# flupkede/codesearch

Measured on AMD Instinct MI355X. Metric: chunks embedded+searched/sec over 10M×384 corpus; recall@10 vs CPU ref, higher is better.
Workload: dtype f32

## Files before the change

codesearch_amd/_lib.py:

```python
from __future__ import annotations

import ctypes as C
import os

PKG_DIR = os.path.dirname(os.path.abspath(__file__))
LIB_PATH = os.environ.get("CS_LIBCSGPU") or os.path.join(PKG_DIR, "libcsgpu.so")
DIAG_LIB_PATH = os.environ.get("CS_LIBCSGPU_DIAG") or os.path.join(PKG_DIR, "libcsgpu_diag.so")

CS_OK, CS_ERR_BAD_ARG, CS_ERR_DIM_MISMATCH, CS_ERR_NOT_BUILT = 0, 1, 2, 3
CS_ERR_CANCELLED, CS_ERR_OOM, CS_ERR_HIP, CS_ERR_UNSUPPORTED = 4, 5, 6, 7
CS_GEMM_F32, CS_GEMM_SPLIT_F16, CS_GEMM_Q8_DYNAMIC = 0, 1, 2
CS_MAX_K = 1024
CS_MAX_QUERIES = 4096
CS_SIMILAR_EXCLUDE_NONE, CS_SIMILAR_EXCLUDE_SELF, CS_SIMILAR_EXCLUDE_GROUP = 0, 1, 2
CS_SIMILAR_ROUTE_AUTO, CS_SIMILAR_ROUTE_SCAN, CS_SIMILAR_ROUTE_FILTER = 0, 1, 2
CS_MAX_PAIRS = 1 << 22
CS_PAIRS_ALL, CS_PAIRS_OTHER_GROUP = 0, 1
CS_NO_ID = 0xFFFFFFFF
CS_NO_CLASS = 0xFFFF
CS_MAX_CLASSES = 4096

f32p = C.POINTER(C.c_float)
u32p = C.POINTER(C.c_uint32)
u16p = C.POINTER(C.c_uint16)
# ... 87 lines not shown
    "cs_index_search_similar": (C.c_int32, [vp, u32p, C.c_uint32, C.c_uint32, C.c_int32, C.c_float, f32p, u32p, u32p]),
    "cs_index_set_similar_route": (C.c_int32, [vp, C.c_int32]),
    "cs_index_similar_route_info": (C.c_int32, [vp, u64p, u64p, u64p]),
    "cs_index_search_similar_scoped": (C.c_int32, [vp, vp, u32p, C.c_uint32, C.c_uint32, C.c_int32, C.c_float, f32p, u32p,
                                                   u32p]),
    "cs_index_similar_pairs": (C.c_int32, [vp, C.c_float, C.c_int32, C.c_uint32, u32p, u32p, f32p, u64p]),
    "cs_index_similar_pairs_info": (C.c_int32, [u64p, u32p, f64p, f64p, f64p]),
    "cs_index_similar_clusters": (C.c_int32, [vp, C.c_float, C.c_int32, u32p, C.c_uint64, u64p, u64p]),
    "cs_index_similar_clusters_info": (C.c_int32, [u64p, u64p, u64p, u32p, f64p, f64p]),
    "cs_index_similar_clusters_scoped": (C.c_int32, [vp, vp, vp, C.c_float, C.c_int32, u32p, u32p, C.c_uint64, u64p, u64p, u64p]),
    "cs_index_similar_clusters_scoped_info": (C.c_int32, [f64p, u64p, u64p, u64p]),
    "cs_index_similar_pairs_scoped": (C.c_int32, [vp, vp, vp, C.c_float, C.c_int32, C.c_uint32, u32p, u32p, f32p, u64p]),
    "cs_index_similar_pairs_scoped_info": (C.c_int32, [f64p, u64p, u64p, u64p]),
    "cs_index_search_scoped": (C.c_int32, [vp, vp, f32p, C.c_uint32, C.c_uint32, C.c_uint32, f32p, u32p, u32p]),
    "cs_index_search_variants_scoped": (C.c_int32, [vp, vp, f32p, C.c_uint32, C.c_uint32, C.c_uint32, f32p, u32p, u32p,
                                                    i32p]),
    "cs_index_search_scoped_device": (C.c_int32, [vp, vp, vp, C.c_uint32, C.c_uint32, C.c_uint32, vp, vp, vp, vp, vp]),
    "cs_merge_variants_device": (C.c_int32, [C.c_int32, vp, C.c_uint32, C.c_uint32, C.c_uint32, vp, vp, vp, vp, vp, vp]),
    "cs_index_search_status": (C.c_int32, [vp, vp, u32p]),
    "cs_index_release_stream": (C.c_int32, [vp, vp]),
    "cs_merge_topk_device": (C.c_int32, [C.c_int32, vp, C.c_uint32, C.c_uint32, C.c_uint32, vp, vp, vp, vp, vp]),
    "cs_shards_create": (C.c_int32, [C.c_uint32, C.c_uint32, i32p, C.c_uint64, C.c_uint64, C.POINTER(vp)]),
    "cs_shards_destroy": (None, [vp]),
    "cs_shards_add": (C.c_int32, [vp, f32p, C.c_uint64, C.c_uint32, u32p]),
    "cs_shards_add_device": (C.c_int32, [vp, vp, C.c_int32, C.c_uint64, C.c_uint32, u32p, vp]),
    "cs_shards_add_synthetic": (C.c_int32, [vp, C.c_uint64, C.c_uint64, C.c_uint64, u32p]),
    "cs_shards_remove": (C.c_int32, [vp, u32p, C.c_uint64, u64p]),
    "cs_shards_build": (C.c_int32, [vp]),
    "cs_shards_clear": (C.c_int32, [vp]),
    "cs_shards_is_built": (C.c_int32, [vp]),
    "cs_shards_len": (C.c_uint64, [vp]),
    "cs_shards_stored_rows": (C.c_uint64, [vp]),
    "cs_shards_next_id": (C.c_uint32, [vp]),
    "cs_shards_dim": (C.c_uint32, [vp]),
    "cs_shards_count": (C.c_uint32, [vp]),
    "cs_shards_shard_len": (C.c_uint64, [vp, C.c_uint32]),
    "cs_shards_direct_gather": (C.c_int32, [vp]),
    "cs_shards_search": (C.c_int32, [vp, f32p, C.c_uint32, C.c_uint32, C.c_uint32, f32p, u32p, u32p]),
    "cs_shards_search_device": (C.c_int32, [vp, vp, C.c_uint32, C.c_uint32, C.c_uint32, vp, vp, vp, vp, vp]),
    "cs_shards_search_status": (C.c_int32, [vp, vp, u32p]),
    "cs_shards_root_device": (C.c_int32, [vp]),
    "cs_shards_shard_device": (C.c_int32, [vp, C.c_uint32]),
    "cs_shards_shard_index": (vp, [vp, C.c_uint32]),
    "cs_shards_search_variants": (C.c_int32, [vp, f32p, C.c_uint32, C.c_uint32, C.c_uint32, f32p, u32p, u32p, i32p]),
    "cs_shards_search_masked": (C.c_int32, [vp, f32p, C.c_uint32, C.c_uint32, C.c_uint32, u32p, C.c_uint64, f32p, u32p,
                                            u32p]),
    "cs_shards_search_variants_masked": (C.c_int32, [vp, f32p, C.c_uint32, C.c_uint32, C.c_uint32, u32p, C.c_uint64, f32p,
                                                     u32p, u32p, i32p]),
    "cs_shards_scope_create": (C.c_int32, [vp, u32p, C.c_uint64, C.POINTER(vp)]),
    "cs_shards_search_scoped": (C.c_int32, [vp, vp, f32p, C.c_uint32, C.c_uint32, C.c_uint32, f32p, u32p, u32p]),
    "cs_shards_search_variants_scoped": (C.c_int32, [vp, vp, f32p, C.c_uint32, C.c_uint32, C.c_uint32, f32p, u32p, u32p,
                                                     i32p]),
    "cs_shards_read_rows": (C.c_int32, [vp, C.c_uint64, C.c_uint64, f32p]),
    "cs_index_read_rows": (C.c_int32, [vp, C.c_uint64, C.c_uint64, f32p]),
    "cs_index_debug_counters": (C.c_int32, [vp, u64p, u64p]),
    "cs_index_filter_state": (C.c_int32, [vp, C.POINTER(C.c_int32), C.POINTER(C.c_float), u64p]),
    "cs_index_filter_copies": (C.c_int32, [vp, C.POINTER(C.c_int32), C.POINTER(C.c_int32), u64p]),
    "cs_index_set_filter_min_queries": (C.c_int32, [vp, C.c_uint32]),
    "cs_index_set_single_query_route": (C.c_int32, [vp, C.c_int32]),
    "cs_index_profile": (C.c_int32, [vp, C.c_int32]),
    "cs_index_profile_read": (C.c_int32, [vp, f64p, u64p, f64p, C.c_int32]),
    "cs_bert_config_bge_small": (None, [C.POINTER(BertConfig)]),
    "cs_bert_param_count": (C.c_uint64, [C.POINTER(BertConfig)]),
    "cs_embedder_create": (C.c_int32, [C.POINTER(BertConfig), f32p, C.c_uint64, C.c_int32, C.POINTER(vp)]),
    "cs_embedder_create_quantized": (C.c_int32, [C.POINTER(BertConfig), f32p, f32p, C.c_uint64, C.c_int32, C.POINTER(vp)]),
    "cs_bert_quant_columns": (C.c_uint64, [C.POINTER(BertConfig)]),
    "cs_bert_params_from_onnx_q": (C.c_int32, [C.c_char_p, C.POINTER(BertConfig), f32p, C.c_uint64, f32p, C.c_uint64,
                                               C.POINTER(C.c_int32)]),
    "cs_bert_config_from_dir": (C.c_int32, [C.c_char_p, C.c_int32, C.POINTER(BertConfig)]),
    "cs_bert_params_from_safetensors": (C.c_int32, [C.c_char_p, C.POINTER(BertConfig), f32p, C.c_uint64]),
    "cs_bert_params_from_onnx": (C.c_int32, [C.c_char_p, C.POINTER(BertConfig), f32p, C.c_uint64]),
    "cs_embedder_create_from_dir": (C.c_int32, [C.c_char_p, C.c_int32, C.c_int32, C.POINTER(vp)]),
    "cs_embedder_destroy": (None, [vp]),
    "cs_embedder_dim": (C.c_uint32, [vp]),
    "cs_embedder_embed_ids": (C.c_int32, [vp, i32p, i32p, C.c_uint64, C.c_uint32, C.c_uint32, f32p, i32p]),
    "cs_embedder_embed_ids_device": (C.c_int32, [vp, i32p, i32p, C.c_uint64, C.c_uint32, C.c_uint32, vp, i32p]),
    "cs_embedder_last_hidden": (C.c_int32, [vp, f32p, C.c_uint64]),
    "cs_embedder_profile_read": (C.c_int32, [vp, f64p, u64p, C.c_int32]),
    "cs_embedder_profile_stages": (C.c_int32, [vp, C.c_int32]),
    "cs_embedder_profile_stages_read": (C.c_int32, [vp, f64p, u64p, C.c_int32]),
    "cs_embedder_set_gemm_mode": (C.c_int32, [vp, C.c_int32]),
    "cs_embedder_gemm_mode": (C.c_int32, [vp]),
    "cs_embedder_debug_counters": (C.c_int32, [vp, u64p, u64p, u64p]),
    "cs_tokenizer_create": (C.c_int32, [C.c_char_p, C.c_uint64, C.c_int32, C.c_uint32, C.POINTER(vp)]),
    "cs_tokenizer_create_from_file": (C.c_int32, [C.c_char_p, C.c_int32, C.c_uint32, C.POINTER(vp)]),
    "cs_tokenizer_create_from_json": (C.c_int32, [C.c_char_p, C.c_uint32, C.POINTER(vp)]),
    "cs_tokenizer_create_from_dir": (C.c_int32, [C.c_char_p, C.c_uint32, C.POINTER(vp)]),
    "cs_tokenizer_destroy": (None, [vp]),
    "cs_tokenizer_vocab_size": (C.c_uint32, [vp]),
    "cs_tokenizer_max_length": (C.c_uint32, [vp]),
    "cs_tokenizer_pad_id": (C.c_int32, [vp]),
    "cs_tokenizer_token_to_id": (C.c_int32, [vp, C.c_char_p]),
    "cs_tokenizer_encode_batch": (C.c_int32, [vp, C.c_char_p, u64p, C.c_uint32, C.c_uint32, i32p, i32p,
                                              C.c_uint32, u32p]),
    "cs_tokenizer_encode_pairs": (C.c_int32, [vp, C.c_char_p, u64p, C.c_uint32, C.c_char_p, u64p, C.c_uint32, C.c_uint32, i32p, i32p,
                                              i32p, C.c_uint32, u32p]),
    "cs_embedder_embed_texts": (C.c_int32, [vp, vp, C.c_char_p, u64p, C.c_uint64, C.c_uint32, f32p, i32p]),
    "cs_embedder_embed_texts_device": (C.c_int32, [vp, vp, C.c_char_p, u64p, C.c_uint64, C.c_uint32, vp, i32p]),
    "cs_embedder_submit_texts": (C.c_int32, [vp, vp, C.c_char_p, u64p, C.c_uint64, u64p]),
    "cs_embedder_submit_ids": (C.c_int32, [vp, i32p, i32p, C.c_uint64, C.c_uint32, u64p]),
    "cs_embedder_wait": (C.c_int32, [vp, C.c_uint64, f32p, i32p]),
    "cs_embedder_wait_device": (C.c_int32, [vp, C.c_uint64, vp, i32p]),
    "cs_embedder_discard": (C.c_int32, [vp, C.c_uint64]),
    "cs_embedder_queued_rows": (C.c_uint64, [vp]),
    "cs_shards_plan_append": (C.c_int32, [vp, C.c_uint64, C.c_uint32, u32p, u64p, u64p, u32p]),
    "cs_shards_add_device_parts": (C.c_int32, [vp, C.c_uint32, C.POINTER(vp), i32p, u64p, C.c_uint32, u32p]),
    "cs_embedders_create": (C.c_int32, [C.POINTER(BertConfig), f32p, C.c_uint64, i32p, C.c_uint32, C.POINTER(vp)]),
    "cs_embedders_create_from_dir": (C.c_int32, [C.c_char_p, C.c_int32, i32p, C.c_uint32, C.POINTER(vp)]),
    "cs_embedders_destroy": (None, [vp]),
    "cs_embedders_count": (C.c_uint32, [vp]),
    "cs_embedders_dim": (C.c_uint32, [vp]),
    "cs_embedders_replica": (vp, [vp, C.c_uint32]),
    "cs_embedders_device": (C.c_int32, [vp, C.c_uint32]),
    "cs_embedders_embed_texts": (C.c_int32, [vp, vp, C.c_char_p, u64p, C.c_uint64, C.c_uint32, f32p, i32p]),
    "cs_embedders_embed_ids": (C.c_int32, [vp, i32p, i32p, C.c_uint64, C.c_uint32, C.c_uint32, f32p, i32p]),
    "cs_embedders_index_texts": (C.c_int32, [vp, vp, vp, C.c_char_p, u64p, C.c_uint64, C.c_uint32, u32p, i32p]),
    "cs_embedders_index_ids": (C.c_int32, [vp, vp, i32p, i32p, C.c_uint64, C.c_uint32, C.c_uint32, u32p, i32p]),
    "cs_rerank_head_count": (C.c_uint64, [C.POINTER(BertConfig)]),
    "cs_reranker_create": (C.c_int32, [C.POINTER(BertConfig), f32p, f32p, C.c_uint64, C.c_int32, C.POINTER(vp)]),
    "cs_rerank_head_from_safetensors": (C.c_int32, [C.c_char_p, C.POINTER(BertConfig), f32p, C.c_uint64]),
    "cs_reranker_create_from_dir": (C.c_int32, [C.c_char_p, C.c_int32, C.POINTER(vp)]),
    "cs_reranker_destroy": (None, [vp]),
    "cs_reranker_embedder": (vp, [vp]),
    "cs_reranker_score_ids": (C.c_int32, [vp, i32p, i32p, i32p, C.c_uint64, C.c_uint32, C.c_uint32, f32p, i32p]),
    "cs_reranker_rerank_texts": (C.c_int32, [vp, vp, C.c_char_p, C.c_char_p, u64p, C.c_uint64, C.c_uint32, f32p, u32p, f32p]),
    "cs_rerank_order": (C.c_int32, [f32p, C.c_uint64, u32p, f32p]),
    "cs_rerank_blend": (C.c_int32, [f32p, f32p, C.c_uint64, u32p, f32p]),
}

DIAG_SIGNATURES = {
    "cs_debug_small_forward_counters": (C.c_int32, [vp, u64p, u64p]),
    "cs_debug_gemm_time": (C.c_int32, [C.c_int32, C.c_int32, C.c_int32, C.c_uint32, C.c_uint32, C.c_uint32, C.c_uint32,
                                       C.c_int32, f64p]),
    "cs_debug_gemm_q8": (C.c_int32, [C.c_int32, C.c_int32, C.c_int32, f32p, f32p, f32p, f32p, f32p, f32p, C.c_uint32,
                                     C.c_uint32, C.c_uint32, C.POINTER(C.c_uint8), f32p, i32p]),
    "cs_debug_gemm_q8_units": (C.c_int32, [C.c_int32, C.c_int32, f32p, f32p, f32p, f32p, f32p, f32p, C.c_uint32, C.c_uint32,
                                           C.c_uint32, u32p, C.c_uint32, f32p, i32p]),
    "cs_debug_gemm": (C.c_int32, [C.c_int32, C.c_int32, C.c_int32, f32p, f32p, f32p, f32p, f32p,
                                  C.c_uint32, C.c_uint32, C.c_uint32, u32p]),
    "cs_debug_rows": (C.c_int32, [C.c_int32, C.c_int32, C.c_uint32, C.c_uint32, C.c_uint32, C.c_uint32, C.c_float, C.c_int32,
                                  i32p, f32p, f32p, f32p, i32p, C.c_uint32, C.c_uint32, f32p, i32p, f32p, C.c_uint32, f32p, f32p, f32p,
                                  C.c_int32, f32p, f32p, f32p, f32p, u32p]),
    "cs_debug_elementwise": (C.c_int32, [C.c_int32, C.c_int32, C.c_int32, C.c_uint32, C.c_uint32, C.c_uint32, C.c_uint32, C.c_uint32,
                                         C.c_int32, C.c_float, f32p, f32p, f32p, f32p, u32p]),
    "cs_debug_attention_cls": (C.c_int32, [C.c_int32, f32p, i32p, C.c_uint32, C.c_uint32, C.c_uint32, C.c_uint32, f32p, u32p, f32p,
                                           f32p, C.POINTER(C.c_uint16)]),
    "cs_debug_attention_f32": (C.c_int32, [C.c_int32, f32p, i32p, C.c_uint32, C.c_uint32, C.c_uint32, C.c_uint32, f32p, C.c_uint32,
                                           f32p]),
    "cs_debug_small_path": (C.c_int32, [C.c_int32, C.c_int32, C.c_int32, C.c_int32, C.c_uint32, C.c_uint32, C.c_uint32, C.c_uint32,
                                        C.c_float, f32p, f32p, f32p, f32p, f32p, f32p, i32p, f32p, f32p, f32p, i32p, C.c_uint32,
                                        C.c_uint32, f32p, f32p, f32p, f32p, f32p, f32p, u32p, u32p]),
    "cs_debug_attention": (C.c_int32, [C.c_int32, f32p, i32p, C.c_uint32, C.c_uint32, C.c_uint32, C.c_uint32, f32p, C.c_uint32,
                                       u32p, u32p, C.c_uint32, f32p, f32p, f32p, f32p, f32p, C.c_uint32, u32p, u32p]),
}

_LIB = None
_DIAG = None


def load() -> C.CDLL:
    global _LIB
    if _LIB is not None:
        return _LIB
    if not os.path.exists(LIB_PATH):
        raise FileNotFoundError(
            f"{LIB_PATH} is missing: build it with `python -c 'import __graft_entry__ as g; g.build()'` "
            "(make -C codesearch_amd/csrc). There is no CPU fallback."
        )
    try:
        import torch
    except Exception:
        pass
    lib = C.CDLL(LIB_PATH, mode=C.RTLD_GLOBAL)
    for name, (res, args) in SIGNATURES.items():
        fn = getattr(lib, name)
        fn.restype = res
        fn.argtypes = args
    _LIB = lib
    return lib


def load_diag() -> C.CDLL:
    global _DIAG
    if _DIAG is not None:
        return _DIAG
    if not os.path.exists(DIAG_LIB_PATH):
        raise FileNotFoundError(f"{DIAG_LIB_PATH} is missing: build it with `make -C codesearch_amd/csrc`")
    load()
    lib = C.CDLL(DIAG_LIB_PATH, mode=C.RTLD_LOCAL)
    for name, (res, args) in {**SIGNATURES, **DIAG_SIGNATURES}.items():
        fn = getattr(lib, name)
        fn.restype = res
        fn.argtypes = args
    _DIAG = lib
    return lib


def check_diag(status: int) -> None:
    if status != CS_OK:
        raise CsError(status, load_diag().cs_last_error().decode("utf-8", "replace"))


def last_error() -> str:
    return load().cs_last_error().decode("utf-8", "replace")


def check(status: int) -> None:
    if status != CS_OK:
        raise CsError(status, last_error())
```

codesearch_amd/csrc/attention_shx_body.hpp:

```cpp
#pragma once

#include "encoder.hpp"
#include "split_f16.hpp"

#ifndef AT_STAMP
#define AT_STAMP(i)
#endif
#ifndef CS_ATTN_ARITH
#define CS_ATTN_ARITH 2
#endif
#ifndef CS_ATTN_LAZY_RESCALE
#define CS_ATTN_LAZY_RESCALE 4.0f
#endif
#ifndef CS_ATTN_PIPE_FENCE
#define CS_ATTN_PIPE_FENCE __builtin_amdgcn_sched_barrier(0)
#endif

namespace cs {

typedef __fp16 h16x2 __attribute__((ext_vector_type(2)));

constexpr float kLog2e = 1.4426950408889634f;
constexpr float kMaskedLog2 = -3.0e38f;

union Frag8 {
    f16x8 v;
    uint32_t u[4];
    uint2 d[2];
};

typedef short s16x4 __attribute__((ext_vector_type(4)));

union FragTr {
    f16x8 v;
    s16x4 q[2];
};

__device__ __forceinline__ void split_pair_rtz_ng(float a, float b, uint32_t& hi, uint32_t& lo) {
    const h16x2 h = __builtin_amdgcn_cvt_pkrtz(a, b);
    const h16x2 l = __builtin_amdgcn_cvt_pkrtz((a - (float)h[0]) * kShLoScale, (b - (float)h[1]) * kShLoScale);
    hi = __builtin_bit_cast(uint32_t, h);
    lo = __builtin_bit_cast(uint32_t, l);
}

__device__ __forceinline__ float mix_residual_lo(float e, uint32_t hpair) {
    float r;
    asm("v_fma_mix_f32 %0, %1, -1.0, %2 op_sel_hi:[1,0,0]" : "=v"(r) : "v"(hpair), "v"(e));
    return r;
}
__device__ __forceinline__ float mix_residual_hi(float e, uint32_t hpair) {
    float r;
    asm("v_fma_mix_f32 %0, %1, -1.0, %2 op_sel:[1,0,0] op_sel_hi:[1,0,0]" : "=v"(r) : "v"(hpair), "v"(e));
    return r;
}

__device__ __forceinline__ float xhalf_max_swap(float t) {
    const uint32_t u = __builtin_bit_cast(uint32_t, t);
    const auto r = __builtin_amdgcn_permlane32_swap(u, u, false, false);
    const uint32_t a = r[0], b = r[1];
    return fmaxf(__builtin_bit_cast(float, a), __builtin_bit_cast(float, b));
}

struct AttnMemPlain {
    __device__ __forceinline__ f16x8 ld16(const _Float16* p) const { return *reinterpret_cast<const f16x8*>(p); }
    __device__ __forceinline__ f16x8 stage_load(const _Float16* src, char* lds_piece) const { sh_glds16(src, lds_piece); return f16x8{}; }
    __device__ __forceinline__ void stage_store(char*, int, f16x8) const {}
    __device__ __forceinline__ void st8(_Float16* p, f16x4 v) const { *reinterpret_cast<f16x4*>(p) = v; }
};

template <int NC, class MQ, class MO, int POS = 0, int PIPE = 0>
__device__ __forceinline__ void
attention_shx_body(char* smem, const MQ& mq, const MO& mo, const _Float16* qkvs, const int32_t* __restrict__ mask,
                   _Float16* ctxs, uint32_t* __restrict__ flag, uint32_t L, uint32_t H,
                   float scale_log2e, uint32_t HB, float* __restrict__ range_out,
                   const uint32_t* __restrict__ seq_unit, const uint32_t* __restrict__ unit_len,
                   uint32_t bx, uint32_t by, uint32_t bz, uint32_t gx, uint32_t gz, const float* __restrict__ alibi_log2 = nullptr,
                   uint32_t window = 0) {
    constexpr bool ALIBI = POS == 1, WINDOW = POS == 2;
    constexpr bool IMM = PIPE >= 2;
    constexpr bool EARLY = PIPE == 3;
    const float wlimit = (float)window;
    constexpr int KT = 128;
    const uint32_t Lp = (L + 31) & ~31u;
    char* Kt = smem;
    char* Vt = Kt + (size_t)NC * KT * 128;
    float* madd = reinterpret_cast<float*>(Vt + (size_t)NC * KT * 128);
    int* last_valid_p = reinterpret_cast<int*>(madd + Lp);
    const int tid = threadIdx.x, lane = tid & 63;
    const int wave = __builtin_amdgcn_readfirstlane(tid >> 6);
    const int l31 = lane & 31, h = lane >> 5;
    const uint32_t wq = 4 / HB, hsub = (uint32_t)wave / wq, qt = (uint32_t)wave % wq;
    const uint32_t head = bx * HB + hsub, b = by, qb = bz;
    Kt += (size_t)hsub * (KT / HB) * 128;
    Vt += (size_t)hsub * (KT / HB) * 128;
    const uint32_t nh = H / (32 * NC), nch = 3 * nh * NC;
    const _Float16* base = qkvs + (size_t)b * L * nch * 64;
    bool ovf = false;

    AT_STAMP(0);
    if (tid == 0) *last_valid_p = 0;

    const int kswz = (l31 >> 1) & 7;
    int k_hi[2], k_lo[2];
#pragma unroll
    for (int s = 0; s < 2; ++s) {
        k_hi[s] = ((2 * s + h) ^ kswz) * 16;
        k_lo[s] = ((4 + 2 * s + h) ^ kswz) * 16;
    }
    const int vq = (lane & 15) >> 2, vp = lane & 3, vg = (lane >> 4) & 1;
    const int vfv = 4 * ((vq >> 1) & 1);
    const int v_hi = (4 * h + vq) * 128 + (((2 * vg + (vp >> 1)) ^ vfv) * 16) + 8 * (vp & 1);
    const int v_lo = v_hi ^ 64;

    const bool wave_live = qb * 128 + qt * 32 < L;
    const uint32_t query = qb * 128 + qt * 32 + l31;
    const uint32_t qsrc = query < L ? query : L - 1;
    float neg_slope = 0.0f;
    const float qpos = (float)query - (float)(4 * h);
    if constexpr (ALIBI) neg_slope = -alibi_log2[head];
    f16x8 qh[NC][2], ql[NC][2];
#pragma unroll
    for (int c = 0; c < NC; ++c) {
        const _Float16* qp = base + ((size_t)qsrc * nch + head * NC + c) * 64 + 8 * h;
#pragma unroll
        for (int s = 0; s < 2; ++s) {
            qh[c][s] = mq.ld16(qp + 16 * s);
            ql[c][s] = mq.ld16(qp + 32 + 16 * s);
        }
    }
#if CS_ATTN_ARITH == 2 && !defined(CS_ATTN_SCALAR_SOFTMAX)
    f16x8 qhs[NC][2];
#pragma unroll
    for (int c = 0; c < NC; ++c)
#pragma unroll
        for (int s = 0; s < 2; ++s) {
            qhs[c][s] = qh[c][s] * (_Float16)kShLoInv;
            ql[c][s] = ql[c][s] * (_Float16)kShLoInv;
        }
#endif
    sh_f32x16 ohh[NC], oxx[NC];
#pragma unroll
    for (int c = 0; c < NC; ++c)
#pragma unroll
        for (int r = 0; r < 16; ++r) { ohh[c][r] = 0.0f; oxx[c][r] = 0.0f; }
    float m = -__builtin_huge_valf(), lsum = 0.0f;

    auto stage = [&](uint32_t st) {
        const uint32_t live = Lp - st * KT < (uint32_t)KT ? Lp - st * KT : (uint32_t)KT;
        for (uint32_t i0 = qt; i0 < live / 8; i0 += 4 * wq) {
            f16x8 rk[4][NC], rv[4][NC];
#pragma unroll
            for (int u = 0; u < 4; ++u) {
                const uint32_t ii = i0 + u * wq;
                if (ii < live / 8) {
                    const uint32_t row = ii * 8 + (lane >> 3);
                    const uint32_t gk = st * KT + row;
                    const uint32_t key = gk < L ? gk : L - 1;
                    const uint32_t ck = (lane & 7) ^ ((row >> 1) & 7);
                    const uint32_t cv = (lane & 7) ^ (4 * ((row >> 1) & 1));
#pragma unroll
                    for (int c = 0; c < NC; ++c) {
                        rk[u][c] = mq.stage_load(base + ((size_t)key * nch + (nh + head) * NC + c) * 64 + ck * 8, Kt + (size_t)c * KT * 128 + ii * 1024);
                        rv[u][c] = mq.stage_load(base + ((size_t)key * nch + (2 * nh + head) * NC + c) * 64 + cv * 8, Vt + (size_t)c * KT * 128 + ii * 1024);
                    }
                }
            }
#pragma unroll
            for (int u = 0; u < 4; ++u) {
                const uint32_t ii = i0 + u * wq;
                if (ii < live / 8) {
#pragma unroll
                    for (int c = 0; c < NC; ++c) {
                        mq.stage_store(Kt + (size_t)c * KT * 128 + ii * 1024, lane, rk[u][c]);
                        mq.stage_store(Vt + (size_t)c * KT * 128 + ii * 1024, lane, rv[u][c]);
                    }
                }
            }
        }
    };
    stage(0);
    __syncthreads();
    for (uint32_t key = tid; key < Lp; key += 256) {
        const bool ok = key < L && mask[(size_t)b * L + key] != 0;
        madd[key] = ok ? 0.0f : kMaskedLog2;
        if (ok) atomicMax(last_valid_p, (int)key);
    }
    asm volatile("s_waitcnt vmcnt(0)" ::: "memory");
    __syncthreads();
    const uint32_t ntiles = (uint32_t)(*last_valid_p) / 32 + 1;

    typedef __attribute__((address_space(3))) char* lds_char_p;
    typedef __attribute__((address_space(3))) const f16x8* lds_f16x8_cp;
    typedef __attribute__((address_space(3))) const sh_f32x4* lds_f32x4_cp;
    uint32_t ka[4] = {0, 0, 0, 0}, va[2] = {0, 0}, ma0 = 0;
    if constexpr (IMM) {
        const uint32_t k0 = (uint32_t)(uintptr_t)(lds_char_p)Kt + (uint32_t)l31 * 128u, v0 = (uint32_t)(uintptr_t)(lds_char_p)Vt;
#pragma unroll
        for (int s = 0; s < 2; ++s) { ka[s] = k0 + (uint32_t)k_hi[s]; ka[2 + s] = k0 + (uint32_t)k_lo[s]; }
        va[0] = v0 + (uint32_t)v_hi;
        va[1] = v0 + (uint32_t)v_lo;
        ma0 = (uint32_t)(uintptr_t)(lds_char_p)reinterpret_cast<char*>(madd) + 16u * (uint32_t)h;
#pragma unroll
        for (int i = 0; i < 4; ++i) asm volatile("" : "+v"(ka[i]));
        asm volatile("" : "+v"(va[0]), "+v"(va[1]), "+v"(ma0));
    }

    for (uint32_t st = 0; st * 4 < ntiles; ++st) {
        if constexpr (WINDOW) {
            if (st * KT > qb * 128 + 127 + window || st * KT + (KT - 1) + window < qb * 128) continue;
        }
        if (st > 0) {
            __syncthreads();
            stage(st);
            asm volatile("s_waitcnt vmcnt(0)" ::: "memory");
            __syncthreads();
        }
        if (!wave_live) continue;
        const uint32_t kt_end = ntiles - st * 4 < 4 ? ntiles - st * 4 : 4;
        const uint32_t ma_st = ma0 + st * 512u;
        uint32_t kl_lo = 0, kl_hi = kt_end;
        if constexpr (WINDOW) {
            const int q0 = (int)(qb * 128 + qt * 32), w = (int)window, t0 = (int)(st * 4);
            const int first = q0 - 31 - w > 0 ? (q0 - 31 - w + 31) / 32 : 0, past = (q0 + 31 + w) / 32 + 1;
            kl_lo = (uint32_t)(first > t0 ? first - t0 : 0);
            kl_hi = past - t0 < (int)kt_end ? (uint32_t)(past - t0 > 0 ? past - t0 : 0) : kt_end;
        }
        auto compute_s = [&](uint32_t kl, sh_f32x16& hh, sh_f32x16& xx) __attribute__((always_inline)) {
#pragma unroll
            for (int r = 0; r < 16; ++r) { hh[r] = 0.0f; xx[r] = 0.0f; }
            if constexpr (EARLY) {
                f16x8 kf[NC][4];
#pragma unroll
                for (int c = 0; c < NC; ++c)
#pragma unroll
                    for (int i = 0; i < 4; ++i) kf[c][i] = *(lds_f16x8_cp)(uintptr_t)(ka[i] + (uint32_t)(c * KT * 128) + kl * 4096u);
                __builtin_amdgcn_sched_barrier(0);
#pragma unroll
                for (int c = 0; c < NC; ++c)
#pragma unroll
                    for (int s = 0; s < 2; ++s) {
                        hh = __builtin_amdgcn_mfma_f32_32x32x16_f16(kf[c][s], qh[c][s], hh, 0, 0, 0);
#if CS_ATTN_ARITH == 2 && !defined(CS_ATTN_SCALAR_SOFTMAX)
                        hh = __builtin_amdgcn_mfma_f32_32x32x16_f16(kf[c][s], ql[c][s], hh, 0, 0, 0);
                        hh = __builtin_amdgcn_mfma_f32_32x32x16_f16(kf[c][2 + s], qhs[c][s], hh, 0, 0, 0);
#else
                        xx = __builtin_amdgcn_mfma_f32_32x32x16_f16(kf[c][s], ql[c][s], xx, 0, 0, 0);
                        xx = __builtin_amdgcn_mfma_f32_32x32x16_f16(kf[c][2 + s], qh[c][s], xx, 0, 0, 0);
#endif
                    }
                return;
            }
#pragma unroll
            for (int c = 0; c < NC; ++c) {
                const char* kr = Kt + (size_t)c * KT * 128 + (size_t)(kl * 32 + l31) * 128;
#pragma unroll
                for (int s = 0; s < 2; ++s) {
                    f16x8 kh, kl8;
                    if constexpr (IMM) {
                        kh = *(lds_f16x8_cp)(uintptr_t)(ka[s] + (uint32_t)(c * KT * 128) + kl * 4096u);
                        kl8 = *(lds_f16x8_cp)(uintptr_t)(ka[2 + s] + (uint32_t)(c * KT * 128) + kl * 4096u);
                    } else {
                        kh = *reinterpret_cast<const f16x8*>(kr + k_hi[s]);
                        kl8 = *reinterpret_cast<const f16x8*>(kr + k_lo[s]);
                    }
                    hh = __builtin_amdgcn_mfma_f32_32x32x16_f16(kh, qh[c][s], hh, 0, 0, 0);
#if CS_ATTN_ARITH == 2 && !defined(CS_ATTN_SCALAR_SOFTMAX)
                    hh = __builtin_amdgcn_mfma_f32_32x32x16_f16(kh, ql[c][s], hh, 0, 0, 0);
                    hh = __builtin_amdgcn_mfma_f32_32x32x16_f16(kl8, qhs[c][s], hh, 0, 0, 0);
#else
                    xx = __builtin_amdgcn_mfma_f32_32x32x16_f16(kh, ql[c][s], xx, 0, 0, 0);
                    xx = __builtin_amdgcn_mfma_f32_32x32x16_f16(kl8, qh[c][s], xx, 0, 0, 0);
#endif
                }
            }
        };
        auto finish_tile = [&](uint32_t kl, sh_f32x16& hh, sh_f32x16& xx) __attribute__((always_inline)) {
            const uint32_t kt = st * 4 + kl;
#ifndef CS_ATTN_SCALAR_SOFTMAX
            sh_f32x2 p2[8];
            float tmax = -__builtin_huge_valf();
            const sh_f32x2 lo_inv2 = {kShLoInv, kShLoInv}, scale2 = {scale_log2e, scale_log2e};
#pragma unroll
            for (int g = 0; g < 4; ++g) {
                sh_f32x4 ma;
                if constexpr (IMM) ma = *(lds_f32x4_cp)(uintptr_t)(ma_st + (kl * 32u + 8u * g) * 4u);
                else ma = *reinterpret_cast<const sh_f32x4*>(madd + kt * 32 + 8 * g + 4 * h);
#pragma unroll
                for (int e2 = 0; e2 < 2; ++e2) {
                    const int r = 4 * g + 2 * e2;
                    const sh_f32x2 x2 = {xx[r], xx[r + 1]}, h2 = {hh[r], hh[r + 1]};
                    sh_f32x2 m2 = {ma[2 * e2], ma[2 * e2 + 1]};
                    if constexpr (ALIBI) {
                        const float d0 = qpos - (float)(kt * 32 + 8 * g + 2 * e2);
                        m2[0] = fmaf(neg_slope, fabsf(d0), m2[0]);
                        m2[1] = fmaf(neg_slope, fabsf(d0 - 1.0f), m2[1]);
                    }
                    if constexpr (WINDOW) {
                        const float d0 = qpos - (float)(kt * 32 + 8 * g + 2 * e2);
                        m2[0] = fabsf(d0) > wlimit ? kMaskedLog2 : m2[0];
                        m2[1] = fabsf(d0 - 1.0f) > wlimit ? kMaskedLog2 : m2[1];
                    }
#if CS_ATTN_ARITH == 2
                    (void)x2; (void)lo_inv2;
                    const sh_f32x2 s2 = __builtin_elementwise_fma(h2, scale2, m2);
#else
                    const sh_f32x2 s2 = __builtin_elementwise_fma(__builtin_elementwise_fma(x2, lo_inv2, h2), scale2, m2);
#endif
                    p2[r / 2] = s2;
                    tmax = fmaxf(tmax, fmaxf(s2[0], s2[1]));
                }
            }
            if constexpr (IMM) tmax = xhalf_max_swap(tmax);
            else tmax = fmaxf(tmax, __shfl_xor(tmax, 32, 64));
#if CS_ATTN_ARITH == 2
            if (__any(tmax > m + CS_ATTN_LAZY_RESCALE)) {
#else
            if (__any(tmax > m)) {
#endif
                const float mnew = fmaxf(m, tmax);
                const float alpha = __builtin_amdgcn_exp2f(m - mnew);
                lsum *= alpha;
#pragma unroll
                for (int c = 0; c < NC; ++c)
#pragma unroll
                    for (int r = 0; r < 16; ++r) { ohh[c][r] *= alpha; oxx[c][r] *= alpha; }
                m = mnew;
            }
            typedef __attribute__((address_space(3))) s16x4* lds_s16x4_p;
            FragTr vhe[NC][2], vle[NC][2];
            if constexpr (EARLY) {
#pragma unroll
                for (int c = 0; c < NC; ++c)
#pragma unroll
                    for (int s = 0; s < 2; ++s) {
                        const uint32_t off = (uint32_t)(c * KT * 128) + kl * 4096u + (uint32_t)(s * 16 * 128);
                        vhe[c][s].q[0] = __builtin_amdgcn_ds_read_tr16_b64_v4i16((lds_s16x4_p)(uintptr_t)(va[0] + off));
                        vhe[c][s].q[1] = __builtin_amdgcn_ds_read_tr16_b64_v4i16((lds_s16x4_p)(uintptr_t)(va[0] + off + 1024u));
                        vle[c][s].q[0] = __builtin_amdgcn_ds_read_tr16_b64_v4i16((lds_s16x4_p)(uintptr_t)(va[1] + off));
                        vle[c][s].q[1] = __builtin_amdgcn_ds_read_tr16_b64_v4i16((lds_s16x4_p)(uintptr_t)(va[1] + off + 1024u));
                    }
                __builtin_amdgcn_sched_barrier(0);
            }
#if CS_ATTN_ARITH == 2
            const sh_f32x2 m2v = {m - 11.0f, m - 11.0f};
#else
            const sh_f32x2 m2v = {m, m};
#endif
            sh_f32x2 ps2 = {0.0f, 0.0f};
            Frag8 ph[2], pl[2];
            const sh_f32x2 lo_scale2 = {kShLoScale, kShLoScale};
#pragma unroll
            for (int i = 0; i < 8; ++i) {
                const sh_f32x2 d2 = p2[i] - m2v;
                const sh_f32x2 e2 = {__builtin_amdgcn_exp2f(d2[0]), __builtin_amdgcn_exp2f(d2[1])};
                ps2 += e2;
                const h16x2 hi = __builtin_amdgcn_cvt_pkrtz(e2[0], e2[1]);
#if CS_ATTN_ARITH == 2
                (void)lo_scale2;
                const uint32_t hib = __builtin_bit_cast(uint32_t, hi);
                const h16x2 lo = __builtin_amdgcn_cvt_pkrtz(mix_residual_lo(e2[0], hib), mix_residual_hi(e2[1], hib));
#else
                const sh_f32x2 back = {(float)hi[0], (float)hi[1]};
                const sh_f32x2 r2 = (e2 - back) * lo_scale2;
                const h16x2 lo = __builtin_amdgcn_cvt_pkrtz(r2[0], r2[1]);
#endif
                ph[i >> 2].u[i & 3] = __builtin_bit_cast(uint32_t, hi);
                pl[i >> 2].u[i & 3] = __builtin_bit_cast(uint32_t, lo);
            }
            lsum += ps2[0] + ps2[1];
#else
            float tmax = -__builtin_huge_valf();
#pragma unroll
            for (int g = 0; g < 4; ++g) {
                const sh_f32x4 ma = *reinterpret_cast<const sh_f32x4*>(madd + kt * 32 + 8 * g + 4 * h);
#pragma unroll
                for (int e = 0; e < 4; ++e) {
                    const int r = 4 * g + e;
                    float me = ma[e];
                    if constexpr (ALIBI) me = fmaf(neg_slope, fabsf(qpos - (float)(kt * 32 + 8 * g + e)), me);
                    if constexpr (WINDOW) me = fabsf(qpos - (float)(kt * 32 + 8 * g + e)) > wlimit ? kMaskedLog2 : me;
                    hh[r] = fmaf(fmaf(xx[r], kShLoInv, hh[r]), scale_log2e, me);
                    tmax = fmaxf(tmax, hh[r]);
                }
            }
            tmax = fmaxf(tmax, __shfl_xor(tmax, 32, 64));
            if (__any(tmax > m)) {
                const float mnew = fmaxf(m, tmax);
                const float alpha = __builtin_amdgcn_exp2f(m - mnew);
                lsum *= alpha;
#pragma unroll
                for (int c = 0; c < NC; ++c)
#pragma unroll
                    for (int r = 0; r < 16; ++r) { ohh[c][r] *= alpha; oxx[c][r] *= alpha; }
                m = mnew;
            }
            float psum = 0.0f;
#pragma unroll
            for (int r = 0; r < 16; ++r) {
                hh[r] = __builtin_amdgcn_exp2f(hh[r] - m);
                psum += hh[r];
            }
            lsum += psum;
            Frag8 ph[2], pl[2];
#pragma unroll
            for (int s = 0; s < 2; ++s)
#pragma unroll
                for (int w2 = 0; w2 < 4; ++w2) {
#ifdef CS_ATTN_P_HI_ONLY
                    const f16x2 pr = __builtin_convertvector(sh_f32x2{hh[8 * s + 2 * w2], hh[8 * s + 2 * w2 + 1]}, f16x2);
                    ph[s].u[w2] = __builtin_bit_cast(uint32_t, pr);
                    pl[s].u[w2] = 0u;
#else
                    split_pair_rtz_ng(hh[8 * s + 2 * w2], hh[8 * s + 2 * w2 + 1], ph[s].u[w2], pl[s].u[w2]);
#endif
                }
#endif
#ifdef CS_ATTN_SCALAR_SOFTMAX
            typedef __attribute__((address_space(3))) s16x4* lds_s16x4_p;
            FragTr vhe[NC][2], vle[NC][2];
#endif
#pragma unroll
            for (int c = 0; c < NC; ++c) {
                const char* vr = Vt + (size_t)c * KT * 128 + (size_t)kl * 32 * 128;
#pragma unroll
                for (int s = 0; s < 2; ++s) {
                    FragTr vh, vl;
                    if constexpr (EARLY) {
                        vh = vhe[c][s];
                        vl = vle[c][s];
                    } else if constexpr (IMM) {
                        const uint32_t off = (uint32_t)(c * KT * 128) + kl * 4096u + (uint32_t)(s * 16 * 128);
                        vh.q[0] = __builtin_amdgcn_ds_read_tr16_b64_v4i16((lds_s16x4_p)(uintptr_t)(va[0] + off));
                        vh.q[1] = __builtin_amdgcn_ds_read_tr16_b64_v4i16((lds_s16x4_p)(uintptr_t)(va[0] + off + 1024u));
                        vl.q[0] = __builtin_amdgcn_ds_read_tr16_b64_v4i16((lds_s16x4_p)(uintptr_t)(va[1] + off));
                        vl.q[1] = __builtin_amdgcn_ds_read_tr16_b64_v4i16((lds_s16x4_p)(uintptr_t)(va[1] + off + 1024u));
                    } else {
                    vh.q[0] = __builtin_amdgcn_ds_read_tr16_b64_v4i16((lds_s16x4_p)(vr + s * 16 * 128 + v_hi));
                    vh.q[1] = __builtin_amdgcn_ds_read_tr16_b64_v4i16((lds_s16x4_p)(vr + s * 16 * 128 + 8 * 128 + v_hi));
                    vl.q[0] = __builtin_amdgcn_ds_read_tr16_b64_v4i16((lds_s16x4_p)(vr + s * 16 * 128 + v_lo));
                    vl.q[1] = __builtin_amdgcn_ds_read_tr16_b64_v4i16((lds_s16x4_p)(vr + s * 16 * 128 + 8 * 128 + v_lo));
                    }
                    ohh[c] = __builtin_amdgcn_mfma_f32_32x32x16_f16(vh.v, ph[s].v, ohh[c], 0, 0, 0);
#if CS_ATTN_ARITH == 2 && !defined(CS_ATTN_SCALAR_SOFTMAX)
                    ohh[c] = __builtin_amdgcn_mfma_f32_32x32x16_f16(vh.v, pl[s].v, ohh[c], 0, 0, 0);
#elif !defined(CS_ATTN_P_HI_ONLY)
                    oxx[c] = __builtin_amdgcn_mfma_f32_32x32x16_f16(vh.v, pl[s].v, oxx[c], 0, 0, 0);
#endif
                    oxx[c] = __builtin_amdgcn_mfma_f32_32x32x16_f16(vl.v, ph[s].v, oxx[c], 0, 0, 0);
                }
            }
        };
        if constexpr (PIPE == 0) {
            for (uint32_t kl = kl_lo; kl < kl_hi; ++kl) {
                sh_f32x16 hh, xx;
                compute_s(kl, hh, xx);
                finish_tile(kl, hh, xx);
            }
        } else if constexpr (IMM) {
#pragma unroll
            for (uint32_t kl = 0; kl < 4; ++kl) {
                if (kl >= kl_lo && kl < kl_hi) {
                    sh_f32x16 hh, xx;
                    compute_s(kl, hh, xx);
                    finish_tile(kl, hh, xx);
                }
            }
        } else {
            sh_f32x16 hhA, xxA, hhB, xxB;
            if (kl_lo < kl_hi) compute_s(kl_lo, hhA, xxA);
            for (uint32_t kl = kl_lo; kl < kl_hi; kl += 2) {
                if (kl + 1 < kl_hi) compute_s(kl + 1, hhB, xxB);
                CS_ATTN_PIPE_FENCE;
                finish_tile(kl, hhA, xxA);
                if (kl + 1 < kl_hi) {
                    if (kl + 2 < kl_hi) compute_s(kl + 2, hhA, xxA);
                    CS_ATTN_PIPE_FENCE;
                    finish_tile(kl + 1, hhB, xxB);
                }
            }
        }
    }
    lsum += __shfl_xor(lsum, 32, 64);
    const float inv = lsum > 0.0f ? 1.0f / lsum : 0.0f;
    float rlo = 0.0f, rhi = 0.0f;
    if (wave_live && query < L) {
#pragma unroll
        for (int c = 0; c < NC; ++c) {
            _Float16* op = ctxs + (((size_t)b * L + query) * nh + head) * NC * 64 + c * 64 + 4 * h;
#pragma unroll
            for (int g = 0; g < 4; ++g) {
                f16x4 hi, lo;
#pragma unroll
                for (int e = 0; e < 4; ++e) {
                    _Float16 a, bb;
                    const float o = fmaf(oxx[c][4 * g + e], kShLoInv, ohh[c][4 * g + e]) * inv;
                    ovf |= sh_split(o, a, bb);
                    hi[e] = a; lo[e] = bb;
                    rlo = fminf(rlo, o);
                    rhi = fmaxf(rhi, o);
                }
                mo.st8(op + 8 * g, hi);
                mo.st8(op + 32 + 8 * g, lo);
            }
        }
    }
    AT_STAMP(2);
    if (ovf && flag) atomicOr(flag, 1u);
    if (range_out) {
        if (unit_len && query >= unit_len[seq_unit[b]]) rlo = rhi = 0.0f;
#pragma unroll
        for (int o = 32; o > 0; o >>= 1) {
            rlo = fminf(rlo, __shfl_xor(rlo, o, 64));
            rhi = fmaxf(rhi, __shfl_xor(rhi, o, 64));
        }
        if (lane == 0) {
            const size_t blk = ((size_t)by * gz + bz) * gx + bx;
            _Float16 a, bb;
            (void)sh_split(rlo, a, bb);
            range_out[(blk * 4 + wave) * 2] = fmaf((float)bb, kShLoInv, (float)a);
            (void)sh_split(rhi, a, bb);
            range_out[(blk * 4 + wave) * 2 + 1] = fmaf((float)bb, kShLoInv, (float)a);
        }
    }
}

}
```

codesearch_amd/csrc/attention_split.hip:

```cpp
#include <cstdlib>
#include "encoder.hpp"
#include "split_f16.hpp"
#include "attention_shx_body.hpp"

#ifndef AT_STAMP
#define AT_STAMP(i)
#endif

namespace cs {

#ifndef CS_ATTN_PIPE_WAVES
#define CS_ATTN_PIPE_WAVES 3
#endif

constexpr int kAttnPipeDefault32 = 2, kAttnPipeDefault64 = 3;

#ifdef CS_DIAGNOSTICS
__global__ void __launch_bounds__(256, 2)
attention_sh2_kernel(const _Float16* __restrict__ qkvs, const int32_t* __restrict__ mask,
                     _Float16* __restrict__ ctxs, uint32_t* __restrict__ flag, uint32_t L, uint32_t H,
                     float scale_log2e) {
    extern __shared__ __attribute__((aligned(16))) char smem[];
    const uint32_t Lp = (L + 31) & ~31u;
    char* Kt = smem;
    char* Vt = Kt + (size_t)Lp * 128;
    float* madd = reinterpret_cast<float*>(Vt + (size_t)Lp * 128);
    int* last_valid_p = reinterpret_cast<int*>(madd + Lp);
    const int tid = threadIdx.x, lane = tid & 63;
    const int wave = __builtin_amdgcn_readfirstlane(tid >> 6);
    const int l31 = lane & 31, h = lane >> 5;
    const uint32_t head = blockIdx.x, b = blockIdx.y;
    const uint32_t nh = H / 32, nch = 3 * nh;
    const _Float16* base = qkvs + (size_t)b * L * nch * 64;
    bool ovf = false;

    AT_STAMP(0);
    if (tid == 0) *last_valid_p = 0;
    for (uint32_t ii = wave; ii < Lp / 8; ii += 4) {
        const uint32_t row = ii * 8 + (lane >> 3);
        const uint32_t key = row < L ? row : L - 1;
        const uint32_t ck = (lane & 7) ^ ((row >> 1) & 7);
        const uint32_t cv = (lane & 7) ^ (4 * ((row >> 1) & 1));
        sh_glds16(base + ((size_t)key * nch + nh + head) * 64 + ck * 8, Kt + ii * 1024);
        sh_glds16(base + ((size_t)key * nch + 2 * nh + head) * 64 + cv * 8, Vt + ii * 1024);
    }
    __syncthreads();
    for (uint32_t key = tid; key < Lp; key += 256) {
        const bool ok = key < L && mask[(size_t)b * L + key] != 0;
        madd[key] = ok ? 0.0f : kMaskedLog2;
        if (ok) atomicMax(last_valid_p, (int)key);
    }
    asm volatile("s_waitcnt vmcnt(0)" ::: "memory");
    __syncthreads();
    const uint32_t ntiles = (uint32_t)(*last_valid_p) / 32 + 1;
    AT_STAMP(1);

    const int kswz = (l31 >> 1) & 7;
    const char* k_lane = Kt + l31 * 128;
    int k_hi[2], k_lo[2];
#pragma unroll
    for (int s = 0; s < 2; ++s) {
        k_hi[s] = ((2 * s + h) ^ kswz) * 16;
        k_lo[s] = ((4 + 2 * s + h) ^ kswz) * 16;
    }
    const int vq = (lane & 15) >> 2, vp = lane & 3, vg = (lane >> 4) & 1;
    const int vfv = 4 * ((vq >> 1) & 1);
    const int v_hi = (4 * h + vq) * 128 + (((2 * vg + (vp >> 1)) ^ vfv) * 16) + 8 * (vp & 1);
    const int v_lo = v_hi ^ 64;

    for (uint32_t qb = 0; qb * 128 < L; ++qb) {
        if (qb * 128 + wave * 32 >= L) break;
        const uint32_t query = qb * 128 + wave * 32 + l31;
        const uint32_t qsrc = query < L ? query : L - 1;
        const _Float16* qp = base + ((size_t)qsrc * nch + head) * 64 + 8 * h;
        f16x8 qh[2], ql[2];
#pragma unroll
        for (int s = 0; s < 2; ++s) {
            qh[s] = *reinterpret_cast<const f16x8*>(qp + 16 * s);
            ql[s] = *reinterpret_cast<const f16x8*>(qp + 32 + 16 * s);
        }
        sh_f32x16 ohh, oxx;
#pragma unroll
        for (int r = 0; r < 16; ++r) { ohh[r] = 0.0f; oxx[r] = 0.0f; }
        float m = -__builtin_huge_valf(), lsum = 0.0f;

        for (uint32_t kt = 0; kt < ntiles; ++kt) {
            sh_f32x16 hh, xx;
#pragma unroll
            for (int r = 0; r < 16; ++r) { hh[r] = 0.0f; xx[r] = 0.0f; }
            const char* kr = k_lane + (size_t)kt * 32 * 128;
#pragma unroll
            for (int s = 0; s < 2; ++s) {
                const f16x8 kh = *reinterpret_cast<const f16x8*>(kr + k_hi[s]);
                const f16x8 kl = *reinterpret_cast<const f16x8*>(kr + k_lo[s]);
                hh = __builtin_amdgcn_mfma_f32_32x32x16_f16(kh, qh[s], hh, 0, 0, 0);
                xx = __builtin_amdgcn_mfma_f32_32x32x16_f16(kh, ql[s], xx, 0, 0, 0);
                xx = __builtin_amdgcn_mfma_f32_32x32x16_f16(kl, qh[s], xx, 0, 0, 0);
            }
            float tmax = -__builtin_huge_valf();
#pragma unroll
            for (int g = 0; g < 4; ++g) {
                const sh_f32x4 ma = *reinterpret_cast<const sh_f32x4*>(madd + kt * 32 + 8 * g + 4 * h);
#pragma unroll
                for (int e = 0; e < 4; ++e) {
                    const int r = 4 * g + e;
                    hh[r] = fmaf(fmaf(xx[r], kShLoInv, hh[r]), scale_log2e, ma[e]);
                    tmax = fmaxf(tmax, hh[r]);
                }
            }
            tmax = fmaxf(tmax, __shfl_xor(tmax, 32, 64));
            if (__any(tmax > m)) {
                const float mnew = fmaxf(m, tmax);
                const float alpha = __builtin_amdgcn_exp2f(m - mnew);
                lsum *= alpha;
#pragma unroll
                for (int r = 0; r < 16; ++r) { ohh[r] *= alpha; oxx[r] *= alpha; }
                m = mnew;
            }
            float psum = 0.0f;
#pragma unroll
            for (int r = 0; r < 16; ++r) {
                hh[r] = __builtin_amdgcn_exp2f(hh[r] - m);
                psum += hh[r];
            }
            lsum += psum;
            Frag8 ph[2], pl[2];
#pragma unroll
            for (int s = 0; s < 2; ++s)
#pragma unroll
                for (int w2 = 0; w2 < 4; ++w2)
                    split_pair_rtz_ng(hh[8 * s + 2 * w2], hh[8 * s + 2 * w2 + 1], ph[s].u[w2], pl[s].u[w2]);
            typedef __attribute__((address_space(3))) s16x4* lds_s16x4_p;
            const char* vr = Vt + (size_t)kt * 32 * 128;
#pragma unroll
            for (int s = 0; s < 2; ++s) {
                FragTr vh, vl;
                vh.q[0] = __builtin_amdgcn_ds_read_tr16_b64_v4i16((lds_s16x4_p)(vr + s * 16 * 128 + v_hi));
                vh.q[1] = __builtin_amdgcn_ds_read_tr16_b64_v4i16((lds_s16x4_p)(vr + s * 16 * 128 + 8 * 128 + v_hi));
                vl.q[0] = __builtin_amdgcn_ds_read_tr16_b64_v4i16((lds_s16x4_p)(vr + s * 16 * 128 + v_lo));
                vl.q[1] = __builtin_amdgcn_ds_read_tr16_b64_v4i16((lds_s16x4_p)(vr + s * 16 * 128 + 8 * 128 + v_lo));
                ohh = __builtin_amdgcn_mfma_f32_32x32x16_f16(vh.v, ph[s].v, ohh, 0, 0, 0);
                oxx = __builtin_amdgcn_mfma_f32_32x32x16_f16(vh.v, pl[s].v, oxx, 0, 0, 0);
                oxx = __builtin_amdgcn_mfma_f32_32x32x16_f16(vl.v, ph[s].v, oxx, 0, 0, 0);
            }
        }
        lsum += __shfl_xor(lsum, 32, 64);
        const float inv = 1.0f / lsum;
        if (query < L) {
            _Float16* op = ctxs + (((size_t)b * L + query) * nh + head) * 64 + 4 * h;
#pragma unroll
            for (int g = 0; g < 4; ++g) {
                f16x4 hi, lo;
#pragma unroll
                for (int e = 0; e < 4; ++e) {
                    _Float16 a, bb;
                    ovf |= sh_split(fmaf(oxx[4 * g + e], kShLoInv, ohh[4 * g + e]) * inv, a, bb);
                    hi[e] = a; lo[e] = bb;
                }
                *reinterpret_cast<f16x4*>(op + 8 * g) = hi;
                *reinterpret_cast<f16x4*>(op + 32 + 8 * g) = lo;
            }
        }
    }
    AT_STAMP(2);
    if (ovf && flag) atomicOr(flag, 1u);
}
#endif

template <int NC, int POS = 0, int PIPE = 0>
__global__ void __launch_bounds__(256, NC == 1 ? (PIPE == 1 ? CS_ATTN_PIPE_WAVES : (PIPE >= 2 ? 4 : 2)) : 2)
attention_shx_kernel(const _Float16* __restrict__ qkvs, const int32_t* __restrict__ mask,
                     _Float16* __restrict__ ctxs, uint32_t* __restrict__ flag, uint32_t L, uint32_t H,
                     float scale_log2e, uint32_t HB, float* __restrict__ range_out,
                     const uint32_t* __restrict__ seq_unit, const uint32_t* __restrict__ unit_len,
                     const float* __restrict__ alibi_log2, uint32_t window) {
    extern __shared__ __attribute__((aligned(16))) char smem[];
    const AttnMemPlain mem;
    attention_shx_body<NC, AttnMemPlain, AttnMemPlain, POS, PIPE>(smem, mem, mem, qkvs, mask, ctxs, flag, L, H, scale_log2e, HB, range_out,
                                                            seq_unit, unit_len, blockIdx.x, blockIdx.y, blockIdx.z, gridDim.x,
                                                            gridDim.z, alibi_log2, window);
}

namespace {

struct ShxArgs {
    const _Float16* qkv; const int32_t* mask; _Float16* ctx; uint32_t* flag; uint32_t L, H; float scale_log2e; uint32_t hb;
    float* range_out; const uint32_t* seq_unit; const uint32_t* unit_len; const float* alibi_log2; uint32_t window;
};

template <int NC, int POS, int PIPE>
int32_t launch_shx_one(dim3 grid, size_t lds, hipStream_t s, const ShxArgs& a) {
    if (lds > 64 * 1024 - 256) {
        static PerDeviceOnce attr;
        CS_TRY(attr.run([&]() -> int32_t {
            CS_HIP(hipFuncSetAttribute(reinterpret_cast<const void*>(attention_shx_kernel<NC, POS, PIPE>),
                                       hipFuncAttributeMaxDynamicSharedMemorySize, 160 * 1024 - 64));
            return CS_OK;
        }));
    }
    hipLaunchKernelGGL((attention_shx_kernel<NC, POS, PIPE>), grid, dim3(256), lds, s, a.qkv, a.mask, a.ctx, a.flag, a.L, a.H,
                       a.scale_log2e, a.hb, a.range_out, a.seq_unit, a.unit_len, a.alibi_log2, a.window);
    CS_HIP(hipGetLastError());
    return CS_OK;
}

template <int NC>
int32_t launch_shx(int pos, int pipe, dim3 grid, size_t lds, hipStream_t s, const ShxArgs& a) {
#ifndef CS_DIAGNOSTICS
    constexpr int P = NC == 1 ? kAttnPipeDefault32 : kAttnPipeDefault64;
    (void)pipe;
    if (pos == 1) return launch_shx_one<NC, 1, P>(grid, lds, s, a);
    if (pos == 2) return launch_shx_one<NC, 2, P>(grid, lds, s, a);
    return launch_shx_one<NC, 0, P>(grid, lds, s, a);
#else
    if (pipe == 3) {
        if (pos == 1) return launch_shx_one<NC, 1, 3>(grid, lds, s, a);
        if (pos == 2) return launch_shx_one<NC, 2, 3>(grid, lds, s, a);
        return launch_shx_one<NC, 0, 3>(grid, lds, s, a);
    }
    if (pipe == 2) {
        if (pos == 1) return launch_shx_one<NC, 1, 2>(grid, lds, s, a);
        if (pos == 2) return launch_shx_one<NC, 2, 2>(grid, lds, s, a);
        return launch_shx_one<NC, 0, 2>(grid, lds, s, a);
    }
    if (pipe == 1) {
        if (pos == 1) return launch_shx_one<NC, 1, 1>(grid, lds, s, a);
        if (pos == 2) return launch_shx_one<NC, 2, 1>(grid, lds, s, a);
        return launch_shx_one<NC, 0, 1>(grid, lds, s, a);
    }
    if (pos == 1) return launch_shx_one<NC, 1, 0>(grid, lds, s, a);
    if (pos == 2) return launch_shx_one<NC, 2, 0>(grid, lds, s, a);
    return launch_shx_one<NC, 0, 0>(grid, lds, s, a);
#endif
}

}

int32_t launch_attention_sh2(const _Float16* qkv_split, const int32_t* mask, void* ctx_split, uint32_t* flag,
                             uint32_t B, uint32_t L, uint32_t H, uint32_t heads, hipStream_t s, float* range_out,
                             uint32_t* range_pairs, const uint32_t* seq_unit, const uint32_t* unit_len, const float* alibi,
                             uint32_t window) {
    if (alibi && window) return fail(CS_ERR_BAD_ARG, "attention: ALiBi and a local window together are not built");
    const float* alibi_log2 = alibi ? alibi + heads : nullptr;
    const int pos = alibi_log2 ? 1 : (window ? 2 : 0);
    if (range_pairs) *range_pairs = 0;
    const uint32_t dh = heads ? H / heads : 0;
    if ((dh != 32 && dh != 64) || H % heads)
        return fail(CS_ERR_UNSUPPORTED, "head_dim %u not supported (32 or 64)", dh);
    const size_t Lp = (L + 31) & ~31u;
    static const int pipe_env = [] { const char* e = cs_lab_env("CS_ATTN_PIPE"); return e && e[0] >= '0' && e[0] <= '3' ? e[0] - '0' : -1; }();
    ShxArgs a{qkv_split, mask, static_cast<_Float16*>(ctx_split), flag, L, H, 0.0f, 1u, range_out, seq_unit, unit_len, alibi_log2, window};
    if (dh == 64) {
        const size_t lds = 2 * 2 * 128 * 128 + Lp * sizeof(float) + 16;
        a.scale_log2e = (1.0f / sqrtf(64.0f)) * kLog2e;
        const int pipe = pipe_env < 0 ? kAttnPipeDefault64 : pipe_env;
        CS_TRY(launch_shx<2>(pos, pipe, dim3(heads, B, (L + 127) / 128), lds, s, a));
        if (range_pairs) *range_pairs = heads * B * ((L + 127) / 128) * 4;
        return CS_OK;
    }
    static const bool shx1 = [] { const char* e = cs_lab_env("CS_ATTN_SHX1"); return !(e && e[0] == '0'); }();
    if (shx1 || pos) {
        static const size_t lds_pad = [] { const char* e = cs_lab_env("CS_ATTN_LDS_PAD"); return e ? (size_t)std::atol(e) : (size_t)0; }();
        const size_t lds1 = 2 * 1 * 128 * 128 + Lp * sizeof(float) + 16 + lds_pad;
        static const bool pack_heads = [] { const char* e = cs_lab_env("CS_ATTN_PACK_HEADS"); return !(e && e[0] == '0'); }();
        uint32_t hb = !pack_heads ? 1u : (Lp <= 32 ? 4u : (Lp <= 64 ? 2u : 1u));
        while (heads % hb) hb >>= 1;
        a.scale_log2e = (1.0f / sqrtf(32.0f)) * kLog2e;
        a.hb = hb;
        const int pipe = pipe_env < 0 ? kAttnPipeDefault32 : pipe_env;
        CS_TRY(launch_shx<1>(pos, pipe, dim3(heads / hb, B, (L + 127) / 128), lds1, s, a));
        if (range_pairs) *range_pairs = (heads / hb) * B * ((L + 127) / 128) * 4;
        return CS_OK;
    }
#ifndef CS_DIAGNOSTICS
    return fail(CS_ERR_UNSUPPORTED, "attention: no kernel for head_dim %u", dh);
#else
    const size_t lds = 2 * Lp * 128 + Lp * sizeof(float) + 16;
    if (lds > 160 * 1024 - 64) return fail(CS_ERR_UNSUPPORTED, "sequence length %u exceeds the LDS-resident K/V limit", L);
    static PerDeviceOnce attr_set;
    CS_TRY(attr_set.run([&]() -> int32_t {
        CS_HIP(hipFuncSetAttribute(reinterpret_cast<const void*>(attention_sh2_kernel),
                                   hipFuncAttributeMaxDynamicSharedMemorySize, 160 * 1024 - 64));
        return CS_OK;
    }));
    hipLaunchKernelGGL(attention_sh2_kernel, dim3(heads, B), dim3(256), lds, s, qkv_split, mask,
                       static_cast<_Float16*>(ctx_split), flag, L, H, (1.0f / sqrtf(32.0f)) * kLog2e);
    CS_HIP(hipGetLastError());
    return CS_OK;
#endif
}

}
```

codesearch_amd/csrc/diagnostics.hip:

```cpp
#include "embedder_state.hpp"
#include "scan.hpp"
#include "../../include/codesearch_gpu_diag.h"

using namespace cs;
using namespace cs::emb;

extern "C" {

int32_t cs_debug_gemm(int32_t device, int32_t mode, int32_t epilogue, const float* A, const float* W,
                      const float* bias, const float* resid, float* C, uint32_t M, uint32_t N, uint32_t K,
                      uint32_t* range_flag) {
    if (!A || !W || !bias || !C || ((epilogue == 2 || epilogue == 3) && !resid)) return fail(CS_ERR_BAD_ARG, "null buffer");
    const bool wide = mode == 2;
    if (wide) mode = CS_GEMM_SPLIT_F16;
    if (epilogue == 3 && !(wide && N == 384)) return fail(CS_ERR_UNSUPPORTED, "epilogue 3 needs mode 2 and N = 384");
    if (epilogue < 0 || epilogue > 4 || (mode != CS_GEMM_F32 && mode != CS_GEMM_SPLIT_F16))
        return fail(CS_ERR_BAD_ARG, "unknown epilogue/mode");
    if (wide && !gemm_wide_supported(N, K)) return fail(CS_ERR_UNSUPPORTED, "wide kernel needs N %% 384 == 0");
    if (M == 0 || N % 128 || K % 32 || K == 0) return fail(CS_ERR_UNSUPPORTED, "cs_debug_gemm needs M > 0, N %% 128 == 0, K %% 32 == 0");
    int ndev = 0;
    CS_HIP(hipGetDeviceCount(&ndev));
    if (device < 0 || device >= ndev) return fail(CS_ERR_HIP, "HIP device %d not available (%d visible)", device, ndev);
    DeviceGuard g(device);
    const size_t a_n = (size_t)M * K, w_n = (size_t)N * K, c_n = (size_t)M * N;
// ... 163 lines not shown
                Q8RowMeta rm0;
                CS_HIP(hipMemcpy(hq.data(), dXq, a_n, hipMemcpyDeviceToHost));
                CS_HIP(hipMemcpy(&rm0, dRm, sizeof(rm0), hipMemcpyDeviceToHost));
                if (xq_out) for (size_t i = 0; i < a_n; ++i) xq_out[i] = (uint8_t)((int)hq[i] + 128);
                if (xparams) { xparams[0] = rm0.xs; xparams[1] = (float)(rm0.za + 128); }
            }
            return CS_OK;
        }
        const int epi = epilogue == 0 ? SH_OUT_F32 : epilogue == 1 ? SH_OUT_SPLIT_GELU : epilogue == 2 ? SH_OUT_F32_RESID : SH_OUT_SPLIT;
        if (epi == SH_OUT_SPLIT_GELU || epi == SH_OUT_SPLIT) CS_HIP(hipMalloc(&sC, c_n * 4));
        if (a_split & 4) {
            if (dAcc) CS_HIP(hipMemset(dAcc, 0, c_n * 4));
            CS_TRY(launch_gemm_q8_skinny(epi, (a_split & 1) ? Q8_SRC_SPLIT : Q8_SRC_F32, (a_split & 1) ? (const void*)sA : (const void*)dA,
                                         reinterpret_cast<const float*>(dRange), 1, dWq, dCm, dR, dC, sC, M, N, K, dF, nullptr, nullptr, nullptr));
        } else if (a_split & 16) {
            if (dAcc) CS_HIP(hipMemset(dAcc, 0, c_n * 4));
            CS_TRY(launch_gemm_q8_slab_split(dA, dRange, dWq, dCmT, sC, M, N, K, dF, nullptr));
        } else if (a_split & 8) {
            if (dAcc) CS_HIP(hipMemset(dAcc, 0, c_n * 4));
            CS_TRY(launch_gemm_q8_from_source(epi, (a_split & 1) ? Q8_SRC_SPLIT : Q8_SRC_F32, (a_split & 1) ? (const void*)sA : (const void*)dA, dRange,
                                              dWq, dCm, dB, dR, dC, sC, M, N, K, dF, nullptr));
        } else
        CS_TRY(launch_gemm_q8(epi, dXq, dRm, dWq, dCm, dB, dR, dC, sC, M, N, K, dF, nullptr, dAcc));
        CS_HIP(hipDeviceSynchronize());
        uint32_t flags[2] = {0, 0};
        CS_HIP(hipMemcpy(flags, dF, 8, hipMemcpyDeviceToHost));
        if (flags[1]) return fail(CS_ERR_BAD_ARG, "cs_debug_gemm_q8: W is not a quantised matrix for these column scales (flag %u)", flags[1]);
        if (sC) {
            std::vector<_Float16> hs(c_n * 2);
            CS_HIP(hipMemcpy(hs.data(), sC, c_n * 4, hipMemcpyDeviceToHost));
            const size_t nch = N / 32;
            for (size_t m = 0; m < M; ++m)
                for (size_t n = 0; n < N; ++n) {
                    const _Float16* line = hs.data() + (m * nch + n / 32) * 64;
                    C[m * N + n] = (float)line[n % 32] + (float)line[32 + n % 32] * (1.0f / 2048.0f);
                }
        } else {
            CS_HIP(hipMemcpy(C, dC, c_n * 4, hipMemcpyDeviceToHost));
        }
        if (acc_out) CS_HIP(hipMemcpy(acc_out, dAcc, c_n * 4, hipMemcpyDeviceToHost));
        if (xq_out || xparams) {
            std::vector<int8_t> hq(a_n);
            Q8RowMeta rm0;
            CS_HIP(hipMemcpy(hq.data(), dXq, a_n, hipMemcpyDeviceToHost));
            CS_HIP(hipMemcpy(&rm0, dRm, sizeof(rm0), hipMemcpyDeviceToHost));
            if (xq_out) for (size_t i = 0; i < a_n; ++i) xq_out[i] = (uint8_t)((int)hq[i] + 128);
            if (xparams) { xparams[0] = rm0.xs; xparams[1] = (float)(rm0.za + 128); }
        }
        return CS_OK;
    };
    const int32_t st = run();
    for (void* p : {(void*)dA, (void*)dW, (void*)dS, (void*)dB, (void*)dR, (void*)dC, (void*)sA, (void*)sC, (void*)dXq, (void*)dWq,
                    (void*)dRm, (void*)dCm, (void*)dF, (void*)dRange, (void*)dAcc, (void*)dCmT})
        if (p) (void)hipFree(p);
    return st;
}

int32_t cs_debug_gemm_q8_units(int32_t device, int32_t epilogue, const float* A, const float* W, const float* wscale,
                               const float* bias, const float* resid, float* C, uint32_t M, uint32_t N, uint32_t K,
                               const uint32_t* row_slot, uint32_t units, float* row_params, int32_t* rowsums) {
    if (!A || !W || !wscale || !bias || !C || !row_slot || (epilogue == 2 && !resid)) return fail(CS_ERR_BAD_ARG, "null buffer");
    if (epilogue != 2 && epilogue != 4 && epilogue != 5) return fail(CS_ERR_BAD_ARG, "unknown epilogue %d", epilogue);
    if (M == 0 || units == 0 || N % 128 || !q8_rows_from_source(forward_knobs(), M, K))
        return fail(CS_ERR_UNSUPPORTED, "cs_debug_gemm_q8_units: M=%u N=%u K=%u is not a row-block product", M, N, K);
    for (uint32_t m = 0; m < M; ++m)
        if ((row_slot[m] & 0x7fffffffu) >= units || (m && (row_slot[m] & 0x7fffffffu) < (row_slot[m - 1] & 0x7fffffffu)))
            return fail(CS_ERR_BAD_ARG, "row_slot[%u]: units must be consecutive runs of rows, in order", m);
    int ndev = 0;
    CS_HIP(hipGetDeviceCount(&ndev));
    if (device < 0 || device >= ndev) return fail(CS_ERR_HIP, "HIP device %d not available (%d visible)", device, ndev);
    DeviceGuard g(device);
    const size_t a_n = (size_t)M * K, w_n = (size_t)N * K, c_n = (size_t)M * N;
    float *dA = nullptr, *dW = nullptr, *dS = nullptr, *dB = nullptr, *dR = nullptr, *dC = nullptr;
    _Float16 *sA = nullptr, *sC = nullptr;
    int8_t *dXq = nullptr, *dWq = nullptr, *dOut = nullptr;
    Q8RowMeta *dRm = nullptr, *dRm2 = nullptr;
    Q8ColMeta* dCm = nullptr;
    uint32_t *dF = nullptr, *dRange = nullptr, *dRange2 = nullptr, *dSlot = nullptr;
    auto run = [&]() -> int32_t {
        const size_t rbytes = (size_t)units * Q8_RANGE_WORDS * 4;
        CS_HIP(hipMalloc(&dA, a_n * 4)); CS_HIP(hipMalloc(&dW, w_n * 4)); CS_HIP(hipMalloc(&dS, (size_t)N * 4));
        CS_HIP(hipMalloc(&dB, (size_t)N * 4)); CS_HIP(hipMalloc(&dC, c_n * 4)); CS_HIP(hipMalloc(&dF, 16));
        CS_HIP(hipMalloc(&dXq, a_n)); CS_HIP(hipMalloc(&dWq, w_n)); CS_HIP(hipMalloc(&dRm, (size_t)M * sizeof(Q8RowMeta)));
        CS_HIP(hipMalloc(&dCm, (size_t)N * sizeof(Q8ColMeta))); CS_HIP(hipMalloc(&dRange, rbytes)); CS_HIP(hipMalloc(&dRange2, rbytes));
        CS_HIP(hipMalloc(&dSlot, (size_t)M * 4));
        CS_HIP(hipMemcpy(dA, A, a_n * 4, hipMemcpyHostToDevice));
        CS_HIP(hipMemcpy(dW, W, w_n * 4, hipMemcpyHostToDevice));
        CS_HIP(hipMemcpy(dS, wscale, (size_t)N * 4, hipMemcpyHostToDevice));
        CS_HIP(hipMemcpy(dB, bias, (size_t)N * 4, hipMemcpyHostToDevice));
        CS_HIP(hipMemcpy(dSlot, row_slot, (size_t)M * 4, hipMemcpyHostToDevice));
        CS_HIP(hipMemset(dF, 0, 16));
        CS_HIP(hipMemset(dRange, 0, rbytes));
        CS_HIP(hipMemset(dRange2, 0, rbytes));
        CS_TRY(launch_q8_pack_weight(dW, dS, dB, N, K, dWq, dCm, dF + 1, nullptr));
        if (epilogue == 2) {
            CS_HIP(hipMalloc(&sA, a_n * 4));
            CS_HIP(hipMalloc(&dR, c_n * 4));
            CS_HIP(hipMemcpy(dR, resid, c_n * 4, hipMemcpyHostToDevice));
            CS_TRY(launch_split_rows(dA, sA, M, K, dF, nullptr));
            CS_TRY(launch_q8_quantize(Q8_SRC_SPLIT, sA, M, K, dRange, dSlot, dXq, dRm, nullptr));
            CS_TRY(launch_gemm_q8_from_source(SH_OUT_F32_RESID, Q8_SRC_SPLIT, sA, dRange, dWq, dCm, dB, dR, dC, nullptr, M, N, K, dF, nullptr, dSlot));
        } else {
            CS_TRY(launch_q8_quantize(Q8_SRC_F32, dA, M, K, dRange, dSlot, dXq, dRm, nullptr));
            if (epilogue == 4) {
                CS_HIP(hipMalloc(&sC, c_n * 4));
                CS_TRY(launch_gemm_q8_from_source(SH_OUT_SPLIT, Q8_SRC_F32, dA, dRange, dWq, dCm, dB, nullptr, nullptr, sC, M, N, K, dF, nullptr, dSlot));
            } else {
                CS_HIP(hipMalloc(&dOut, c_n));
                CS_HIP(hipMalloc(&dRm2, (size_t)M * sizeof(Q8RowMeta)));
                CS_TRY(launch_gemm_q8_gelu_requant_from_source(dA, dRange, dWq, dCm, dB, M, N, K, dRange2, dOut, dRm2, nullptr, dSlot));
            }
        }
        CS_HIP(hipDeviceSynchronize());
        uint32_t flags[2] = {0, 0};
        CS_HIP(hipMemcpy(flags, dF, 8, hipMemcpyDeviceToHost));
        if (flags[1]) return fail(CS_ERR_BAD_ARG, "cs_debug_gemm_q8_units: W is not a quantised matrix for these column scales (flag %u)", flags[1]);
        std::vector<Q8RowMeta> hr(M), hr2;
        CS_HIP(hipMemcpy(hr.data(), dRm, (size_t)M * sizeof(Q8RowMeta), hipMemcpyDeviceToHost));
        if (epilogue == 5) {
            std::vector<int8_t> ho(c_n);
            hr2.resize(M);
            CS_HIP(hipMemcpy(ho.data(), dOut, c_n, hipMemcpyDeviceToHost));
            CS_HIP(hipMemcpy(hr2.data(), dRm2, (size_t)M * sizeof(Q8RowMeta), hipMemcpyDeviceToHost));
            for (size_t i = 0; i < c_n; ++i) C[i] = (float)((int)ho[i] + 128);
            if (rowsums) for (size_t m = 0; m < M; ++m) rowsums[m] = hr2[m].rowsum + 128 * (int32_t)N;
        } else if (sC) {
            std::vector<_Float16> hs(c_n * 2);
            CS_HIP(hipMemcpy(hs.data(), sC, c_n * 4, hipMemcpyDeviceToHost));
            const size_t nch = N / 32;
            for (size_t m = 0; m < M; ++m)
                for (size_t n = 0; n < N; ++n) {
                    const _Float16* line = hs.data() + (m * nch + n / 32) * 64;
                    C[m * N + n] = (float)line[n % 32] + (float)line[32 + n % 32] * (1.0f / 2048.0f);
                }
        } else {
            CS_HIP(hipMemcpy(C, dC, c_n * 4, hipMemcpyDeviceToHost));
        }
        if (row_params)
            for (size_t m = 0; m < M; ++m) {
                row_params[4 * m] = hr[m].xs;
                row_params[4 * m + 1] = (float)(hr[m].za + 128);
                row_params[4 * m + 2] = epilogue == 5 ? hr2[m].xs : 0.0f;
                row_params[4 * m + 3] = epilogue == 5 ? (float)(hr2[m].za + 128) : 0.0f;
            }
        return CS_OK;
    };
    const int32_t st = run();
    for (void* p : {(void*)dA, (void*)dW, (void*)dS, (void*)dB, (void*)dR, (void*)dC, (void*)sA, (void*)sC, (void*)dXq, (void*)dWq,
                    (void*)dOut, (void*)dRm, (void*)dRm2, (void*)dCm, (void*)dF, (void*)dRange, (void*)dRange2, (void*)dSlot})
        if (p) (void)hipFree(p);
    return st;
}

int32_t cs_debug_attention(int32_t device, const float* qkv, const int32_t* mask, uint32_t B, uint32_t L, uint32_t H,
                           uint32_t heads, const float* alibi_slopes, uint32_t window, const uint32_t* seq_unit,
                           const uint32_t* unit_len, uint32_t units, const float* proj_w, const float* proj_bias,
                           const float* proj_resid, float* out, float* range_pairs_out, uint32_t range_pairs_cap,
                           uint32_t* range_pairs, uint32_t* range_flag) {
    if (!qkv || !mask || !out) return fail(CS_ERR_BAD_ARG, "null buffer");
    if (B == 0 || L == 0 || H == 0 || heads == 0) return fail(CS_ERR_BAD_ARG, "cs_debug_attention needs B, L, H, heads > 0");
    if (H % heads || (H / heads != 32 && H / heads != 64))
        return fail(CS_ERR_UNSUPPORTED, "head_dim %u not supported (32 or 64)", H / heads);
    if (L > 8192 || (uint64_t)B * L > (1u << 20)) return fail(CS_ERR_UNSUPPORTED, "cs_debug_attention: L <= 8192, B * L <= 2^20");
    if ((units != 0) != (seq_unit != nullptr) || (units != 0) != (unit_len != nullptr))
        return fail(CS_ERR_BAD_ARG, "seq_unit, unit_len and units go together");
    for (uint32_t b = 0; b < B && units; ++b)
        if (seq_unit[b] >= units) return fail(CS_ERR_BAD_ARG, "seq_unit[%u] = %u: only %u units", b, seq_unit[b], units);
    if ((range_pairs_out != nullptr) != (range_pairs != nullptr) || (range_pairs_out && range_pairs_cap == 0))
        return fail(CS_ERR_BAD_ARG, "range_pairs_out, its capacity and range_pairs go together");
    const uint32_t T = B * L;
    if (!proj_w != !proj_bias || !proj_w != !proj_resid) return fail(CS_ERR_BAD_ARG, "proj_w, proj_bias and proj_resid go together");
    if (proj_w) {
        if (alibi_slopes || window || units || range_pairs_out)
            return fail(CS_ERR_BAD_ARG, "attention inside the out-projection takes no ALiBi, window, units or range pairs");
        if (!sp_attn_proj_supported(H, heads, T, L))
            return fail(CS_ERR_UNSUPPORTED, "attention + out-projection in one launch: %u rows of %u tokens, hidden %u, %u heads not built", T, L, H, heads);
    }
    int ndev = 0;
    CS_HIP(hipGetDeviceCount(&ndev));
    if (device < 0 || device >= ndev) return fail(CS_ERR_HIP, "HIP device %d not available (%d visible)", device, ndev);
    DeviceGuard g(device);
    const size_t q_n = (size_t)T * 3 * H, c_n = (size_t)T * H;
    const size_t pair_cap = (size_t)heads * B * ((L + 127) / 128) * 4;
    float *dQ = nullptr, *dW = nullptr, *dB = nullptr, *dR = nullptr, *dC = nullptr, *dAl = nullptr, *dRp = nullptr;
    _Float16 *sQ = nullptr, *sW = nullptr, *sC = nullptr;
    int32_t* dM = nullptr;
    uint32_t *dF = nullptr, *dSu = nullptr, *dUl = nullptr;
    auto run = [&]() -> int32_t {
        CS_HIP(hipMalloc(&dQ, q_n * 4)); CS_HIP(hipMalloc(&sQ, q_n * 4)); CS_HIP(hipMalloc(&dM, (size_t)T * 4)); CS_HIP(hipMalloc(&dF, 4));
        CS_HIP(hipMemcpy(dQ, qkv, q_n * 4, hipMemcpyHostToDevice));
        CS_HIP(hipMemcpy(dM, mask, (size_t)T * 4, hipMemcpyHostToDevice));
        CS_HIP(hipMemset(dF, 0, 4));
        CS_TRY(launch_split_rows(dQ, sQ, T, 3 * H, dF, nullptr));
        if (proj_w) {
            CS_HIP(hipMalloc(&dW, (size_t)H * H * 4)); CS_HIP(hipMalloc(&sW, (size_t)H * H * 4)); CS_HIP(hipMalloc(&dB, (size_t)H * 4));
            CS_HIP(hipMalloc(&dR, c_n * 4)); CS_HIP(hipMalloc(&dC, c_n * 4));
            CS_HIP(hipMemcpy(dW, proj_w, (size_t)H * H * 4, hipMemcpyHostToDevice));
            CS_HIP(hipMemcpy(dB, proj_bias, (size_t)H * 4, hipMemcpyHostToDevice));
            CS_HIP(hipMemcpy(dR, proj_resid, c_n * 4, hipMemcpyHostToDevice));
            CS_TRY(launch_split_rows(dW, sW, H, H, dF, nullptr));
            CS_TRY(launch_sp_attn_proj(sQ, dM, sW, dB, dR, dC, T, L, H, heads, dF, nullptr));
            CS_HIP(hipDeviceSynchronize());
            CS_HIP(hipMemcpy(out, dC, c_n * 4, hipMemcpyDeviceToHost));
            if (range_flag) CS_HIP(hipMemcpy(range_flag, dF, 4, hipMemcpyDeviceToHost));
            return CS_OK;
        }
        CS_HIP(hipMalloc(&sC, c_n * 4));
        CS_HIP(hipMemset(sC, 0, c_n * 4));
        if (alibi_slopes) {
            std::vector<float> sl(2 * (size_t)heads);
            for (uint32_t i = 0; i < heads; ++i) { sl[i] = alibi_slopes[i]; sl[heads + i] = sl[i] * 1.4426950408889634f; }
            CS_HIP(hipMalloc(&dAl, sl.size() * 4));
            CS_HIP(hipMemcpy(dAl, sl.data(), sl.size() * 4, hipMemcpyHostToDevice));
        }
        if (units) {
            CS_HIP(hipMalloc(&dSu, (size_t)B * 4)); CS_HIP(hipMalloc(&dUl, (size_t)units * 4));
            CS_HIP(hipMemcpy(dSu, seq_unit, (size_t)B * 4, hipMemcpyHostToDevice));
            CS_HIP(hipMemcpy(dUl, unit_len, (size_t)units * 4, hipMemcpyHostToDevice));
        }
        if (range_pairs_out) {
            CS_HIP(hipMalloc(&dRp, pair_cap * 8));
            CS_HIP(hipMemset(dRp, 0, pair_cap * 8));
        }
        uint32_t pairs = 0;
        CS_TRY(launch_attention_sh2(sQ, dM, sC, dF, B, L, H, heads, nullptr, dRp, range_pairs_out ? &pairs : nullptr, dSu, dUl, dAl, window));
        CS_HIP(hipDeviceSynchronize());
        if (range_pairs_out) {
            *range_pairs = pairs;
            if (pairs > pair_cap) return fail(CS_ERR_HIP, "attention reported %u range pairs, more than one per wave (%zu)", pairs, pair_cap);
            if (pairs > range_pairs_cap) return fail(CS_ERR_BAD_ARG, "range_pairs_out holds %u pairs, the launch wrote %u", range_pairs_cap, pairs);
            CS_HIP(hipMemcpy(range_pairs_out, dRp, (size_t)pairs * 8, hipMemcpyDeviceToHost));
        }
        std::vector<_Float16> hs(c_n * 2);
        CS_HIP(hipMemcpy(hs.data(), sC, c_n * 4, hipMemcpyDeviceToHost));
        const size_t nch = H / 32;
        for (size_t m = 0; m < T; ++m)
            for (size_t n = 0; n < H; ++n) {
                const _Float16* line = hs.data() + (m * nch + n / 32) * 64;
                out[m * H + n] = (float)line[n % 32] + (float)line[32 + n % 32] * (1.0f / 2048.0f);
            }
        if (range_flag) CS_HIP(hipMemcpy(range_flag, dF, 4, hipMemcpyDeviceToHost));
        return CS_OK;
    };
    const int32_t st = run();
    if (st != CS_OK) (void)hipDeviceSynchronize();
    for (void* p : {(void*)dQ, (void*)dW, (void*)dB, (void*)dR, (void*)dC, (void*)dAl, (void*)dRp, (void*)sQ, (void*)sW, (void*)sC,
                    (void*)dM, (void*)dF, (void*)dSu, (void*)dUl})
        if (p) (void)hipFree(p);
    return st;
}

}

namespace {

struct DiagBufs {
    std::vector<void*> owned;
    ~DiagBufs() {
        (void)hipDeviceSynchronize();
        for (void* q : owned) (void)hipFree(q);
    }
    template <class T>
    int32_t get(T** out, size_t bytes, const void* host = nullptr) {
        void* q = nullptr;
        CS_HIP(hipMalloc(&q, bytes ? bytes : 4));
        owned.push_back(q);
        if (host && bytes) CS_HIP(hipMemcpy(q, host, bytes, hipMemcpyHostToDevice));
        *out = static_cast<T*>(q);
        return CS_OK;
    }
};

int32_t diag_device(int32_t device) {
    int ndev = 0;
    CS_HIP(hipGetDeviceCount(&ndev));
    if (device < 0 || device >= ndev) return fail(CS_ERR_HIP, "HIP device %d not available (%d visible)", device, ndev);
    return CS_OK;
}

int32_t diag_read_split(const _Float16* d_split, size_t rows, size_t N, float* out) {
    std::vector<_Float16> hs(rows * N * 2);
    CS_HIP(hipMemcpy(hs.data(), d_split, rows * N * 4, hipMemcpyDeviceToHost));
    const size_t nch = N / 32;
    for (size_t m = 0; m < rows; ++m)
        for (size_t n = 0; n < N; ++n) {
            const _Float16* line = hs.data() + (m * nch + n / 32) * 64;
            out[m * N + n] = (float)line[n % 32] + (float)line[32 + n % 32] * (1.0f / 2048.0f);
        }
    return CS_OK;
}

}

extern "C" {

int32_t cs_debug_rows(int32_t device, int32_t which, uint32_t H, uint32_t T, uint32_t L, uint32_t B, float eps, int32_t pooling,
                      const int32_t* ids, const float* word, const float* pos, const float* type_table, const int32_t* types,
                      uint32_t ntypes, uint32_t vocab, const float* x, const int32_t* mask, const float* parts, uint32_t nparts,
                      const float* bias, const float* gamma, const float* beta, int32_t range_mode, float* out, float* out_split,
                      float* src_after, float* range_out, uint32_t* range_flag) {
    if (which < 0 || which > 4) return fail(CS_ERR_BAD_ARG, "cs_debug_rows: which = %d (0 embeddings, 1 LayerNorm, 2 pooling, 3 slab sum, 4 LayerNorm of a source)", which);
    if (!out || H == 0) return fail(CS_ERR_BAD_ARG, "cs_debug_rows: null output or H = 0");
    if (which == 2) {
        if (!x || !mask || B == 0 || L == 0) return fail(CS_ERR_BAD_ARG, "cs_debug_rows: pooling needs x, mask, B > 0 and L > 0");
        if (pooling != CS_POOL_CLS && pooling != CS_POOL_MEAN) return fail(CS_ERR_BAD_ARG, "cs_debug_rows: unknown pooling %d", pooling);
        if (out_split || src_after || range_mode) return fail(CS_ERR_BAD_ARG, "cs_debug_rows: pooling writes f32 rows only");
        T = B * L;
    } else {
        if (T == 0 || !gamma || !beta) return fail(CS_ERR_BAD_ARG, "cs_debug_rows: needs T > 0, gamma and beta");
        if (which == 0 && (!ids || !word || !type_table || vocab == 0 || ntypes == 0 || L == 0))
            return fail(CS_ERR_BAD_ARG, "cs_debug_rows: the embedding kernel needs ids, the word and type tables, vocab, ntypes and L > 0");
        if (which != 0 && !x) return fail(CS_ERR_BAD_ARG, "cs_debug_rows: null input rows");
        if (which == 3 && (!parts || !bias || nparts == 0)) return fail(CS_ERR_BAD_ARG, "cs_debug_rows: the slab sum needs parts, bias and nparts > 0");
        if (range_mode < 0 || range_mode > 2 || (range_mode != 0) != (range_out != nullptr))
            return fail(CS_ERR_BAD_ARG, "cs_debug_rows: range_mode (1 per block, 2 per row) and range_out go together");
        if (range_mode && which != 0 && which != 1) return fail(CS_ERR_BAD_ARG, "cs_debug_rows: only kernels 0 and 1 report ranges");
        if (src_after && which != 4) return fail(CS_ERR_BAD_ARG, "cs_debug_rows: src_after belongs to kernel 4");
    }
    if ((uint64_t)T * H > (1ull << 28)) return fail(CS_ERR_UNSUPPORTED, "cs_debug_rows: T * H <= 2^28");
    CS_TRY(diag_device(device));
    DeviceGuard g(device);
    DiagBufs bufs;
    const size_t row_n = (size_t)T * H;
    EncoderLaunch a;
    float *dX = nullptr, *dSrc = nullptr, *dOut = nullptr, *dRange = nullptr;
    _Float16* dXs = nullptr;
    uint32_t* dF = nullptr;
    CS_TRY(bufs.get(&dF, 4));
    CS_HIP(hipMemset(dF, 0, 4));
    a.flag = dF;
    a.eps = eps;
    a.T = T; a.L = L; a.B = B;
    if (which == 2) {
        int32_t* dM = nullptr;
        CS_TRY(bufs.get(&dX, row_n * 4, x));
        CS_TRY(bufs.get(&dM, (size_t)T * 4, mask));
        CS_TRY(bufs.get(&dOut, (size_t)B * H * 4));
        CS_HIP(hipMemset(dOut, 0xff, (size_t)B * H * 4));
        a.x = dX; a.mask = dM; a.out = dOut; a.pooling = pooling;
        CS_TRY(launch_row_kernel(2, a, H, nullptr));
        CS_HIP(hipDeviceSynchronize());
        CS_HIP(hipMemcpy(out, dOut, (size_t)B * H * 4, hipMemcpyDeviceToHost));
        if (range_flag) CS_HIP(hipMemcpy(range_flag, dF, 4, hipMemcpyDeviceToHost));
        return CS_OK;
    }
    float *dG = nullptr, *dB = nullptr;
    CS_TRY(bufs.get(&dG, (size_t)H * 4, gamma));
    CS_TRY(bufs.get(&dB, (size_t)H * 4, beta));
    a.g = dG; a.b = dB;
    if (which == 0) {
        int32_t *dIds = nullptr, *dTypes = nullptr;
        float *dWord = nullptr, *dPos = nullptr, *dType = nullptr;
        CS_TRY(bufs.get(&dIds, (size_t)T * 4, ids));
        CS_TRY(bufs.get(&dWord, (size_t)vocab * H * 4, word));
        CS_TRY(bufs.get(&dType, (size_t)ntypes * H * 4, type_table));
        if (pos) CS_TRY(bufs.get(&dPos, (size_t)L * H * 4, pos));
        if (types) CS_TRY(bufs.get(&dTypes, (size_t)T * 4, types));
        CS_TRY(bufs.get(&dX, row_n * 4));
        CS_HIP(hipMemset(dX, 0xff, row_n * 4));
        a.ids = dIds; a.word = dWord; a.pos = dPos; a.type0 = dType; a.types = dTypes; a.ntypes = ntypes; a.vocab = vocab;
    } else if (which == 4) {
        CS_TRY(bufs.get(&dSrc, row_n * 4, x));
        CS_TRY(bufs.get(&dX, row_n * 4));
        CS_HIP(hipMemset(dX, 0xff, row_n * 4));
        a.src = dSrc;
    } else {
        CS_TRY(bufs.get(&dX, row_n * 4, x));
        if (which == 3) {
            float *dParts = nullptr, *dBias = nullptr;
            CS_TRY(bufs.get(&dParts, (size_t)nparts * row_n * 4, parts));
            CS_TRY(bufs.get(&dBias, (size_t)H * 4, bias));
            a.parts = dParts; a.nparts = nparts; a.bias = dBias;
        }
    }
    a.x = dX;
    if (out_split) {
        if (H % 32) return fail(CS_ERR_UNSUPPORTED, "cs_debug_rows: the split form needs H %% 32 == 0");
        CS_TRY(bufs.get(&dXs, row_n * 4));
        CS_HIP(hipMemset(dXs, 0xff, row_n * 4));
        a.xs = dXs;
    }
    const size_t range_pairs = range_mode == 2 ? T : (T + 3) / 4;
    if (range_mode) {
        CS_TRY(bufs.get(&dRange, range_pairs * 8));
        CS_HIP(hipMemset(dRange, 0xff, range_pairs * 8));
        a.range_out = dRange;
        a.range_rows = range_mode == 2;
    }
    CS_TRY(launch_row_kernel(which, a, H, nullptr));
    CS_HIP(hipDeviceSynchronize());
    CS_HIP(hipMemcpy(out, dX, row_n * 4, hipMemcpyDeviceToHost));
    if (out_split) CS_TRY(diag_read_split(dXs, T, H, out_split));
    if (src_after) CS_HIP(hipMemcpy(src_after, dSrc, row_n * 4, hipMemcpyDeviceToHost));
    if (range_mode) CS_HIP(hipMemcpy(range_out, dRange, range_pairs * 8, hipMemcpyDeviceToHost));
    if (range_flag) CS_HIP(hipMemcpy(range_flag, dF, 4, hipMemcpyDeviceToHost));
    return CS_OK;
}

int32_t cs_debug_elementwise(int32_t device, int32_t op, int32_t split, uint32_t T, uint32_t L, uint32_t H, uint32_t heads,
                             uint32_t I, int32_t gelu_gate, float eps, const float* a, const float* b, const float* table,
                             float* out, uint32_t* flags) {
    if (op < 0 || op > 2) return fail(CS_ERR_BAD_ARG, "cs_debug_elementwise: op = %d (0 rotary map, 1 gate, 2 query / key LayerNorm)", op);
// ... 303 lines not shown
```

codesearch_amd/csrc/embedder_forward.hip:

```cpp
#include "embedder_state.hpp"

using namespace cs;

namespace cs {
namespace emb {

size_t mid_width(const cs_bert_config& c) { return (size_t)c.intermediate * (cs_arch_gated(c.arch) ? 3 : 1); }

void free_workspace(cs_embedder* h) {
    if (h->d_ids) (void)hipFree(h->d_ids);
    if (h->d_mask) (void)hipFree(h->d_mask);
    if (h->d_types) (void)hipFree(h->d_types);
    if (h->d_x) (void)hipFree(h->d_x);
    if (h->d_xs) (void)hipFree(h->d_xs);
    if (h->d_qkv) (void)hipFree(h->d_qkv);
    if (h->d_ctx) (void)hipFree(h->d_ctx);
    if (h->d_mid) (void)hipFree(h->d_mid);
    if (h->d_pooled) (void)hipFree(h->d_pooled);
    if (h->d_perm) (void)hipFree(h->d_perm);
    if (h->d_rmeta) (void)hipFree(h->d_rmeta);
    if (h->d_rmeta2) (void)hipFree(h->d_rmeta2);
    if (h->d_range_pairs) (void)hipFree(h->d_range_pairs);
    if (h->d_seq_unit) (void)hipFree(h->d_seq_unit);
    if (h->d_unit_len) (void)hipFree(h->d_unit_len);
    if (h->d_row_slot) (void)hipFree(h->d_row_slot);
    if (h->d_range) (void)hipFree(h->d_range);
    h->d_rmeta = h->d_rmeta2 = nullptr;
    h->d_range_pairs = nullptr;
    h->d_seq_unit = h->d_unit_len = h->d_row_slot = h->d_range = nullptr;
    h->d_perm = nullptr;
    h->d_ids = h->d_mask = h->d_types = nullptr;
    h->cap_types = 0;
    h->d_x = h->d_xs = h->d_qkv = h->d_ctx = h->d_mid = h->d_pooled = nullptr;
    h->cap_tokens = h->cap_seqs = 0;
}

int32_t reserve(cs_embedder* h, size_t seqs, size_t tokens) {
    if (tokens <= h->cap_tokens && seqs <= h->cap_seqs) return CS_OK;
    free_workspace(h);
    const size_t H = h->cfg.hidden, I = h->cfg.intermediate;
    CS_HIP(hipMalloc(&h->d_ids, tokens * sizeof(int32_t)));
    CS_HIP(hipMalloc(&h->d_mask, tokens * sizeof(int32_t)));
    CS_HIP(hipMalloc(&h->d_x, tokens * H * sizeof(float)));
    CS_HIP(hipMalloc(&h->d_xs, tokens * H * sizeof(float)));
    CS_HIP(hipMalloc(&h->d_qkv, tokens * 3 * H * sizeof(float)));
    CS_HIP(hipMalloc(&h->d_ctx, tokens * H * sizeof(float)));
    CS_HIP(hipMalloc(&h->d_mid, tokens * mid_width(h->cfg) * sizeof(float)));
    CS_HIP(hipMalloc(&h->d_pooled, seqs * H * sizeof(float)));
    CS_HIP(hipMalloc(&h->d_perm, seqs * sizeof(uint32_t)));
    if (h->quantized) {
        CS_HIP(hipMalloc(&h->d_rmeta, tokens * sizeof(Q8RowMeta)));
        CS_HIP(hipMalloc(&h->d_rmeta2, tokens * sizeof(Q8RowMeta)));
        h->cap_range_pairs = std::max<size_t>(tokens + 1, (size_t)h->cfg.heads * 4 * (tokens / 128 + seqs));
        h->cap_range_pairs2 = (size_t)(I / 16) * (tokens / 16 + 1);
        CS_HIP(hipMalloc(&h->d_range_pairs, (h->cap_range_pairs + h->cap_range_pairs2) * 2 * sizeof(float)));
        CS_HIP(hipMalloc(&h->d_seq_unit, seqs * sizeof(uint32_t)));
        CS_HIP(hipMalloc(&h->d_unit_len, seqs * sizeof(uint32_t)));
        CS_HIP(hipMalloc(&h->d_row_slot, tokens * sizeof(uint32_t)));
        h->q8_units = (uint32_t)seqs;
        CS_HIP(hipMalloc(&h->d_range, (size_t)h->cfg.layers * 4 * Q8_RANGE_WORDS * h->q8_units * sizeof(uint32_t)));
    }
    h->cap_tokens = tokens;
    h->cap_seqs = seqs;
    return CS_OK;
}

SplitLayer split_layer(const cs_bert_config& c) {
    const size_t H = c.hidden, I = c.intermediate;
    SplitLayer o;
    o.qkv = 0;
    o.ao = o.qkv + 3 * H * H * 2;
    o.up = o.ao + H * H * 2;
    o.down = o.up + (cs_arch_gated(c.arch) ? 2 : 1) * I * H * 2;
    o.total = o.down + H * I * 2;
    return o;
}

}

static ForwardKnobs forward_knobs_from_env() {
    ForwardKnobs kn;
    auto on = [](const char* e) { return !(e && e[0] == '0'); };
    if (const char* e = cs_lab_env("CS_GEMM_SPLITK_MIN_M")) kn.split_k_min = (uint32_t)std::atoi(e);
    if (const char* e = cs_lab_env("CS_GEMM_SPLITK_MAX_M")) kn.split_k_max = (uint32_t)std::atoi(e);
    if (const char* e = cs_lab_env("CS_GEMM_SPLITK_MAX2_M")) kn.split_k_max2 = (uint32_t)std::atoi(e);
    if (const char* e = cs_lab_env("CS_GEMM_SPLITK_AO_MAX_M")) kn.split_k_ao_max = (uint32_t)std::atoi(e);
    if (const char* e = cs_lab_env("CS_GEMM_WIDE_MIN_M")) kn.wide_min_m = (uint32_t)std::atoll(e);
    kn.mid192 = on(cs_lab_env("CS_GEMM_WIDE_MID"));
    kn.ln_fuse = on(cs_lab_env("CS_GEMM_WIDE_LN"));
    kn.split_resid = on(cs_lab_env("CS_GEMM_WIDE_LN_SPLIT_RESID"));
    kn.gate_fused = on(cs_lab_env("CS_NOMIC_GATE_FUSED"));
    kn.q8_rows_units = on(cs_lab_env("CS_Q8_ROWS_UNITS"));
    if (const char* e = cs_lab_env("CS_Q8_LN_SLOT")) kn.q8_ln_slot = e[0] == '1';
    if (const char* e = cs_lab_env("CS_Q8_ROWS")) kn.q8_rows_min_m = std::atoi(e);
    kn.q8_rows_src = on(cs_lab_env("CS_Q8_ROWS_SRC"));
    if (const char* e = cs_lab_env("CS_Q8_SKINNY_MAX_M")) kn.q8_skinny_max_m = (uint32_t)std::atoll(e);
    kn.cls_tail = on(std::getenv("CS_ENCODER_CLS_TAIL"));
    if (const char* e = std::getenv("CS_ENCODER_CLS_TAIL_MIN_TOKENS")) kn.cls_tail_min_tokens = (uint32_t)std::atoll(e);
    if (const char* e = cs_lab_env("CS_ENCODER_STREAM_MIN_TOKENS")) kn.stream_min_tokens = (uint64_t)std::atoll(e);
    return kn;
}
const ForwardKnobs& forward_knobs() {
    static const ForwardKnobs kn = forward_knobs_from_env();
    return kn;
}

namespace emb {
namespace {

ForwardToggles forward_toggles_from_env() {
    ForwardToggles tg;
    auto on = [](const char* e) { return !(e && e[0] == '0'); };
    tg.small_path = on(std::getenv("CS_SMALL_PATH"));
    tg.small_fuse = on(std::getenv("CS_SMALL_FUSE"));
    tg.q8_skinny_ln = on(std::getenv("CS_Q8_SKINNY_LN"));
    tg.q8_ln_fused = on(cs_lab_env("CS_Q8_LN_FUSED"));
    if (const char* e = cs_lab_env("CS_SMALL_FORWARD")) tg.small_forward = e[0] == '1';
    return tg;
}

ForwardShape shape_of(const cs_embedder* h, uint32_t b0, uint32_t nb, uint32_t L, int mode) {
    const cs_bert_config& c = h->cfg;
    ForwardShape s;
    s.arch = c.arch; s.hidden = c.hidden; s.intermediate = c.intermediate; s.heads = c.heads; s.layers = c.layers;
    s.pooling = c.pooling; s.mode = mode;
    s.nb = nb; s.L = L; s.b0 = b0; s.units = h->cur_units;
    s.streams_in_flight = h->streams_in_flight; s.n_streams = h->n_streams; s.streams_forced = h->streams_forced;
    s.wide_ok = h->wide_ok;
    s.cap_range_pairs = h->cap_range_pairs; s.cap_range_pairs2 = h->cap_range_pairs2;
    s.stage_profile = h->stage_profile;
    s.cus = h->cus;
    return s;
}

struct Q8LayerArgs {
    Q8Layer ql;
    const int8_t *wq, *wst;
    const Q8ColMeta* cm;
    const uint32_t* cmt;
    uint32_t U, ln_pairs;
    uint32_t* rg;
    size_t rstep;
    const uint32_t* rs;
    int8_t* xq;
    Q8RowMeta* rm;
    float* rp;
};

struct Slice {
    cs_embedder* h;
    const cs_bert_config& cfg;
    hipStream_t s;
    uint32_t b0, nb, L, T, H, I;
    int mode;
    size_t t0;
    const float* P;
    float *x, *qkv, *ctx, *mid;
    const int32_t* mask;
    _Float16 *xs, *qkvs, *ctxs, *mids;
    SplitLayer sl;
    EncoderLaunch a;
    cs_bert_layer_offsets lo;
    const float* bqkv;

    Slice(cs_embedder* h_, hipStream_t s_, uint32_t b0_, uint32_t nb_, uint32_t L_, int mode_, const ForwardPlan& p)
        : h(h_), cfg(h_->cfg), s(s_), b0(b0_), nb(nb_), L(L_), T(nb_ * L_), H(cfg.hidden), I(cfg.intermediate), mode(mode_),
          t0((size_t)b0_ * L_), P(h_->d_params), sl(split_layer(cfg)) {
        x = h->d_x + t0 * H;
        qkv = h->d_qkv + t0 * 3 * H;
        ctx = h->d_ctx + t0 * H;
        mid = h->d_mid + t0 * mid_width(cfg);
        mask = h->d_mask + t0;
        xs = reinterpret_cast<_Float16*>(h->d_xs + t0 * H);
        qkvs = reinterpret_cast<_Float16*>(qkv);
        ctxs = reinterpret_cast<_Float16*>(ctx);
        mids = reinterpret_cast<_Float16*>(mid);
        a.ids = h->d_ids + t0; a.mask = mask;
        a.word = P + h->off.word; a.pos = cs_arch_gated(cfg.arch) ? nullptr : P + h->off.pos; a.type0 = P + h->off.type;
        a.types = h->types_on ? h->d_types + t0 : nullptr; a.ntypes = cfg.type_vocab_size;
        a.g = P + h->off.emb_ln_g; a.b = P + h->off.emb_ln_b;
        a.eps = cfg.layer_norm_eps; a.T = T; a.L = L; a.B = nb; a.vocab = cfg.vocab_size;
        a.pooling = cfg.pooling; a.x = x; a.out = (h->pooled_dst ? h->pooled_dst : h->d_pooled) + (size_t)b0 * out_width(h);
        a.xs = mode == CS_GEMM_SPLIT_F16 ? (void*)(h->d_xs + t0 * H) : nullptr;
        a.flag = h->d_flag;
        if (mode == CS_GEMM_Q8_DYNAMIC) a.range_out = h->d_range_pairs;
        a.range_rows = p.multi_unit;
    }

    int32_t mark(int tag) const {
        if (!h->stage_profile) return CS_OK;
        const size_t i = h->stage_tag.size() + 1;
        while (h->stage_ev.size() <= i) {
            hipEvent_t e;
            CS_HIP(hipEventCreate(&e));
            h->stage_ev.push_back(e);
        }
        if (tag < 0) { CS_HIP(hipEventRecord(h->stage_ev[0], s)); return CS_OK; }
        CS_HIP(hipEventRecord(h->stage_ev[i], s));
        h->stage_tag.push_back(tag);
        return CS_OK;
    }
    int32_t dense(DenseKernel k, int epi, const _Float16* Ain, const _Float16* Wt, const float* bias, const float* resid, float* Cf,
                  _Float16* Csp, uint32_t Mr, uint32_t Nn, uint32_t Kk) const {
        if (k == DenseKernel::Wide384) return launch_gemm_wide(epi, Ain, Wt, bias, resid, Cf, Csp, Mr, Nn, Kk, h->d_flag, s);
        if (k == DenseKernel::Wide192) return launch_gemm_wide(epi, Ain, Wt, bias, resid, Cf, Csp, Mr, Nn, Kk, h->d_flag, s, 192);
        return launch_gemm_split(epi, Ain, Wt, bias, resid, Cf, Csp, Mr, Nn, Kk, h->d_flag, s);
    }
    int32_t embed() const {
        CS_TRY(mark(-1));
        CS_TRY(launch_row_kernel(0, a, H, s));
        return mark(CS_STAGE_EMBED_LN);
    }
    int32_t layer_norm(uint64_t g, uint64_t b) {
        a.g = P + g; a.b = P + b;
        return launch_row_kernel(1, a, H, s);
    }
    int32_t out_stage(const EncoderLaunch& e) const {
        if (h->head_on) return launch_rerank_head(e.x, (size_t)e.L * H, h->d_head, e.B, H, e.out, s);
        return launch_row_kernel(2, e, H, s);
    }
    int32_t pool() const {
        CS_TRY(out_stage(a));
        return mark(CS_STAGE_POOL);
    }
    void layer_begin(uint32_t l) {
        cs_bert_layer_layout(&cfg, &h->off, l, &lo);
        bqkv = h->d_bqkv + (size_t)l * 3 * H;
    }
    Q8LayerArgs q8_layer_begin(uint32_t l);
    int32_t run_modern(const ForwardPlan& p);
    int32_t run_small(const ForwardPlan& p);
    int32_t run_q8_few_rows(const ForwardPlan& p);
    int32_t run_q8_rows_source(const ForwardPlan& p);
    int32_t run_q8_multi_unit();
    int32_t run_q8_quantise();
    int32_t run_cls_tail(const ForwardPlan& p, const _Float16* ws);
    int32_t run_split(const ForwardPlan& p);
    int32_t run_f32();
};

int32_t Slice::run_modern(const ForwardPlan& p) {
    const bool split = mode == CS_GEMM_SPLIT_F16;
    if (a.types) return fail(CS_ERR_UNSUPPORTED, "the ModernBERT encoder has no token-type table: token-type ids cannot be given");
    a.pos = nullptr; a.type0 = h->d_zero_row;
    CS_TRY(embed());
    EncoderLaunch n = a;
    n.src = x; n.x = ctx;
    for (uint32_t l = 0; l < cfg.layers; ++l) {
        layer_begin(l);
        const bool global = cfg.global_every == 0 || l % cfg.global_every == 0;
        const float2* rope = global ? h->d_rope : h->d_rope_local;
        const uint32_t window = global ? 0u : cfg.local_window;
        if (l) {
            n.g = P + lo.ao_ln_g; n.b = P + lo.ao_ln_b;
            CS_TRY(launch_row_kernel(4, n, H, s));
        }
        if (split) {
            const _Float16* ws = h->d_wsplit + (size_t)l * sl.total;
            CS_TRY(dense(p.qkv, SH_OUT_SPLIT, xs, ws + sl.qkv, bqkv, nullptr, nullptr, qkvs, T, 3 * H, H));
            CS_TRY(launch_rope_split(qkvs, rope, T, L, H, cfg.heads, h->d_flag, s));
            CS_TRY(mark(CS_STAGE_QKV));
            CS_TRY(launch_attention_sh2(qkvs, mask, ctxs, h->d_flag, nb, L, H, cfg.heads, s, nullptr, nullptr, nullptr, nullptr, nullptr, window));
            CS_TRY(mark(CS_STAGE_ATTENTION));
            CS_TRY(dense(p.ao, SH_OUT_F32_RESID, ctxs, ws + sl.ao, P + lo.ao_b, x, x, nullptr, T, H, H));
            CS_TRY(mark(CS_STAGE_OUT_PROJ));
            n.g = P + lo.out_ln_g; n.b = P + lo.out_ln_b;
            CS_TRY(launch_row_kernel(4, n, H, s));
            CS_TRY(mark(CS_STAGE_LN_ATTN));
            _Float16* gated = reinterpret_cast<_Float16*>(mid + (size_t)T * 2 * I);
            const float* bup = h->d_bup + (size_t)l * 2 * I;
            if (p.gate_epilogue) {
                CS_TRY(launch_gemm_wide(GW_OUT_GEGLU, xs, ws + sl.up, bup, nullptr, nullptr, gated, T, 2 * I, H, h->d_flag, s, p.up == DenseKernel::Wide192 ? 192 : 0));
            } else {
                CS_TRY(dense(p.up, SH_OUT_SPLIT, xs, ws + sl.up, bup, nullptr, nullptr, mids, T, 2 * I, H));
                CS_TRY(launch_swiglu_split(mids, gated, T, I, h->d_flag, s, true));
            }
            CS_TRY(mark(CS_STAGE_FFN_UP));
            CS_TRY(dense(p.down, SH_OUT_F32_RESID, gated, ws + sl.down, P + lo.down_b, x, x, nullptr, T, H, I));
            CS_TRY(mark(CS_STAGE_FFN_DOWN));
        } else {
            const float* nin = l ? ctx : x;
            const float* wqkv = h->d_wqkv + (size_t)l * 3 * H * H;
            CS_TRY(launch_gemm(GEMM_BIAS, nin, wqkv, bqkv, nullptr, qkv, T, 3 * H, H, s));
            CS_TRY(launch_rope_f32(qkv, rope, T, L, H, cfg.heads, s));
            CS_TRY(mark(CS_STAGE_QKV));
            CS_TRY(launch_attention(qkv, mask, ctx, nb, L, H, cfg.heads, s, nullptr, window));
            CS_TRY(mark(CS_STAGE_ATTENTION));
            CS_TRY(launch_gemm(GEMM_RESID, ctx, P + lo.ao_w, P + lo.ao_b, x, x, T, H, H, s));
            CS_TRY(mark(CS_STAGE_OUT_PROJ));
            n.g = P + lo.out_ln_g; n.b = P + lo.out_ln_b;
            CS_TRY(launch_row_kernel(4, n, H, s));
            CS_TRY(mark(CS_STAGE_LN_ATTN));
            float* gate = mid + (size_t)T * I;
            CS_TRY(launch_gemm(GEMM_BIAS, ctx, P + lo.up_w, P + lo.up_b, nullptr, mid, T, I, H, s));
            CS_TRY(launch_gemm(GEMM_BIAS, ctx, P + lo.gate_w, P + lo.gate_b, nullptr, gate, T, I, H, s));
            CS_TRY(launch_swiglu_f32(mid, gate, T, I, s, true));
            CS_TRY(mark(CS_STAGE_FFN_UP));
            CS_TRY(launch_gemm(GEMM_RESID, mid, P + lo.down_w, P + lo.down_b, x, x, T, H, I, s));
            CS_TRY(mark(CS_STAGE_FFN_DOWN));
        }
    }
    a.g = P + h->off.final_ln_g; a.b = P + h->off.final_ln_b; a.xs = nullptr;
    CS_TRY(launch_row_kernel(1, a, H, s));
    CS_TRY(mark(CS_STAGE_LN_FFN));
    h->last_hidden_partial = false;
    return pool();
}

int32_t Slice::run_small(const ForwardPlan& p) {
    if (!h->d_sp_ws) CS_HIP(hipMalloc(&h->d_sp_ws, (size_t)5 * SP_MAX_ROWS * H * sizeof(float)));
    float* parts = h->d_sp_ws;
    float* xa = h->d_sp_ws + (size_t)4 * SP_MAX_ROWS * H;
    float* y = h->d_xs + t0 * H;
#ifdef CS_DIAGNOSTICS
    if (p.path == ForwardPath::SmallOneLaunch) {
        uint32_t hb = L <= 32 ? 4u : (L <= 64 ? 2u : 1u);
        if (const char* ph = cs_lab_env("CS_ATTN_PACK_HEADS")) if (ph[0] == '0') hb = 1;
        while (cfg.heads % hb) hb >>= 1;
        SfArgs sa{};
        sa.ids = a.ids; sa.mask = mask; sa.word = a.word; sa.pos = a.pos; sa.type0 = a.type0; sa.types = a.types; sa.ntypes = a.ntypes; sa.emb_g = a.g; sa.emb_b = a.b;
        sa.layers = h->d_sf_layers; sa.n_layers = cfg.layers; sa.eps = cfg.layer_norm_eps;
        sa.T = T; sa.L = L; sa.B = nb; sa.vocab = cfg.vocab_size; sa.heads = cfg.heads; sa.hb = hb;
        sa.X = x; sa.XA = xa; sa.Y = y; sa.PARTS = parts; sa.QKVS = qkvs; sa.CTXS = ctxs;
        sa.MIDS = mids; sa.flag = h->d_flag; sa.sync = h->d_sf_sync;
        sa.dbg = h->d_sf_dbg;
        CS_HIP(hipMemsetAsync(h->d_sf_sync, 0, 16, s));
        CS_TRY(launch_small_forward(sa, s));
        h->sf_ran = true;
        h->last_hidden_partial = false;
        CS_TRY(out_stage(a));
        return CS_OK;
    }
#endif
    CS_TRY(mark(-1));
    for (uint32_t l = 0; l < cfg.layers; ++l) {
        cs_bert_layer_offsets lp;
        layer_begin(l);
        if (l) cs_bert_layer_layout(&cfg, &h->off, l - 1, &lp);
        const _Float16* ws = h->d_wsplit + (size_t)l * sl.total;
        SpLnGemmArgs g1{};
        g1.Y = y; g1.parts = parts; g1.parts_bias = l ? P + lp.down_b : nullptr; g1.X = x;
        g1.ids = a.ids; g1.word = a.word; g1.pos = a.pos; g1.type0 = a.type0; g1.types = a.types; g1.ntypes = a.ntypes; g1.L = L; g1.vocab = cfg.vocab_size;
        g1.ln_g = l ? P + lp.out_ln_g : a.g; g1.ln_b = l ? P + lp.out_ln_b : a.b; g1.eps = cfg.layer_norm_eps;
        g1.Xout = xa; g1.W = ws + sl.qkv; g1.bias = bqkv; g1.Cs = qkvs; g1.T = T; g1.N = 3 * H; g1.flag = h->d_flag;
        CS_TRY(launch_sp_ln_gemm(SH_OUT_SPLIT, l ? 1 : 2, g1, H, s));
        CS_TRY(mark(CS_STAGE_QKV));
        if (p.attn_proj_fused) {
            CS_TRY(mark(CS_STAGE_ATTENTION));
            CS_TRY(launch_sp_attn_proj(qkvs, mask, ws + sl.ao, P + lo.ao_b, xa, y, T, L, H, cfg.heads, h->d_flag, s));
        } else {
            CS_TRY(launch_attention_sh2(qkvs, mask, ctxs, h->d_flag, nb, L, H, cfg.heads, s));
            CS_TRY(mark(CS_STAGE_ATTENTION));
            CS_TRY(launch_gemm_split(SH_OUT_F32_RESID, ctxs, ws + sl.ao, P + lo.ao_b, xa, y, nullptr, T, H, H, h->d_flag, s));
        }
        CS_TRY(mark(CS_STAGE_OUT_PROJ));
        SpLnGemmArgs g4 = g1;
        g4.ln_g = P + lo.ao_ln_g; g4.ln_b = P + lo.ao_ln_b; g4.Xout = x; g4.W = ws + sl.up; g4.bias = P + lo.up_b; g4.Cs = mids; g4.N = I;
        CS_TRY(launch_sp_ln_gemm(SH_OUT_SPLIT_GELU, 0, g4, H, s));
        CS_TRY(mark(CS_STAGE_FFN_UP));
        CS_TRY(launch_sp_partial(mids, ws + sl.down, parts, T, H, H, s));
        CS_TRY(mark(CS_STAGE_FFN_DOWN));
    }
    cs_bert_layer_offsets ll;
    cs_bert_layer_layout(&cfg, &h->off, cfg.layers - 1, &ll);
    a.parts = parts; a.nparts = 4; a.bias = P + ll.down_b; a.g = P + ll.out_ln_g; a.b = P + ll.out_ln_b;
    a.xs = nullptr;
    CS_TRY(launch_row_kernel(3, a, H, s));
    CS_TRY(mark(CS_STAGE_LN_FFN));
    h->last_hidden_partial = false;
    return pool();
}

Q8LayerArgs Slice::q8_layer_begin(uint32_t l) {
    layer_begin(l);
    Q8LayerArgs q;
    q.ql = q8_layer(H, I);
    q.wq = h->d_wq8 + (size_t)l * q.ql.total;
    q.cm = h->d_cmeta + (size_t)l * (5 * (size_t)H + I);
    q.wst = h->d_wq8_stages ? h->d_wq8_stages + (size_t)l * ((size_t)H * H + (size_t)H * I) : nullptr;
    q.cmt = (H % 128 == 0 && I % 128 == 0) ? h->d_cmeta_tiles + (size_t)l * (5 * (size_t)H + I) * 4 : nullptr;
    q.U = h->cur_units;
    q.rg = h->d_range + (size_t)l * 4 * Q8_RANGE_WORDS * q.U;
    q.rstep = (size_t)Q8_RANGE_WORDS * q.U;
    q.rs = q.U > 1 ? h->d_row_slot : nullptr;
    q.xq = reinterpret_cast<int8_t*>(h->d_xs + t0 * H);
    q.rm = h->d_rmeta + t0;
    q.rp = h->d_range_pairs;
    q.ln_pairs = (T + 3) / 4;
    return q;
}

int32_t Slice::run_q8_few_rows(const ForwardPlan& p) {
    CS_TRY(embed());
    for (uint32_t l = 0; l < cfg.layers; ++l) {
        const Q8LayerArgs q = q8_layer_begin(l);
        float* rp2 = q.rp + 2 * h->cap_range_pairs;
        const bool fold = p.fold_ln;
        float* ybuf = h->d_xs + t0 * H;
        const bool last = l + 1 == cfg.layers;
        if (fold && l) {
            cs_bert_layer_offsets lp;
            cs_bert_layer_layout(&cfg, &h->off, l - 1, &lp);
            CS_TRY(launch_gemm_q8_skinny_ln(SH_OUT_SPLIT, ybuf, P + lp.out_ln_g, P + lp.out_ln_b, cfg.layer_norm_eps, x, q.wq + q.ql.qkv, q.cm, qkvs, T, 3 * H,
                                            h->d_flag, nullptr, nullptr, s));
        } else {
            CS_TRY(launch_gemm_q8_skinny(SH_OUT_SPLIT, Q8_SRC_F32, x, q.rp, q.ln_pairs, q.wq + q.ql.qkv, q.cm, nullptr, nullptr, qkvs, T, 3 * H, H, h->d_flag,
                                         nullptr, nullptr, s));
        }
        CS_TRY(mark(CS_STAGE_QKV));
        uint32_t att_pairs = 0, up_pairs = 0;
        CS_TRY(launch_attention_sh2(qkvs, mask, ctxs, h->d_flag, nb, L, H, cfg.heads, s, q.rp, &att_pairs));
        CS_TRY(mark(CS_STAGE_ATTENTION));
        if (!att_pairs) return fail(CS_ERR_UNSUPPORTED, "attention kernel without range pairs in the few-rows quantised path");
        CS_TRY(launch_gemm_q8_skinny(SH_OUT_F32_RESID, Q8_SRC_SPLIT, ctxs, q.rp, att_pairs, q.wq + q.ql.ao, q.cm + 3 * H, x, fold ? ybuf : x, nullptr, T, H, H,
                                     h->d_flag, nullptr, nullptr, s));
        CS_TRY(mark(CS_STAGE_OUT_PROJ));
        if (fold) {
            CS_TRY(mark(CS_STAGE_LN_ATTN));
            CS_TRY(launch_gemm_q8_skinny_ln(SH_OUT_SPLIT_GELU, ybuf, P + lo.ao_ln_g, P + lo.ao_ln_b, cfg.layer_norm_eps, x, q.wq + q.ql.up, q.cm + 4 * H, mids, T, I,
                                            h->d_flag, rp2, &up_pairs, s));
        } else {
            CS_TRY(layer_norm(lo.ao_ln_g, lo.ao_ln_b));
            CS_TRY(mark(CS_STAGE_LN_ATTN));
            CS_TRY(launch_gemm_q8_skinny(SH_OUT_SPLIT_GELU, Q8_SRC_F32, x, q.rp, q.ln_pairs, q.wq + q.ql.up, q.cm + 4 * H, nullptr, nullptr, mids, T, I, H,
                                         h->d_flag, rp2, &up_pairs, s));
        }
        CS_TRY(mark(CS_STAGE_FFN_UP));
        CS_TRY(launch_gemm_q8_skinny(SH_OUT_F32_RESID, Q8_SRC_SPLIT, mids, rp2, up_pairs, q.wq + q.ql.down, q.cm + 4 * H + I, x, fold && !last ? ybuf : x, nullptr,
                                     T, H, I, h->d_flag, nullptr, nullptr, s));
        CS_TRY(mark(CS_STAGE_FFN_DOWN));
        if (!fold || last) {
            CS_TRY(layer_norm(lo.out_ln_g, lo.out_ln_b));
        }
        CS_TRY(mark(CS_STAGE_LN_FFN));
        if (last) h->last_hidden_partial = false;
    }
    return pool();
}

int32_t Slice::run_q8_rows_source(const ForwardPlan& p) {
    CS_TRY(embed());
    for (uint32_t l = 0; l < cfg.layers; ++l) {
        const Q8LayerArgs q = q8_layer_begin(l);
        if (l == 0) h->q8_x_pairs = q.ln_pairs;
        if (h->q8_x_pairs) CS_TRY(launch_q8_range(Q8_SRC_F32, x, T, H, q.rg, s, q.rp, h->q8_x_pairs));
        CS_TRY(launch_gemm_q8_from_source(SH_OUT_SPLIT, Q8_SRC_F32, x, q.rg, q.wq + q.ql.qkv, q.cm, bqkv, nullptr, nullptr, qkvs, T, 3 * H, H, h->d_flag, s, nullptr, q.cmt,
                                          q.xq));
        CS_TRY(mark(CS_STAGE_QKV));
        uint32_t att_pairs = 0;
        CS_TRY(launch_attention_sh2(qkvs, mask, ctxs, h->d_flag, nb, L, H, cfg.heads, s, q.rp, &att_pairs));
        CS_TRY(mark(CS_STAGE_ATTENTION));
        CS_TRY(launch_q8_range(Q8_SRC_SPLIT, ctxs, T, H, q.rg + q.rstep, s, q.rp, att_pairs));
        if (p.ln_fused_ao) {
            CS_TRY(launch_gemm_q8_ln(Q8_SRC_SPLIT, ctxs, nullptr, q.rg + q.rstep, q.wst ? q.wst : q.wq + q.ql.ao, q.cm + 3 * H, x, P + lo.ao_ln_g, P + lo.ao_ln_b,
                                     cfg.layer_norm_eps, T, H, q.rp, &h->q8_x_pairs, s, p.ln_slot ? q.rg + 2 * q.rstep : nullptr, q.wst != nullptr));
            CS_TRY(mark(CS_STAGE_OUT_PROJ));
        } else {
            CS_TRY(launch_gemm_q8_from_source(SH_OUT_F32_RESID, Q8_SRC_SPLIT, ctxs, q.rg + q.rstep, q.wq + q.ql.ao, q.cm + 3 * H, P + lo.ao_b, x, x, nullptr, T, H, H,
                                              h->d_flag, s));
            CS_TRY(mark(CS_STAGE_OUT_PROJ));
            CS_TRY(layer_norm(lo.ao_ln_g, lo.ao_ln_b));
            h->q8_x_pairs = q.ln_pairs;
        }
        CS_TRY(mark(CS_STAGE_LN_ATTN));
        if (h->q8_x_pairs) CS_TRY(launch_q8_range(Q8_SRC_F32, x, T, H, q.rg + 2 * q.rstep, s, q.rp, h->q8_x_pairs));
        int8_t* midq = reinterpret_cast<int8_t*>(mid);
        Q8RowMeta* rm2 = h->d_rmeta2 + t0;
        CS_TRY(launch_gemm_q8_gelu_requant_from_source(x, q.rg + 2 * q.rstep, q.wq + q.ql.up, q.cm + 4 * H, P + lo.up_b, T, I, H, q.rg + 3 * q.rstep, midq, rm2, s, nullptr,
                                                       q.cmt ? q.cmt + 4 * 4 * H : nullptr, q.xq));
        CS_TRY(mark(CS_STAGE_FFN_UP));
        if (p.ln_fused_down) {
            CS_TRY(launch_gemm_q8_ln(Q8_SRC_PREQUANT, midq, rm2, nullptr, q.wst ? q.wst + (size_t)H * H : q.wq + q.ql.down, q.cm + 4 * H + I, x, P + lo.out_ln_g, P + lo.out_ln_b,
                                     cfg.layer_norm_eps, T, I, q.rp, &h->q8_x_pairs, s, p.ln_slot && l + 1 < cfg.layers ? q.rg + 4 * q.rstep : nullptr, q.wst != nullptr));
            CS_TRY(mark(CS_STAGE_FFN_DOWN));
        } else {
            CS_TRY(launch_gemm_q8(SH_OUT_F32_RESID, midq, rm2, q.wq + q.ql.down, q.cm + 4 * H + I, P + lo.down_b, x, x, nullptr, T, H, I, h->d_flag, s));
            CS_TRY(mark(CS_STAGE_FFN_DOWN));
            CS_TRY(layer_norm(lo.out_ln_g, lo.out_ln_b));
            h->q8_x_pairs = q.ln_pairs;
        }
        CS_TRY(mark(CS_STAGE_LN_FFN));
        if (l + 1 == cfg.layers) h->last_hidden_partial = false;
    }
    return pool();
}

int32_t Slice::run_q8_multi_unit() {
    CS_TRY(embed());
    for (uint32_t l = 0; l < cfg.layers; ++l) {
        const Q8LayerArgs q = q8_layer_begin(l);
        if (q.rs && l == 0) CS_TRY(launch_q8_row_slots(h->d_seq_unit, h->d_unit_len, T, L, h->d_row_slot, s));
        const uint32_t* su = h->d_seq_unit + b0;
        CS_TRY(launch_q8_range_units(q.rp, L, true, su, h->d_unit_len, nb, q.U, q.rg, s));
        CS_TRY(launch_gemm_q8_from_source(SH_OUT_SPLIT, Q8_SRC_F32, x, q.rg, q.wq + q.ql.qkv, q.cm, bqkv, nullptr, nullptr, qkvs, T, 3 * H, H, h->d_flag, s, q.rs));
        CS_TRY(mark(CS_STAGE_QKV));
        uint32_t att_pairs = 0;
        CS_TRY(launch_attention_sh2(qkvs, mask, ctxs, h->d_flag, nb, L, H, cfg.heads, s, q.rp, &att_pairs, su, h->d_unit_len));
        CS_TRY(mark(CS_STAGE_ATTENTION));
        if (!att_pairs || att_pairs > h->cap_range_pairs)
            return fail(CS_ERR_HIP, "attention range pairs (%u) do not fit the pair buffer (%zu)", att_pairs, h->cap_range_pairs);
        CS_TRY(launch_q8_range_units(q.rp, att_pairs / nb, false, su, h->d_unit_len, nb, q.U, q.rg + q.rstep, s));
        CS_TRY(launch_gemm_q8_from_source(SH_OUT_F32_RESID, Q8_SRC_SPLIT, ctxs, q.rg + q.rstep, q.wq + q.ql.ao, q.cm + 3 * H, P + lo.ao_b, x, x, nullptr, T, H, H,
                                          h->d_flag, s, q.rs));
        CS_TRY(mark(CS_STAGE_OUT_PROJ));
        CS_TRY(layer_norm(lo.ao_ln_g, lo.ao_ln_b));
        CS_TRY(mark(CS_STAGE_LN_ATTN));
        CS_TRY(launch_q8_range_units(q.rp, L, true, su, h->d_unit_len, nb, q.U, q.rg + 2 * q.rstep, s));
        int8_t* midq = reinterpret_cast<int8_t*>(mid);
        Q8RowMeta* rm2 = h->d_rmeta2 + t0;
        CS_TRY(launch_gemm_q8_gelu_requant_from_source(x, q.rg + 2 * q.rstep, q.wq + q.ql.up, q.cm + 4 * H, P + lo.up_b, T, I, H, q.rg + 3 * q.rstep, midq, rm2, s, q.rs));
        CS_TRY(mark(CS_STAGE_FFN_UP));
        CS_TRY(launch_gemm_q8(SH_OUT_F32_RESID, midq, rm2, q.wq + q.ql.down, q.cm + 4 * H + I, P + lo.down_b, x, x, nullptr, T, H, I, h->d_flag, s));
        CS_TRY(mark(CS_STAGE_FFN_DOWN));
        CS_TRY(layer_norm(lo.out_ln_g, lo.out_ln_b));
        CS_TRY(mark(CS_STAGE_LN_FFN));
        if (l + 1 == cfg.layers) h->last_hidden_partial = false;
    }
    return pool();
}

int32_t Slice::run_q8_quantise() {
    CS_TRY(embed());
    for (uint32_t l = 0; l < cfg.layers; ++l) {
        const Q8LayerArgs q = q8_layer_begin(l);
        if (q.rs && l == 0) CS_TRY(launch_q8_row_slots(h->d_seq_unit, h->d_unit_len, T, L, h->d_row_slot, s));
        CS_TRY(launch_q8_quantize(Q8_SRC_F32, x, T, H, q.rg, q.rs, q.xq, q.rm, s, q.rp, q.ln_pairs));
        CS_TRY(launch_gemm_q8(SH_OUT_SPLIT, q.xq, q.rm, q.wq + q.ql.qkv, q.cm, bqkv, nullptr, nullptr, qkvs, T, 3 * H, H, h->d_flag, s));
        CS_TRY(mark(CS_STAGE_QKV));
        uint32_t att_pairs = 0;
        CS_TRY(launch_attention_sh2(qkvs, mask, ctxs, h->d_flag, nb, L, H, cfg.heads, s, q.rp, &att_pairs));
        if (att_pairs > h->cap_range_pairs) return fail(CS_ERR_HIP, "range pair buffer too small (%u > %zu)", att_pairs, h->cap_range_pairs);
        CS_TRY(mark(CS_STAGE_ATTENTION));
        CS_TRY(launch_q8_quantize(Q8_SRC_SPLIT, ctxs, T, H, q.rg + q.rstep, q.rs, q.xq, q.rm, s, q.rp, att_pairs));
        CS_TRY(launch_gemm_q8(SH_OUT_F32_RESID, q.xq, q.rm, q.wq + q.ql.ao, q.cm + 3 * H, P + lo.ao_b, x, x, nullptr, T, H, H, h->d_flag, s));
        CS_TRY(mark(CS_STAGE_OUT_PROJ));
        CS_TRY(layer_norm(lo.ao_ln_g, lo.ao_ln_b));
        CS_TRY(mark(CS_STAGE_LN_ATTN));
        CS_TRY(launch_q8_quantize(Q8_SRC_F32, x, T, H, q.rg + 2 * q.rstep, q.rs, q.xq, q.rm, s, q.rp, q.ln_pairs));
        int8_t* midq = reinterpret_cast<int8_t*>(mid);
        Q8RowMeta* rm2 = h->d_rmeta2 + t0;
        if (q.rs) {
            CS_TRY(launch_gemm_q8(SH_OUT_SPLIT_GELU, q.xq, q.rm, q.wq + q.ql.up, q.cm + 4 * H, P + lo.up_b, nullptr, nullptr, mids, T, I, H, h->d_flag, s));
            CS_TRY(mark(CS_STAGE_FFN_UP));
            CS_TRY(launch_q8_quantize(Q8_SRC_SPLIT, mids, T, I, q.rg + 3 * q.rstep, q.rs, q.xq, q.rm, s));
            midq = q.xq;
            rm2 = q.rm;
        } else {
            CS_TRY(launch_gemm_q8_gelu_requant(q.xq, q.rm, q.wq + q.ql.up, q.cm + 4 * H, P + lo.up_b, T, I, H, q.rg + 3 * q.rstep, midq, rm2, s));
            CS_TRY(mark(CS_STAGE_FFN_UP));
        }
        CS_TRY(launch_gemm_q8(SH_OUT_F32_RESID, midq, rm2, q.wq + q.ql.down, q.cm + 4 * H + I, P + lo.down_b, x, x, nullptr, T, H, I, h->d_flag, s));
        CS_TRY(mark(CS_STAGE_FFN_DOWN));
        CS_TRY(layer_norm(lo.out_ln_g, lo.out_ln_b));
        CS_TRY(mark(CS_STAGE_LN_FFN));
        if (l + 1 == cfg.layers) h->last_hidden_partial = false;
    }
    return pool();
}

int32_t Slice::run_cls_tail(const ForwardPlan& p, const _Float16* ws) {
    h->last_hidden_partial = true;
    float* x_cls = mid;
    _Float16* xs_cls = reinterpret_cast<_Float16*>(mid + (size_t)nb * H);
    _Float16* ctxs_cls = reinterpret_cast<_Float16*>(mid + (size_t)2 * nb * H);
    _Float16* q_cls = reinterpret_cast<_Float16*>(mid + (size_t)3 * nb * H);
    _Float16* mids_cls = reinterpret_cast<_Float16*>(mid + (size_t)4 * nb * H);
    CS_TRY(dense(p.kv_tail, SH_OUT_SPLIT, xs, ws + sl.qkv + (size_t)H * H * 2, bqkv + H, nullptr, nullptr, qkvs, T, 2 * H, H));
    CS_TRY(launch_gather_cls(xs, x_cls, xs_cls, nb, L, H, s));
    CS_TRY(launch_gemm_split(SH_OUT_SPLIT, xs_cls, ws + sl.qkv, bqkv, nullptr, nullptr, q_cls, nb, H, H, h->d_flag, s));
    CS_TRY(mark(CS_STAGE_QKV));
    CS_TRY(launch_attention_cls(q_cls, qkvs, mask, ctxs_cls, h->d_flag, nb, L, H, cfg.heads, s));
    CS_TRY(mark(CS_STAGE_ATTENTION));
    EncoderLaunch t = a;
    t.x = x_cls; t.xs = xs_cls; t.T = nb; t.L = 1; t.B = nb;
    CS_TRY(launch_gemm_split(SH_OUT_F32_RESID, ctxs_cls, ws + sl.ao, P + lo.ao_b, x_cls, x_cls, nullptr, nb, H, H, h->d_flag, s));
    CS_TRY(mark(CS_STAGE_OUT_PROJ));
    t.g = P + lo.ao_ln_g; t.b = P + lo.ao_ln_b;
    CS_TRY(launch_row_kernel(1, t, H, s));
    CS_TRY(mark(CS_STAGE_LN_ATTN));
    CS_TRY(launch_gemm_split(SH_OUT_SPLIT_GELU, xs_cls, ws + sl.up, P + lo.up_b, nullptr, nullptr, mids_cls, nb, I, H, h->d_flag, s));
    CS_TRY(mark(CS_STAGE_FFN_UP));
    CS_TRY(launch_gemm_split(SH_OUT_F32_RESID, mids_cls, ws + sl.down, P + lo.down_b, x_cls, x_cls, nullptr, nb, H, I, h->d_flag, s));
    CS_TRY(mark(CS_STAGE_FFN_DOWN));
    t.g = P + lo.out_ln_g; t.b = P + lo.out_ln_b;
    CS_TRY(launch_row_kernel(1, t, H, s));
    CS_TRY(mark(CS_STAGE_LN_FFN));
    CS_TRY(out_stage(t));
    return mark(CS_STAGE_POOL);
}

int32_t Slice::run_split(const ForwardPlan& p) {
    const bool nomic = cs_arch_gated(cfg.arch), rotary = cfg.arch == CS_ARCH_NOMIC, jina = cs_arch_alibi(cfg.arch);
    const bool qknorm = cfg.arch == CS_ARCH_JINA_QKNORM;
    const float* alibi = jina ? h->d_alibi : nullptr;
    CS_TRY(embed());
    for (uint32_t l = 0; l < cfg.layers; ++l) {
        layer_begin(l);
        const _Float16* ws = h->d_wsplit + (size_t)l * sl.total;
        if (l + 1 == cfg.layers) h->last_hidden_partial = false;
        if (p.cls_tail && l + 1 == cfg.layers) return run_cls_tail(p, ws);
        CS_TRY(dense(p.qkv, SH_OUT_SPLIT, xs, ws + sl.qkv, bqkv, nullptr, nullptr, qkvs, T, 3 * H, H));
        if (rotary) CS_TRY(launch_rope_split(qkvs, h->d_rope, T, L, H, cfg.heads, h->d_flag, s));
        if (qknorm) CS_TRY(launch_qk_layernorm_split(qkvs, P + lo.qln_g, cfg.layer_norm_eps, T, H, h->d_flag, s));
        CS_TRY(mark(CS_STAGE_QKV));
        CS_TRY(launch_attention_sh2(qkvs, mask, ctxs, h->d_flag, nb, L, H, cfg.heads, s, nullptr, nullptr, nullptr, nullptr, alibi));
        CS_TRY(mark(CS_STAGE_ATTENTION));
        a.g = P + lo.ao_ln_g; a.b = P + lo.ao_ln_b;
        if (p.fuse_ln) {
            CS_TRY(launch_gemm_wide_ln(ctxs, ws + sl.ao, P + lo.ao_b, x, a.g, a.b, cfg.layer_norm_eps,
                                       p.split_resid ? nullptr : x, xs, T, H, h->d_flag, s, p.split_resid ? xs : nullptr));
            CS_TRY(mark(CS_STAGE_OUT_PROJ));
        } else if (p.ao_slices) {
            CS_TRY(launch_gemm_split_partial(ctxs, ws + sl.ao, qkv, T, H, H, p.ao_slices, s));
            CS_TRY(mark(CS_STAGE_OUT_PROJ));
            a.parts = qkv; a.nparts = p.ao_slices; a.bias = P + lo.ao_b;
            CS_TRY(launch_row_kernel(3, a, H, s));
        } else {
            CS_TRY(dense(p.ao, SH_OUT_F32_RESID, ctxs, ws + sl.ao, P + lo.ao_b, x, x, nullptr, T, H, H));
            CS_TRY(mark(CS_STAGE_OUT_PROJ));
            CS_TRY(launch_row_kernel(1, a, H, s));
        }
        CS_TRY(mark(CS_STAGE_LN_ATTN));
        a.g = P + lo.out_ln_g; a.b = P + lo.out_ln_b;
        const _Float16* ffn_in = mids;
        if (nomic) {
            _Float16* gated = reinterpret_cast<_Float16*>(mid + (size_t)T * 2 * I);
            const float* bup = h->d_bup + (size_t)l * 2 * I;
            if (p.gate_epilogue) {
                CS_TRY(launch_gemm_wide(jina ? GW_OUT_GEGLU : GW_OUT_SWIGLU, xs, ws + sl.up, bup, nullptr, nullptr, gated, T, 2 * I, H, h->d_flag, s, p.up == DenseKernel::Wide192 ? 192 : 0));
            } else {
                CS_TRY(dense(p.up, SH_OUT_SPLIT, xs, ws + sl.up, bup, nullptr, nullptr, mids, T, 2 * I, H));
                CS_TRY(launch_swiglu_split(mids, gated, T, I, h->d_flag, s, jina));
            }
            ffn_in = gated;
        } else {
            CS_TRY(dense(p.up, SH_OUT_SPLIT_GELU, xs, ws + sl.up, P + lo.up_b, nullptr, nullptr, mids, T, I, H));
        }
        CS_TRY(mark(CS_STAGE_FFN_UP));
        if (p.fuse_ln) {
            CS_TRY(launch_gemm_wide_ln(ffn_in, ws + sl.down, P + lo.down_b, x, a.g, a.b, cfg.layer_norm_eps,
                                       (p.split_resid && l + 1 < cfg.layers) ? nullptr : x, xs, T, I, h->d_flag, s,
                                       p.split_resid ? xs : nullptr));
            CS_TRY(mark(CS_STAGE_FFN_DOWN));
        } else if (p.down_slices) {
            CS_TRY(launch_gemm_split_partial(ffn_in, ws + sl.down, qkv, T, H, I, p.down_slices, s));
            CS_TRY(mark(CS_STAGE_FFN_DOWN));
            a.parts = qkv; a.nparts = p.down_slices; a.bias = P + lo.down_b;
            CS_TRY(launch_row_kernel(3, a, H, s));
        } else {
            CS_TRY(dense(p.down, SH_OUT_F32_RESID, ffn_in, ws + sl.down, P + lo.down_b, x, x, nullptr, T, H, I));
            CS_TRY(mark(CS_STAGE_FFN_DOWN));
            CS_TRY(launch_row_kernel(1, a, H, s));
        }
        CS_TRY(mark(CS_STAGE_LN_FFN));
    }
    return pool();
}

int32_t Slice::run_f32() {
    const bool nomic = cs_arch_gated(cfg.arch), rotary = cfg.arch == CS_ARCH_NOMIC, jina = cs_arch_alibi(cfg.arch);
    const bool qknorm = cfg.arch == CS_ARCH_JINA_QKNORM;
    const float* alibi = jina ? h->d_alibi : nullptr;
    CS_TRY(embed());
    for (uint32_t l = 0; l < cfg.layers; ++l) {
        layer_begin(l);
        const float* wqkv = h->d_wqkv + (size_t)l * 3 * H * H;
        CS_TRY(launch_gemm(GEMM_BIAS, x, wqkv, bqkv, nullptr, qkv, T, 3 * H, H, s));
        if (rotary) CS_TRY(launch_rope_f32(qkv, h->d_rope, T, L, H, cfg.heads, s));
        if (qknorm) CS_TRY(launch_qk_layernorm_f32(qkv, P + lo.qln_g, cfg.layer_norm_eps, T, H, s));
        CS_TRY(mark(CS_STAGE_QKV));
        CS_TRY(launch_attention(qkv, mask, ctx, nb, L, H, cfg.heads, s, alibi));
        CS_TRY(mark(CS_STAGE_ATTENTION));
        CS_TRY(launch_gemm(GEMM_RESID, ctx, P + lo.ao_w, P + lo.ao_b, x, x, T, H, H, s));
        CS_TRY(mark(CS_STAGE_OUT_PROJ));
        CS_TRY(layer_norm(lo.ao_ln_g, lo.ao_ln_b));
        CS_TRY(mark(CS_STAGE_LN_ATTN));
        if (nomic) {
            float* gate = mid + (size_t)T * I;
            CS_TRY(launch_gemm(GEMM_BIAS, x, P + lo.up_w, P + lo.up_b, nullptr, mid, T, I, H, s));
            CS_TRY(launch_gemm(GEMM_BIAS, x, P + lo.gate_w, P + lo.gate_b, nullptr, gate, T, I, H, s));
            CS_TRY(launch_swiglu_f32(mid, gate, T, I, s, jina));
        } else {
            CS_TRY(launch_gemm(GEMM_GELU, x, P + lo.up_w, P + lo.up_b, nullptr, mid, T, I, H, s));
        }
        CS_TRY(mark(CS_STAGE_FFN_UP));
        CS_TRY(launch_gemm(GEMM_RESID, mid, P + lo.down_w, P + lo.down_b, x, x, T, H, I, s));
        CS_TRY(mark(CS_STAGE_FFN_DOWN));
        CS_TRY(layer_norm(lo.out_ln_g, lo.out_ln_b));
        CS_TRY(mark(CS_STAGE_LN_FFN));
    }
    return pool();
}

int32_t forward_range(cs_embedder* h, hipStream_t s, const ForwardToggles& tg, uint32_t b0, uint32_t nb, uint32_t L, int mode) {
    ForwardShape shape = shape_of(h, b0, nb, L, mode);
#ifdef CS_DIAGNOSTICS
    if (tg.small_forward)
        shape.small_forward_ok = h->d_sf_layers && !h->sf_off && small_forward_supported(h->cfg.hidden, h->cfg.intermediate, h->cfg.heads, nb * L, L);
#endif
    const ForwardPlan p = plan_forward(forward_knobs(), tg, shape);
    if (p.path == ForwardPath::Refused) return fail(CS_ERR_UNSUPPORTED, "the dynamic-quantisation mode is not built for the ModernBERT encoder");
    Slice c(h, s, b0, nb, L, mode, p);
    if (p.path == ForwardPath::Modern) return c.run_modern(p);
    h->sf_ran = false;
    switch (p.path) {
        case ForwardPath::Small:
        case ForwardPath::SmallOneLaunch: return c.run_small(p);
        case ForwardPath::Q8FewRows: return c.run_q8_few_rows(p);
        case ForwardPath::Q8RowsSource: return c.run_q8_rows_source(p);
        case ForwardPath::Q8MultiUnit: return c.run_q8_multi_unit();
        case ForwardPath::Q8Quantise: return c.run_q8_quantise();
        case ForwardPath::Split: return c.run_split(p);
        default: return c.run_f32();
    }
}

}

int32_t forward(cs_embedder* h, uint32_t B, uint32_t L, int mode) {
    hipStream_t s = h->stream;
    CS_HIP(hipEventRecord(h->ev0, s));
    if (mode != CS_GEMM_F32) CS_HIP(hipMemsetAsync(h->d_flag, 0, sizeof(uint32_t), s));
    if (mode == CS_GEMM_Q8_DYNAMIC)
        CS_HIP(hipMemsetAsync(h->d_range, 0, (size_t)h->cfg.layers * 4 * Q8_RANGE_WORDS * h->cur_units * sizeof(uint32_t), s));
    h->stage_tag.clear();
    const ForwardToggles tg = forward_toggles_from_env();
    const uint32_t ns = plan_streams(forward_knobs(), shape_of(h, 0, B, L, mode));
    h->streams_in_flight = (int)ns;
    if (ns >= 2) {
        hipStream_t st[4] = {s, h->stream2, h->xstreams[0], h->xstreams[1]};
        hipEvent_t jn[4] = {nullptr, h->ev_join, h->xjoin[0], h->xjoin[1]};
        CS_HIP(hipEventRecord(h->ev_fork, s));
        for (uint32_t i = ns; i-- > 0;) {
            const uint32_t lo = (uint32_t)((uint64_t)B * i / ns), hi = (uint32_t)((uint64_t)B * (i + 1) / ns);
            if (i) CS_HIP(hipStreamWaitEvent(st[i], h->ev_fork, 0));
            CS_TRY(forward_range(h, st[i], tg, lo, hi - lo, L, mode));
            if (i) CS_HIP(hipEventRecord(jn[i], st[i]));
        }
        for (uint32_t i = 1; i < ns; ++i) CS_HIP(hipStreamWaitEvent(s, jn[i], 0));
    } else {
        CS_TRY(forward_range(h, s, tg, 0, B, L, mode));
    }
    CS_HIP(hipEventRecord(h->ev1, s));
    h->last_B = B;
    h->last_L = L;
    return CS_OK;
}
}
}
```

codesearch_amd/csrc/embedder_state.hpp:

```cpp
#pragma once

#include <algorithm>
#include <cstdlib>
#include <cstring>
#include <map>
#include <memory>
#include <mutex>
#include <thread>
#include <vector>

#include "encoder.hpp"
#include "small_forward.hpp"
#include "small_path.hpp"
#include "split_f16.hpp"
#include "gemm_q8.hpp"

using namespace cs;

struct QueuePool {
    std::mutex mu;
    std::vector<std::pair<float*, size_t>> free_bufs;
    std::vector<std::pair<float*, size_t>> free_host;
    int device = 0;
    ~QueuePool() {
        cs::DeviceGuard g(device);
        for (auto& b : free_bufs) (void)hipFree(b.first);
        for (auto& b : free_host) (void)hipHostFree(b.first);
    }
};
struct QueueFlush {
    std::shared_ptr<QueuePool> pool;
    float* d_rows = nullptr;
    size_t cap = 0;
    size_t used = 0;
    std::mutex hmu;
    float* h_rows = nullptr;
    size_t h_cap = 0;
    bool host_ready = false;
    ~QueueFlush() {
        std::lock_guard<std::mutex> lk(pool->mu);
        if (d_rows) pool->free_bufs.emplace_back(d_rows, cap);
        if (h_rows) pool->free_host.emplace_back(h_rows, h_cap);
    }
};
struct QueueEntry {
    uint64_t ticket = 0;
    std::vector<std::vector<int32_t>> ids;
    std::vector<std::vector<int32_t>> mask;
    enum { QUEUED, COMPUTING, DONE, FAILED } state = QUEUED;
    std::shared_ptr<QueueFlush> flush;
    uint64_t first_row = 0;
    int32_t error = 0;
    std::string error_text;
};

struct cs_embedder {
    std::mutex qmu;
    std::mutex cmu;
    std::map<uint64_t, std::shared_ptr<QueueEntry>> queue;
    std::shared_ptr<QueuePool> qpool;
    uint64_t next_ticket = 1;
    int device = 0;
    int cus = 0;
    cs_bert_config cfg{};
    cs_bert_offsets off{};
    float* d_params = nullptr;
    float* d_wqkv = nullptr;
    float* d_bqkv = nullptr;
    float* d_bup = nullptr;
    float2* d_rope = nullptr;
    float2* d_rope_local = nullptr;
    float* d_zero_row = nullptr;
    float* d_alibi = nullptr;
    _Float16* d_wsplit = nullptr;
    uint32_t* d_flag = nullptr;
    SfLayer* d_sf_layers = nullptr;
    uint32_t* d_sf_sync = nullptr;
    uint64_t* d_sf_dbg = nullptr;
    float* d_sp_ws = nullptr;
    bool sf_ran = false, sf_off = false;
    uint64_t sf_forwards = 0, sf_fallbacks = 0;
    bool quantized = false;
    int8_t* d_wq8 = nullptr;
    Q8ColMeta* d_cmeta = nullptr;
    int8_t* d_wq8_stages = nullptr;
    uint32_t* d_cmeta_tiles = nullptr;
    uint32_t* d_range = nullptr;
    uint32_t q8_units = 1;
    Q8RowMeta* d_rmeta = nullptr;
    Q8RowMeta* d_rmeta2 = nullptr;
    float* d_range_pairs = nullptr;
    size_t cap_range_pairs = 0, cap_range_pairs2 = 0;
    uint32_t* d_seq_unit = nullptr;
    uint32_t* d_unit_len = nullptr;
    uint32_t* d_row_slot = nullptr;
    uint32_t cur_units = 1;
    uint32_t q8_x_pairs = 0;
    int gemm_mode = CS_GEMM_SPLIT_F16;
    bool split_unavailable = false;
    bool wide_ok = false;
    int streams_in_flight = 1;
    uint64_t split_forwards = 0, f32_forwards = 0, range_fallbacks = 0, q8_forwards = 0;
    hipStream_t stream = nullptr;
    hipStream_t stream2 = nullptr;
    hipEvent_t ev_fork = nullptr, ev_join = nullptr;
    hipStream_t xstreams[2] = {nullptr, nullptr};
    hipEvent_t xjoin[2] = {nullptr, nullptr};
    int n_streams = 2;
    bool streams_forced = false;
    size_t cap_tokens = 0, cap_seqs = 0;
    int32_t* d_ids = nullptr;
    int32_t* d_mask = nullptr;
    int32_t* d_types = nullptr;
    size_t cap_types = 0;
    bool types_on = false;
    const float* d_head = nullptr;
    bool head_on = false;
    float* d_x = nullptr;
    float* d_xs = nullptr;
    float* d_qkv = nullptr;
    float* d_ctx = nullptr;
    float* d_mid = nullptr;
    float* d_pooled = nullptr;
    float* pooled_dst = nullptr;
    uint32_t* d_perm = nullptr;
    std::vector<float> h_pooled;
    char* h_pin = nullptr;
    uint32_t last_B = 0, last_L = 0;
    bool last_hidden_partial = false;
    hipEvent_t ev0 = nullptr, ev1 = nullptr;
    double forward_ms = 0.0;
    uint64_t forwards = 0;
    bool stage_profile = false;
    std::vector<hipEvent_t> stage_ev;
    std::vector<int> stage_tag;
    double stage_us[CS_ENCODER_STAGES] = {};
    uint64_t stage_forwards = 0;
};

namespace cs {
namespace emb {

size_t mid_width(const cs_bert_config& c);
void free_workspace(cs_embedder* h);
int32_t reserve(cs_embedder* h, size_t seqs, size_t tokens);
struct SplitLayer { size_t qkv, ao, up, down, total; };
SplitLayer split_layer(const cs_bert_config& c);
int32_t forward(cs_embedder* h, uint32_t B, uint32_t L, int mode);
uint32_t default_batch(const cs_embedder* h);
inline uint32_t out_width(const cs_embedder* h) { return h->head_on ? 1u : h->cfg.hidden; }

struct UnitSpec {
    const uint32_t* seq_unit = nullptr;
    const uint32_t* unit_len = nullptr;
    uint32_t units = 1;
};
int32_t embed_impl(cs_embedder* h, const int32_t* ids, const int32_t* mask, uint64_t n, uint32_t seq_len, uint32_t batch,
                   float* out, bool out_on_device, const volatile int32_t* cancel, const uint32_t* perm = nullptr,
                   const UnitSpec* units = nullptr, const int32_t* types = nullptr);
int32_t embed_texts_impl(cs_embedder* h, const cs_tokenizer* t, const char* utf8, const uint64_t* offsets,
                         uint64_t n, uint32_t batch, float* out, bool out_on_device, const volatile int32_t* cancel);
int32_t embed_ids_entry(cs_embedder* h, const int32_t* ids, const int32_t* mask, uint64_t n, uint32_t seq_len,
                        uint32_t batch, float* out, bool out_on_device, const volatile int32_t* cancel,
                        const int32_t* types = nullptr);
struct SeqView { const int32_t* ids; const int32_t* mask; uint32_t len; const int32_t* types = nullptr; };
int32_t run_window(cs_embedder* h, const std::vector<SeqView>& seqs, uint32_t batch, int32_t pad, float* out,
                   bool out_on_device, const volatile int32_t* cancel, std::vector<uint32_t>& order,
                   std::vector<int32_t>& ids, std::vector<int32_t>& mask);

}
}
```

codesearch_amd/csrc/encoder.hpp:

```cpp
#pragma once

#include "common.hpp"
#include "forward_plan.hpp"

#include "../../include/cs_bert_params.h"

namespace cs {

struct EncoderLaunch {
    const int32_t* ids = nullptr;
    const int32_t* mask = nullptr;
    const float* word = nullptr;
    const float* pos = nullptr;
    const float* type0 = nullptr;
    const int32_t* types = nullptr;
    uint32_t ntypes = 1;
    const float* g = nullptr;
    const float* b = nullptr;
    float eps = 1e-12f;
    uint32_t T = 0, L = 0, B = 0, vocab = 0;
    int pooling = CS_POOL_CLS;
    float* x = nullptr;
    float* out = nullptr;
    void* xs = nullptr;
    const float* parts = nullptr;
    const float* bias = nullptr;
    uint32_t nparts = 0;
    const float* src = nullptr;
    uint32_t* flag = nullptr;
    float* range_out = nullptr;
    bool range_rows = false;
};

enum { GEMM_BIAS = 0, GEMM_GELU = 1, GEMM_RESID = 2 };

int32_t launch_row_kernel(int which, const EncoderLaunch& a, uint32_t H, hipStream_t s);
int32_t launch_gemm(int epi, const float* A, const float* W, const float* bias, const float* resid,
                    float* C, uint32_t M, uint32_t N, uint32_t K, hipStream_t s);
int32_t launch_attention(const float* qkv, const int32_t* mask, float* ctx, uint32_t B, uint32_t L,
                         uint32_t H, uint32_t heads, hipStream_t s, const float* alibi = nullptr, uint32_t window = 0);
size_t attention_lds_bytes(uint32_t L);
int32_t launch_attention_sh2(const _Float16* qkv_split, const int32_t* mask, void* ctx_split, uint32_t* flag,
                             uint32_t B, uint32_t L, uint32_t H, uint32_t heads, hipStream_t s, float* range_out = nullptr,
                             uint32_t* range_pairs = nullptr, const uint32_t* seq_unit = nullptr,
                             const uint32_t* unit_len = nullptr, const float* alibi = nullptr, uint32_t window = 0);

enum { SH_OUT_F32 = 0, SH_OUT_F32_RESID = 1, SH_OUT_SPLIT_GELU = 2, SH_OUT_SPLIT = 3,
       SH_OUT_PARTIAL = 4  };
int32_t launch_gemm_split_partial(const _Float16* A, const _Float16* W, float* Cpart, uint32_t M, uint32_t N,
                                  uint32_t K, uint32_t ksplit, hipStream_t s);
int32_t launch_gemm_split(int epi, const _Float16* A, const _Float16* W, const float* bias, const float* resid,
                          float* C, _Float16* Cs, uint32_t M, uint32_t N, uint32_t K, uint32_t* d_flag,
                          hipStream_t s);
constexpr int GW_OUT_SWIGLU = 17;
constexpr int GW_OUT_GEGLU = 18;
int32_t launch_gemm_wide(int epi, const _Float16* A, const _Float16* W, const float* bias, const float* resid, float* C,
                         _Float16* Cs, uint32_t M, uint32_t N, uint32_t K, uint32_t* d_flag, hipStream_t s, int shape = 0);
int32_t launch_gemm_wide_ln(const _Float16* A, const _Float16* W, const float* bias, const float* resid, const float* gamma,
                            const float* beta, float eps, float* X, _Float16* Xs, uint32_t M, uint32_t K, uint32_t* d_flag,
                            hipStream_t s, const _Float16* resid_split = nullptr);
int32_t launch_attention_cls(const _Float16* q_cls, const _Float16* kv_split, const int32_t* mask, _Float16* ctxs_cls,
                             uint32_t* flag, uint32_t B, uint32_t L, uint32_t H, uint32_t heads, hipStream_t s);
int32_t launch_rerank_head(const float* x, size_t row_stride, const float* head, uint32_t B, uint32_t H, float* out, hipStream_t s);
int32_t launch_gather_cls(const _Float16* xs, float* x_cls, _Float16* xs_cls, uint32_t B, uint32_t L, uint32_t H, hipStream_t s);
int32_t launch_rope_split(_Float16* qkvs, const float2* rope, uint32_t T, uint32_t L, uint32_t H, uint32_t heads,
                          uint32_t* flag, hipStream_t s);
int32_t launch_rope_f32(float* qkv, const float2* rope, uint32_t T, uint32_t L, uint32_t H, uint32_t heads, hipStream_t s);
int32_t launch_swiglu_split(const _Float16* up2, _Float16* out, uint32_t T, uint32_t I, uint32_t* flag, hipStream_t s,
                            bool gelu_gate = false);
int32_t launch_swiglu_f32(float* value, const float* gate, uint32_t T, uint32_t I, hipStream_t s, bool gelu_gate = false);
int32_t launch_qk_layernorm_split(_Float16* qkvs, const float* ln, float eps, uint32_t T, uint32_t H, uint32_t* flag, hipStream_t s);
int32_t launch_qk_layernorm_f32(float* qkv, const float* ln, float eps, uint32_t T, uint32_t H, hipStream_t s);
#ifdef CS_DIAGNOSTICS
extern int g_gemm_wide_ablation;
extern int g_gemm_wide_shape;
extern int g_gemm_wide_mfma;
double gemm_wide_read_clock_ghz(double* main_cycles, double* epi_cycles);
#else
constexpr int g_gemm_wide_ablation = 0, g_gemm_wide_shape = 0, g_gemm_wide_mfma = 0;
#endif
const ForwardKnobs& forward_knobs();
int32_t sh_weights_fit_wide(const _Float16* d_wsplit, uint64_t n_f16, uint32_t* d_scratch_flag, bool* ok, hipStream_t s);
int32_t launch_synth_params(float* d_out, const cs_bert_config& cfg, uint64_t seed, hipStream_t s);

}
```

include/codesearch_gpu_diag.h:

```cpp
#ifndef CODESEARCH_GPU_DIAG_H
#define CODESEARCH_GPU_DIAG_H

#include "codesearch_gpu.h"

#ifdef __cplusplus
extern "C" {
#endif

CS_API int32_t cs_debug_gemm(int32_t device, int32_t mode, int32_t epilogue, const float* A,
                      const float* W, const float* bias, const float* resid, float* C,
                      uint32_t M, uint32_t N, uint32_t K, uint32_t* range_flag);

CS_API int32_t cs_debug_gemm_q8(int32_t device, int32_t epilogue, int32_t a_split, const float* A, const float* W,
                         const float* wscale, const float* bias, const float* resid, float* C, uint32_t M, uint32_t N,
                         uint32_t K, uint8_t* xq, float* xparams, int32_t* acc);

CS_API int32_t cs_debug_gemm_q8_units(int32_t device, int32_t epilogue, const float* A, const float* W, const float* wscale,
                               const float* bias, const float* resid, float* C, uint32_t M, uint32_t N, uint32_t K,
                               const uint32_t* row_slot, uint32_t units, float* row_params, int32_t* rowsums);

CS_API int32_t cs_debug_small_forward_counters(cs_embedder* h, uint64_t* forwards, uint64_t* fallbacks);

CS_API int32_t cs_debug_attention(int32_t device, const float* qkv, const int32_t* mask, uint32_t B, uint32_t L, uint32_t H,
                           uint32_t heads, const float* alibi_slopes, uint32_t window, const uint32_t* seq_unit,
                           const uint32_t* unit_len, uint32_t units, const float* proj_w, const float* proj_bias,
                           const float* proj_resid, float* out, float* range_pairs_out, uint32_t range_pairs_cap,
                           uint32_t* range_pairs, uint32_t* range_flag);

CS_API int32_t cs_debug_rows(int32_t device, int32_t which, uint32_t H, uint32_t T, uint32_t L, uint32_t B, float eps, int32_t pooling,
                      const int32_t* ids, const float* word, const float* pos, const float* type_table, const int32_t* types,
                      uint32_t ntypes, uint32_t vocab, const float* x, const int32_t* mask, const float* parts, uint32_t nparts,
                      const float* bias, const float* gamma, const float* beta, int32_t range_mode, float* out, float* out_split,
                      float* src_after, float* range_out, uint32_t* range_flag);

CS_API int32_t cs_debug_elementwise(int32_t device, int32_t op, int32_t split, uint32_t T, uint32_t L, uint32_t H, uint32_t heads,
                             uint32_t I, int32_t gelu_gate, float eps, const float* a, const float* b, const float* table,
                             float* out, uint32_t* flags);

CS_API int32_t cs_debug_attention_cls(int32_t device, const float* qkv, const int32_t* mask, uint32_t B, uint32_t L, uint32_t H,
                               uint32_t heads, float* out, uint32_t* flags, const float* gather_src, float* x_cls,
                               uint16_t* xs_cls);

CS_API int32_t cs_debug_attention_f32(int32_t device, const float* qkv, const int32_t* mask, uint32_t B, uint32_t L, uint32_t H,
                               uint32_t heads, const float* alibi_slopes, uint32_t window, float* out);

CS_API int32_t cs_debug_small_path(int32_t device, int32_t op, int32_t epi, int32_t pro, uint32_t H, uint32_t T, uint32_t N, uint32_t L,
                            float eps, const float* gamma, const float* beta, const float* rows, const float* parts,
                            const float* parts_bias, const float* x, const int32_t* ids, const float* word, const float* pos,
                            const float* type_table, const int32_t* types, uint32_t ntypes, uint32_t vocab, const float* W,
                            const float* bias, float* xout, float* cs_out, float* x_after, float* parts_out, uint32_t* flags,
                            uint32_t* guard_changed);

CS_API int32_t cs_debug_gemm_time(int32_t device, int32_t mode, int32_t epilogue, uint32_t M, uint32_t N, uint32_t K,
                           uint32_t iters, int32_t ablation, double* ms_per_launch);

#ifdef __cplusplus
}
#endif
#endif
```

Measured before the change: 4.638 billion.

## Precompute attention mask plan once per forward and ring-buffer key/value loads

Adds a per-batch mask-plan kernel, run once per forward, that writes the additive mask row and the live tile count. The attention kernel now copies these into LDS instead of rebuilding them with atomics in every block and layer. When planned and pipelined, a four-slot key/value ring issues buffer-to-LDS loads two tiles ahead, replacing the stage/sync/wait sequence per super-tile. Range min/max tracking is compiled out when no range output is needed. The ring adds barrier complexity and extra template instantiations, and the plan costs one extra kernel launch and buffer per forward.

Result: no change. 4.622 billion (-0.3%).

```diff
diff --git a/codesearch_amd/_lib.py b/codesearch_amd/_lib.py
--- a/codesearch_amd/_lib.py
+++ b/codesearch_amd/_lib.py
@@ -263,6 +263,8 @@
                                         C.c_uint32, f32p, f32p, f32p, f32p, f32p, f32p, u32p, u32p]),
     "cs_debug_attention": (C.c_int32, [C.c_int32, f32p, i32p, C.c_uint32, C.c_uint32, C.c_uint32, C.c_uint32, f32p, C.c_uint32,
                                        u32p, u32p, C.c_uint32, f32p, f32p, f32p, f32p, f32p, C.c_uint32, u32p, u32p]),
+    "cs_debug_attention_plan": (C.c_int32, [C.c_int32, f32p, i32p, C.c_uint32, C.c_uint32, C.c_uint32, C.c_uint32, f32p, C.c_uint32,
+                                            u32p, u32p, C.c_uint32, f32p, f32p, C.c_uint32, u32p, u32p]),
 }
 
 _LIB = None
diff --git a/codesearch_amd/csrc/attention_shx_body.hpp b/codesearch_amd/csrc/attention_shx_body.hpp
--- a/codesearch_amd/csrc/attention_shx_body.hpp
+++ b/codesearch_amd/csrc/attention_shx_body.hpp
@@ -68,17 +68,19 @@
     __device__ __forceinline__ void st8(_Float16* p, f16x4 v) const { *reinterpret_cast<f16x4*>(p) = v; }
 };
 
-template <int NC, class MQ, class MO, int POS = 0, int PIPE = 0>
+template <int NC, class MQ, class MO, int POS = 0, int PIPE = 0, bool PLAN = false, bool RANGE = true, bool RING = false>
 __device__ __forceinline__ void
 attention_shx_body(char* smem, const MQ& mq, const MO& mo, const _Float16* qkvs, const int32_t* __restrict__ mask,
                    _Float16* ctxs, uint32_t* __restrict__ flag, uint32_t L, uint32_t H,
                    float scale_log2e, uint32_t HB, float* __restrict__ range_out,
                    const uint32_t* __restrict__ seq_unit, const uint32_t* __restrict__ unit_len,
                    uint32_t bx, uint32_t by, uint32_t bz, uint32_t gx, uint32_t gz, const float* __restrict__ alibi_log2 = nullptr,
-                   uint32_t window = 0) {
+                   uint32_t window = 0, const float* __restrict__ madd_plan = nullptr,
+                   const uint32_t* __restrict__ ntiles_plan = nullptr) {
     constexpr bool ALIBI = POS == 1, WINDOW = POS == 2;
     constexpr bool IMM = PIPE >= 2;
     constexpr bool EARLY = PIPE == 3;
+    static_assert(!RING || (PIPE >= 2 && POS != 2), "the key ring is built for the written-out tile loop without a window");
     const float wlimit = (float)window;
     constexpr int KT = 128;
     const uint32_t Lp = (L + 31) & ~31u;
@@ -98,7 +100,7 @@
     bool ovf = false;
 
     AT_STAMP(0);
-    if (tid == 0) *last_valid_p = 0;
+    if constexpr (!PLAN) { if (tid == 0) *last_valid_p = 0; }
 
     const int kswz = (l31 >> 1) & 7;
     int k_hi[2], k_lo[2];
@@ -179,15 +181,29 @@
         }
     };
     stage(0);
-    __syncthreads();
-    for (uint32_t key = tid; key < Lp; key += 256) {
-        const bool ok = key < L && mask[(size_t)b * L + key] != 0;
-        madd[key] = ok ? 0.0f : kMaskedLog2;
-        if (ok) atomicMax(last_valid_p, (int)key);
-    }
-    asm volatile("s_waitcnt vmcnt(0)" ::: "memory");
-    __syncthreads();
-    const uint32_t ntiles = (uint32_t)(*last_valid_p) / 32 + 1;
+    uint32_t ntiles;
+    if constexpr (PLAN) {
+        const uint32_t stride = attn_plan_stride(L);
+        const _Float16* mrow = reinterpret_cast<const _Float16*>(madd_plan + (size_t)b * stride);
+        for (uint32_t pc = (uint32_t)wave; pc * 256 < stride; pc += 4) {
+            char* piece = reinterpret_cast<char*>(madd) + (size_t)pc * 1024;
+            const f16x8 r = mq.stage_load(mrow + (size_t)pc * 512 + lane * 8, piece);
+            mq.stage_store(piece, lane, r);
+        }
+        ntiles = ntiles_plan[b];
+        asm volatile("s_waitcnt vmcnt(0)" ::: "memory");
+        __syncthreads();
+    } else {
+        __syncthreads();
+        for (uint32_t key = tid; key < Lp; key += 256) {
+            const bool ok = key < L && mask[(size_t)b * L + key] != 0;
+            madd[key] = ok ? 0.0f : kMaskedLog2;
+            if (ok) atomicMax(last_valid_p, (int)key);
+        }
+        asm volatile("s_waitcnt vmcnt(0)" ::: "memory");
+        __syncthreads();
+        ntiles = (uint32_t)(*last_valid_p) / 32 + 1;
+    }
 
     typedef __attribute__((address_space(3))) char* lds_char_p;
     typedef __attribute__((address_space(3))) const f16x8* lds_f16x8_cp;
@@ -205,17 +221,44 @@
         asm volatile("" : "+v"(va[0]), "+v"(va[1]), "+v"(ma0));
     }
 
+    const sh_rsrc kv_rsrc = sh_make_rsrc(base, RING ? L * nch * 128u : 0u);
+    const uint32_t ring_row = qt * 8 + ((uint32_t)lane >> 3);
+    auto ring_request = [&](uint32_t r) __attribute__((always_inline)) {
+        const uint32_t gk = r * 32 + ring_row, key = gk < L ? gk : L - 1;
+        const uint32_t ck = (lane & 7) ^ ((ring_row >> 1) & 7), cv = (lane & 7) ^ (4 * ((ring_row >> 1) & 1));
+        const uint32_t piece = ((r & 3) * 4 + qt) * 1024;
+#pragma unroll
+        for (int c = 0; c < NC; ++c) {
+            sh_blds16(kv_rsrc, (key * nch + (nh + head) * NC + c) * 128 + ck * 16, 0, Kt + (size_t)c * KT * 128 + piece);
+            sh_blds16(kv_rsrc, (key * nch + (2 * nh + head) * NC + c) * 128 + cv * 16, 0, Vt + (size_t)c * KT * 128 + piece);
+        }
+    };
+    auto ring_top = [&](uint32_t t) __attribute__((always_inline)) {
+        const bool data = t >= 4, more = t + 2 < ntiles;
+        if (!data && !more) return;
+        __builtin_amdgcn_sched_barrier(0);
+        if (data) asm volatile("s_waitcnt vmcnt(0)" ::: "memory");
+        asm volatile("s_waitcnt lgkmcnt(0)\n\ts_barrier" ::: "memory");
+        if (more) {
+            ring_request(t + 2);
+            if (t + 3 < ntiles) ring_request(t + 3);
+        }
+        __builtin_amdgcn_sched_barrier(0);
+    };
+
     for (uint32_t st = 0; st * 4 < ntiles; ++st) {
         if constexpr (WINDOW) {
             if (st * KT > qb * 128 + 127 + window || st * KT + (KT - 1) + window < qb * 128) continue;
         }
-        if (st > 0) {
-            __syncthreads();
-            stage(st);
-            asm volatile("s_waitcnt vmcnt(0)" ::: "memory");
-            __syncthreads();
-        }
-        if (!wave_live) continue;
+        if constexpr (!RING) {
+            if (st > 0) {
+                __syncthreads();
+                stage(st);
+                asm volatile("s_waitcnt vmcnt(0)" ::: "memory");
+                __syncthreads();
+            }
+            if (!wave_live) continue;
+        }
         const uint32_t kt_end = ntiles - st * 4 < 4 ? ntiles - st * 4 : 4;
         const uint32_t ma_st = ma0 + st * 512u;
         uint32_t kl_lo = 0, kl_hi = kt_end;
@@ -450,7 +493,19 @@
                 }
             }
         };
-        if constexpr (PIPE == 0) {
+        if constexpr (RING) {
+#pragma unroll
+            for (uint32_t kl = 0; kl < 4; ++kl) {
+                if (kl < kt_end) {
+                    if (kl % 2 == 0 && (st > 0 || kl > 0)) ring_top(st * 4 + kl);
+                    if (wave_live) {
+                        sh_f32x16 hh, xx;
+                        compute_s(kl, hh, xx);
+                        finish_tile(kl, hh, xx);
+                    }
+                }
+            }
+        } else if constexpr (PIPE == 0) {
             for (uint32_t kl = kl_lo; kl < kl_hi; ++kl) {
                 sh_f32x16 hh, xx;
                 compute_s(kl, hh, xx);
@@ -496,8 +551,10 @@
                     const float o = fmaf(oxx[c][4 * g + e], kShLoInv, ohh[c][4 * g + e]) * inv;
                     ovf |= sh_split(o, a, bb);
                     hi[e] = a; lo[e] = bb;
-                    rlo = fminf(rlo, o);
-                    rhi = fmaxf(rhi, o);
+                    if constexpr (RANGE) {
+                        rlo = fminf(rlo, o);
+                        rhi = fmaxf(rhi, o);
+                    }
                 }
                 mo.st8(op + 8 * g, hi);
                 mo.st8(op + 32 + 8 * g, lo);
@@ -506,7 +563,7 @@
     }
     AT_STAMP(2);
     if (ovf && flag) atomicOr(flag, 1u);
-    if (range_out) {
+    if (RANGE && range_out) {
         if (unit_len && query >= unit_len[seq_unit[b]]) rlo = rhi = 0.0f;
 #pragma unroll
         for (int o = 32; o > 0; o >>= 1) {
diff --git a/codesearch_amd/csrc/attention_split.hip b/codesearch_amd/csrc/attention_split.hip
--- a/codesearch_amd/csrc/attention_split.hip
+++ b/codesearch_amd/csrc/attention_split.hip
@@ -167,18 +167,40 @@
 }
 #endif
 
-template <int NC, int POS = 0, int PIPE = 0>
+template <int NC, int POS = 0, int PIPE = 0, bool PLAN = false, bool RANGE = true>
 __global__ void __launch_bounds__(256, NC == 1 ? (PIPE == 1 ? CS_ATTN_PIPE_WAVES : (PIPE >= 2 ? 4 : 2)) : 2)
 attention_shx_kernel(const _Float16* __restrict__ qkvs, const int32_t* __restrict__ mask,
                      _Float16* __restrict__ ctxs, uint32_t* __restrict__ flag, uint32_t L, uint32_t H,
                      float scale_log2e, uint32_t HB, float* __restrict__ range_out,
                      const uint32_t* __restrict__ seq_unit, const uint32_t* __restrict__ unit_len,
-                     const float* __restrict__ alibi_log2, uint32_t window) {
+                     const float* __restrict__ alibi_log2, uint32_t window, const float* __restrict__ plan_madd,
+                     const uint32_t* __restrict__ plan_ntiles) {
     extern __shared__ __attribute__((aligned(16))) char smem[];
     const AttnMemPlain mem;
-    attention_shx_body<NC, AttnMemPlain, AttnMemPlain, POS, PIPE>(smem, mem, mem, qkvs, mask, ctxs, flag, L, H, scale_log2e, HB, range_out,
-                                                            seq_unit, unit_len, blockIdx.x, blockIdx.y, blockIdx.z, gridDim.x,
-                                                            gridDim.z, alibi_log2, window);
+    constexpr bool RING = PLAN && PIPE >= 2 && POS != 2;
+    attention_shx_body<NC, AttnMemPlain, AttnMemPlain, POS, PIPE, PLAN, RANGE, RING>(smem, mem, mem, qkvs, mask, ctxs, flag, L, H, scale_log2e, HB,
+                                                                           range_out, seq_unit, unit_len, blockIdx.x, blockIdx.y,
+                                                                           blockIdx.z, gridDim.x, gridDim.z, alibi_log2, window,
+                                                                           plan_madd, plan_ntiles);
+}
+
+__global__ void __launch_bounds__(256)
+attention_mask_plan_kernel(const int32_t* __restrict__ mask, float* __restrict__ plan_madd, uint32_t* __restrict__ plan_ntiles,
+                           uint32_t L) {
+    __shared__ int wave_last[4];
+    const uint32_t b = blockIdx.x, stride = attn_plan_stride(L);
+    int last = 0;
+    for (uint32_t key = threadIdx.x; key < stride; key += 256) {
+        const bool ok = key < L && mask[(size_t)b * L + key] != 0;
+        plan_madd[(size_t)b * stride + key] = ok ? 0.0f : kMaskedLog2;
+        if (ok) last = (int)key;
+    }
+#pragma unroll
+    for (int o = 32; o > 0; o >>= 1) last = max(last, __shfl_xor(last, o, 64));
+    if ((threadIdx.x & 63) == 0) wave_last[threadIdx.x >> 6] = last;
+    __syncthreads();
+    if (threadIdx.x == 0)
+        plan_ntiles[b] = (uint32_t)max(max(wave_last[0], wave_last[1]), max(wave_last[2], wave_last[3])) / 32 + 1;
 }
 
 namespace {
@@ -186,22 +208,36 @@
 struct ShxArgs {
     const _Float16* qkv; const int32_t* mask; _Float16* ctx; uint32_t* flag; uint32_t L, H; float scale_log2e; uint32_t hb;
     float* range_out; const uint32_t* seq_unit; const uint32_t* unit_len; const float* alibi_log2; uint32_t window;
+    const float* plan_madd; const uint32_t* plan_ntiles;
 };
 
-template <int NC, int POS, int PIPE>
+template <int NC, int POS, int PIPE, bool PLAN = false, bool RANGE = true>
 int32_t launch_shx_one(dim3 grid, size_t lds, hipStream_t s, const ShxArgs& a) {
     if (lds > 64 * 1024 - 256) {
         static PerDeviceOnce attr;
         CS_TRY(attr.run([&]() -> int32_t {
-            CS_HIP(hipFuncSetAttribute(reinterpret_cast<const void*>(attention_shx_kernel<NC, POS, PIPE>),
+            CS_HIP(hipFuncSetAttribute(reinterpret_cast<const void*>(attention_shx_kernel<NC, POS, PIPE, PLAN, RANGE>),
                                        hipFuncAttributeMaxDynamicSharedMemorySize, 160 * 1024 - 64));
             return CS_OK;
         }));
     }
-    hipLaunchKernelGGL((attention_shx_kernel<NC, POS, PIPE>), grid, dim3(256), lds, s, a.qkv, a.mask, a.ctx, a.flag, a.L, a.H,
-                       a.scale_log2e, a.hb, a.range_out, a.seq_unit, a.unit_len, a.alibi_log2, a.window);
+    hipLaunchKernelGGL((attention_shx_kernel<NC, POS, PIPE, PLAN, RANGE>), grid, dim3(256), lds, s, a.qkv, a.mask, a.ctx, a.flag, a.L, a.H,
+                       a.scale_log2e, a.hb, a.range_out, a.seq_unit, a.unit_len, a.alibi_log2, a.window, a.plan_madd, a.plan_ntiles);
     CS_HIP(hipGetLastError());
     return CS_OK;
+}
+
+template <int NC, int PIPE>
+int32_t launch_shx_form(int pos, dim3 grid, size_t lds, hipStream_t s, const ShxArgs& a) {
+    if (a.plan_madd) {
+        if (a.range_out) return launch_shx_one<NC, 0, PIPE, true, true>(grid, lds, s, a);
+        if (pos == 1) return launch_shx_one<NC, 1, PIPE, true, false>(grid, lds, s, a);
+        if (pos == 2) return launch_shx_one<NC, 2, PIPE, true, false>(grid, lds, s, a);
+        return launch_shx_one<NC, 0, PIPE, true, false>(grid, lds, s, a);
+    }
+    if (pos == 1) return launch_shx_one<NC, 1, PIPE>(grid, lds, s, a);
+    if (pos == 2) return launch_shx_one<NC, 2, PIPE>(grid, lds, s, a);
+    return launch_shx_one<NC, 0, PIPE>(grid, lds, s, a);
 }
 
 template <int NC>
@@ -209,37 +245,29 @@
 #ifndef CS_DIAGNOSTICS
     constexpr int P = NC == 1 ? kAttnPipeDefault32 : kAttnPipeDefault64;
     (void)pipe;
-    if (pos == 1) return launch_shx_one<NC, 1, P>(grid, lds, s, a);
-    if (pos == 2) return launch_shx_one<NC, 2, P>(grid, lds, s, a);
-    return launch_shx_one<NC, 0, P>(grid, lds, s, a);
+    return launch_shx_form<NC, P>(pos, grid, lds, s, a);
 #else
-    if (pipe == 3) {
-        if (pos == 1) return launch_shx_one<NC, 1, 3>(grid, lds, s, a);
-        if (pos == 2) return launch_shx_one<NC, 2, 3>(grid, lds, s, a);
-        return launch_shx_one<NC, 0, 3>(grid, lds, s, a);
-    }
-    if (pipe == 2) {
-        if (pos == 1) return launch_shx_one<NC, 1, 2>(grid, lds, s, a);
-        if (pos == 2) return launch_shx_one<NC, 2, 2>(grid, lds, s, a);
-        return launch_shx_one<NC, 0, 2>(grid, lds, s, a);
-    }
-    if (pipe == 1) {
-        if (pos == 1) return launch_shx_one<NC, 1, 1>(grid, lds, s, a);
-        if (pos == 2) return launch_shx_one<NC, 2, 1>(grid, lds, s, a);
-        return launch_shx_one<NC, 0, 1>(grid, lds, s, a);
-    }
-    if (pos == 1) return launch_shx_one<NC, 1, 0>(grid, lds, s, a);
-    if (pos == 2) return launch_shx_one<NC, 2, 0>(grid, lds, s, a);
-    return launch_shx_one<NC, 0, 0>(grid, lds, s, a);
-#endif
-}
-
+    if (pipe == 3) return launch_shx_form<NC, 3>(pos, grid, lds, s, a);
+    if (pipe == 2) return launch_shx_form<NC, 2>(pos, grid, lds, s, a);
+    if (pipe == 1) return launch_shx_form<NC, 1>(pos, grid, lds, s, a);
+    return launch_shx_form<NC, 0>(pos, grid, lds, s, a);
+#endif
+}
+
+}
+
+int32_t launch_attention_mask_plan(const int32_t* mask, float* plan_madd, uint32_t* plan_ntiles, uint32_t B, uint32_t L, hipStream_t s) {
+    if (!mask || !plan_madd || !plan_ntiles || B == 0 || L == 0) return fail(CS_ERR_BAD_ARG, "attention mask plan: null buffer or empty batch");
+    hipLaunchKernelGGL(attention_mask_plan_kernel, dim3(B), dim3(256), 0, s, mask, plan_madd, plan_ntiles, L);
+    CS_HIP(hipGetLastError());
+    return CS_OK;
 }
 
 int32_t launch_attention_sh2(const _Float16* qkv_split, const int32_t* mask, void* ctx_split, uint32_t* flag,
                              uint32_t B, uint32_t L, uint32_t H, uint32_t heads, hipStream_t s, float* range_out,
                              uint32_t* range_pairs, const uint32_t* seq_unit, const uint32_t* unit_len, const float* alibi,
-                             uint32_t window) {
+                             uint32_t window, const float* plan_madd, const uint32_t* plan_ntiles) {
+    if (!plan_madd != !plan_ntiles) return fail(CS_ERR_BAD_ARG, "attention: the mask plan's two buffers go together");
     if (alibi && window) return fail(CS_ERR_BAD_ARG, "attention: ALiBi and a local window together are not built");
     const float* alibi_log2 = alibi ? alibi + heads : nullptr;
     const int pos = alibi_log2 ? 1 : (window ? 2 : 0);
@@ -249,9 +277,12 @@
         return fail(CS_ERR_UNSUPPORTED, "head_dim %u not supported (32 or 64)", dh);
     const size_t Lp = (L + 31) & ~31u;
     static const int pipe_env = [] { const char* e = cs_lab_env("CS_ATTN_PIPE"); return e && e[0] >= '0' && e[0] <= '3' ? e[0] - '0' : -1; }();
-    ShxArgs a{qkv_split, mask, static_cast<_Float16*>(ctx_split), flag, L, H, 0.0f, 1u, range_out, seq_unit, unit_len, alibi_log2, window};
+    const bool plan = plan_madd && !(range_out && pos);
+    const size_t madd_bytes = (plan ? attn_plan_stride(L) : Lp) * sizeof(float);
+    ShxArgs a{qkv_split, mask, static_cast<_Float16*>(ctx_split), flag, L, H, 0.0f, 1u, range_out, seq_unit, unit_len, alibi_log2, window,
+              plan ? plan_madd : nullptr, plan ? plan_ntiles : nullptr};
     if (dh == 64) {
-        const size_t lds = 2 * 2 * 128 * 128 + Lp * sizeof(float) + 16;
+        const size_t lds = 2 * 2 * 128 * 128 + madd_bytes + 16;
         a.scale_log2e = (1.0f / sqrtf(64.0f)) * kLog2e;
         const int pipe = pipe_env < 0 ? kAttnPipeDefault64 : pipe_env;
         CS_TRY(launch_shx<2>(pos, pipe, dim3(heads, B, (L + 127) / 128), lds, s, a));
@@ -261,7 +292,7 @@
     static const bool shx1 = [] { const char* e = cs_lab_env("CS_ATTN_SHX1"); return !(e && e[0] == '0'); }();
     if (shx1 || pos) {
         static const size_t lds_pad = [] { const char* e = cs_lab_env("CS_ATTN_LDS_PAD"); return e ? (size_t)std::atol(e) : (size_t)0; }();
-        const size_t lds1 = 2 * 1 * 128 * 128 + Lp * sizeof(float) + 16 + lds_pad;
+        const size_t lds1 = 2 * 1 * 128 * 128 + madd_bytes + 16 + lds_pad;
         static const bool pack_heads = [] { const char* e = cs_lab_env("CS_ATTN_PACK_HEADS"); return !(e && e[0] == '0'); }();
         uint32_t hb = !pack_heads ? 1u : (Lp <= 32 ? 4u : (Lp <= 64 ? 2u : 1u));
         while (heads % hb) hb >>= 1;
diff --git a/codesearch_amd/csrc/diagnostics.hip b/codesearch_amd/csrc/diagnostics.hip
--- a/codesearch_amd/csrc/diagnostics.hip
+++ b/codesearch_amd/csrc/diagnostics.hip
@@ -339,11 +339,11 @@
     return st;
 }
 
-int32_t cs_debug_attention(int32_t device, const float* qkv, const int32_t* mask, uint32_t B, uint32_t L, uint32_t H,
-                           uint32_t heads, const float* alibi_slopes, uint32_t window, const uint32_t* seq_unit,
-                           const uint32_t* unit_len, uint32_t units, const float* proj_w, const float* proj_bias,
-                           const float* proj_resid, float* out, float* range_pairs_out, uint32_t range_pairs_cap,
-                           uint32_t* range_pairs, uint32_t* range_flag) {
+static int32_t debug_attention(bool with_plan, int32_t device, const float* qkv, const int32_t* mask, uint32_t B, uint32_t L, uint32_t H,
+                               uint32_t heads, const float* alibi_slopes, uint32_t window, const uint32_t* seq_unit,
+                               const uint32_t* unit_len, uint32_t units, const float* proj_w, const float* proj_bias,
+                               const float* proj_resid, float* out, float* range_pairs_out, uint32_t range_pairs_cap,
+                               uint32_t* range_pairs, uint32_t* range_flag) {
     if (!qkv || !mask || !out) return fail(CS_ERR_BAD_ARG, "null buffer");
     if (B == 0 || L == 0 || H == 0 || heads == 0) return fail(CS_ERR_BAD_ARG, "cs_debug_attention needs B, L, H, heads > 0");
     if (H % heads || (H / heads != 32 && H / heads != 64))
@@ -358,6 +358,7 @@
     const uint32_t T = B * L;
     if (!proj_w != !proj_bias || !proj_w != !proj_resid) return fail(CS_ERR_BAD_ARG, "proj_w, proj_bias and proj_resid go together");
     if (proj_w) {
+        if (with_plan) return fail(CS_ERR_BAD_ARG, "attention inside the out-projection takes no mask plan");
         if (alibi_slopes || window || units || range_pairs_out)
             return fail(CS_ERR_BAD_ARG, "attention inside the out-projection takes no ALiBi, window, units or range pairs");
         if (!sp_attn_proj_supported(H, heads, T, L))
@@ -372,7 +373,8 @@
     float *dQ = nullptr, *dW = nullptr, *dB = nullptr, *dR = nullptr, *dC = nullptr, *dAl = nullptr, *dRp = nullptr;
     _Float16 *sQ = nullptr, *sW = nullptr, *sC = nullptr;
     int32_t* dM = nullptr;
-    uint32_t *dF = nullptr, *dSu = nullptr, *dUl = nullptr;
+    uint32_t *dF = nullptr, *dSu = nullptr, *dUl = nullptr, *dPn = nullptr;
+    float* dPm = nullptr;
     auto run = [&]() -> int32_t {
         CS_HIP(hipMalloc(&dQ, q_n * 4)); CS_HIP(hipMalloc(&sQ, q_n * 4)); CS_HIP(hipMalloc(&dM, (size_t)T * 4)); CS_HIP(hipMalloc(&dF, 4));
         CS_HIP(hipMemcpy(dQ, qkv, q_n * 4, hipMemcpyHostToDevice));
@@ -409,8 +411,13 @@
             CS_HIP(hipMalloc(&dRp, pair_cap * 8));
             CS_HIP(hipMemset(dRp, 0, pair_cap * 8));
         }
+        if (with_plan) {
+            CS_HIP(hipMalloc(&dPm, attn_plan_floats(B, L) * 4)); CS_HIP(hipMalloc(&dPn, (size_t)B * 4));
+            CS_TRY(launch_attention_mask_plan(dM, dPm, dPn, B, L, nullptr));
+        }
         uint32_t pairs = 0;
-        CS_TRY(launch_attention_sh2(sQ, dM, sC, dF, B, L, H, heads, nullptr, dRp, range_pairs_out ? &pairs : nullptr, dSu, dUl, dAl, window));
+        CS_TRY(launch_attention_sh2(sQ, dM, sC, dF, B, L, H, heads, nullptr, dRp, range_pairs_out ? &pairs : nullptr, dSu, dUl, dAl, window,
+                                    dPm, dPn));
         CS_HIP(hipDeviceSynchronize());
         if (range_pairs_out) {
             *range_pairs = pairs;
@@ -432,9 +439,26 @@
     const int32_t st = run();
     if (st != CS_OK) (void)hipDeviceSynchronize();
     for (void* p : {(void*)dQ, (void*)dW, (void*)dB, (void*)dR, (void*)dC, (void*)dAl, (void*)dRp, (void*)sQ, (void*)sW, (void*)sC,
-                    (void*)dM, (void*)dF, (void*)dSu, (void*)dUl})
+                    (void*)dM, (void*)dF, (void*)dSu, (void*)dUl, (void*)dPm, (void*)dPn})
         if (p) (void)hipFree(p);
     return st;
+}
+
+int32_t cs_debug_attention(int32_t device, const float* qkv, const int32_t* mask, uint32_t B, uint32_t L, uint32_t H,
+                           uint32_t heads, const float* alibi_slopes, uint32_t window, const uint32_t* seq_unit,
+                           const uint32_t* unit_len, uint32_t units, const float* proj_w, const float* proj_bias,
+                           const float* proj_resid, float* out, float* range_pairs_out, uint32_t range_pairs_cap,
+                           uint32_t* range_pairs, uint32_t* range_flag) {
+    return debug_attention(false, device, qkv, mask, B, L, H, heads, alibi_slopes, window, seq_unit, unit_len, units, proj_w, proj_bias,
+                           proj_resid, out, range_pairs_out, range_pairs_cap, range_pairs, range_flag);
+}
+
+int32_t cs_debug_attention_plan(int32_t device, const float* qkv, const int32_t* mask, uint32_t B, uint32_t L, uint32_t H,
+                                uint32_t heads, const float* alibi_slopes, uint32_t window, const uint32_t* seq_unit,
+                                const uint32_t* unit_len, uint32_t units, float* out, float* range_pairs_out,
+                                uint32_t range_pairs_cap, uint32_t* range_pairs, uint32_t* range_flag) {
+    return debug_attention(true, device, qkv, mask, B, L, H, heads, alibi_slopes, window, seq_unit, unit_len, units, nullptr, nullptr,
+                           nullptr, out, range_pairs_out, range_pairs_cap, range_pairs, range_flag);
 }
 
 }
diff --git a/codesearch_amd/csrc/embedder_forward.hip b/codesearch_amd/csrc/embedder_forward.hip
--- a/codesearch_amd/csrc/embedder_forward.hip
+++ b/codesearch_amd/csrc/embedder_forward.hip
@@ -10,6 +10,10 @@
 void free_workspace(cs_embedder* h) {
     if (h->d_ids) (void)hipFree(h->d_ids);
     if (h->d_mask) (void)hipFree(h->d_mask);
+    if (h->d_attn_madd) (void)hipFree(h->d_attn_madd);
+    if (h->d_attn_ntiles) (void)hipFree(h->d_attn_ntiles);
+    h->d_attn_madd = nullptr;
+    h->d_attn_ntiles = nullptr;
     if (h->d_types) (void)hipFree(h->d_types);
     if (h->d_x) (void)hipFree(h->d_x);
     if (h->d_xs) (void)hipFree(h->d_xs);
@@ -41,6 +45,8 @@
     const size_t H = h->cfg.hidden, I = h->cfg.intermediate;
     CS_HIP(hipMalloc(&h->d_ids, tokens * sizeof(int32_t)));
     CS_HIP(hipMalloc(&h->d_mask, tokens * sizeof(int32_t)));
+    CS_HIP(hipMalloc(&h->d_attn_madd, (tokens + 287 * seqs) * sizeof(float)));
+    CS_HIP(hipMalloc(&h->d_attn_ntiles, seqs * sizeof(uint32_t)));
     CS_HIP(hipMalloc(&h->d_x, tokens * H * sizeof(float)));
     CS_HIP(hipMalloc(&h->d_xs, tokens * H * sizeof(float)));
     CS_HIP(hipMalloc(&h->d_qkv, tokens * 3 * H * sizeof(float)));
@@ -157,6 +163,8 @@
     const float* P;
     float *x, *qkv, *ctx, *mid;
     const int32_t* mask;
+    float* pm;
+    uint32_t* pn;
     _Float16 *xs, *qkvs, *ctxs, *mids;
     SplitLayer sl;
     EncoderLaunch a;
@@ -171,6 +179,8 @@
         ctx = h->d_ctx + t0 * H;
         mid = h->d_mid + t0 * mid_width(cfg);
         mask = h->d_mask + t0;
+        pm = h->d_attn_madd + (size_t)b0_ * attn_plan_stride(L_);
+        pn = h->d_attn_ntiles + b0_;
         xs = reinterpret_cast<_Float16*>(h->d_xs + t0 * H);
         qkvs = reinterpret_cast<_Float16*>(qkv);
         ctxs = reinterpret_cast<_Float16*>(ctx);
@@ -206,6 +216,7 @@
         if (k == DenseKernel::Wide192) return launch_gemm_wide(epi, Ain, Wt, bias, resid, Cf, Csp, Mr, Nn, Kk, h->d_flag, s, 192);
         return launch_gemm_split(epi, Ain, Wt, bias, resid, Cf, Csp, Mr, Nn, Kk, h->d_flag, s);
     }
+    int32_t mask_plan() const { return launch_attention_mask_plan(mask, pm, pn, nb, L, s); }
     int32_t embed() const {
         CS_TRY(mark(-1));
         CS_TRY(launch_row_kernel(0, a, H, s));
@@ -243,6 +254,7 @@
     const bool split = mode == CS_GEMM_SPLIT_F16;
     if (a.types) return fail(CS_ERR_UNSUPPORTED, "the ModernBERT encoder has no token-type table: token-type ids cannot be given");
     a.pos = nullptr; a.type0 = h->d_zero_row;
+    if (split) CS_TRY(mask_plan());
     CS_TRY(embed());
     EncoderLaunch n = a;
     n.src = x; n.x = ctx;
@@ -260,7 +272,7 @@
             CS_TRY(dense(p.qkv, SH_OUT_SPLIT, xs, ws + sl.qkv, bqkv, nullptr, nullptr, qkvs, T, 3 * H, H));
             CS_TRY(launch_rope_split(qkvs, rope, T, L, H, cfg.heads, h->d_flag, s));
             CS_TRY(mark(CS_STAGE_QKV));
-            CS_TRY(launch_attention_sh2(qkvs, mask, ctxs, h->d_flag, nb, L, H, cfg.heads, s, nullptr, nullptr, nullptr, nullptr, nullptr, window));
+            CS_TRY(launch_attention_sh2(qkvs, mask, ctxs, h->d_flag, nb, L, H, cfg.heads, s, nullptr, nullptr, nullptr, nullptr, nullptr, window, pm, pn));
             CS_TRY(mark(CS_STAGE_ATTENTION));
             CS_TRY(dense(p.ao, SH_OUT_F32_RESID, ctxs, ws + sl.ao, P + lo.ao_b, x, x, nullptr, T, H, H));
             CS_TRY(mark(CS_STAGE_OUT_PROJ));
@@ -439,6 +451,7 @@
 }
 
 int32_t Slice::run_q8_rows_source(const ForwardPlan& p) {
+    CS_TRY(mask_plan());
     CS_TRY(embed());
     for (uint32_t l = 0; l < cfg.layers; ++l) {
         const Q8LayerArgs q = q8_layer_begin(l);
@@ -448,7 +461,7 @@
                                           q.xq));
         CS_TRY(mark(CS_STAGE_QKV));
         uint32_t att_pairs = 0;
-        CS_TRY(launch_attention_sh2(qkvs, mask, ctxs, h->d_flag, nb, L, H, cfg.heads, s, q.rp, &att_pairs));
+        CS_TRY(launch_attention_sh2(qkvs, mask, ctxs, h->d_flag, nb, L, H, cfg.heads, s, q.rp, &att_pairs, nullptr, nullptr, nullptr, 0, pm, pn));
         CS_TRY(mark(CS_STAGE_ATTENTION));
         CS_TRY(launch_q8_range(Q8_SRC_SPLIT, ctxs, T, H, q.rg + q.rstep, s, q.rp, att_pairs));
         if (p.ln_fused_ao) {
@@ -486,6 +499,7 @@
 }
 
 int32_t Slice::run_q8_multi_unit() {
+    CS_TRY(mask_plan());
     CS_TRY(embed());
     for (uint32_t l = 0; l < cfg.layers; ++l) {
         const Q8LayerArgs q = q8_layer_begin(l);
@@ -495,7 +509,7 @@
         CS_TRY(launch_gemm_q8_from_source(SH_OUT_SPLIT, Q8_SRC_F32, x, q.rg, q.wq + q.ql.qkv, q.cm, bqkv, nullptr, nullptr, qkvs, T, 3 * H, H, h->d_flag, s, q.rs));
         CS_TRY(mark(CS_STAGE_QKV));
         uint32_t att_pairs = 0;
-        CS_TRY(launch_attention_sh2(qkvs, mask, ctxs, h->d_flag, nb, L, H, cfg.heads, s, q.rp, &att_pairs, su, h->d_unit_len));
+        CS_TRY(launch_attention_sh2(qkvs, mask, ctxs, h->d_flag, nb, L, H, cfg.heads, s, q.rp, &att_pairs, su, h->d_unit_len, nullptr, 0, pm, pn));
         CS_TRY(mark(CS_STAGE_ATTENTION));
         if (!att_pairs || att_pairs > h->cap_range_pairs)
             return fail(CS_ERR_HIP, "attention range pairs (%u) do not fit the pair buffer (%zu)", att_pairs, h->cap_range_pairs);
@@ -520,6 +534,7 @@
 }
 
 int32_t Slice::run_q8_quantise() {
+    CS_TRY(mask_plan());
     CS_TRY(embed());
     for (uint32_t l = 0; l < cfg.layers; ++l) {
         const Q8LayerArgs q = q8_layer_begin(l);
@@ -528,7 +543,7 @@
         CS_TRY(launch_gemm_q8(SH_OUT_SPLIT, q.xq, q.rm, q.wq + q.ql.qkv, q.cm, bqkv, nullptr, nullptr, qkvs, T, 3 * H, H, h->d_flag, s));
         CS_TRY(mark(CS_STAGE_QKV));
         uint32_t att_pairs = 0;
-        CS_TRY(launch_attention_sh2(qkvs, mask, ctxs, h->d_flag, nb, L, H, cfg.heads, s, q.rp, &att_pairs));
+        CS_TRY(launch_attention_sh2(qkvs, mask, ctxs, h->d_flag, nb, L, H, cfg.heads, s, q.rp, &att_pairs, nullptr, nullptr, nullptr, 0, pm, pn));
         if (att_pairs > h->cap_range_pairs) return fail(CS_ERR_HIP, "range pair buffer too small (%u > %zu)", att_pairs, h->cap_range_pairs);
         CS_TRY(mark(CS_STAGE_ATTENTION));
         CS_TRY(launch_q8_quantize(Q8_SRC_SPLIT, ctxs, T, H, q.rg + q.rstep, q.rs, q.xq, q.rm, s, q.rp, att_pairs));
@@ -593,6 +608,7 @@
     const bool nomic = cs_arch_gated(cfg.arch), rotary = cfg.arch == CS_ARCH_NOMIC, jina = cs_arch_alibi(cfg.arch);
     const bool qknorm = cfg.arch == CS_ARCH_JINA_QKNORM;
     const float* alibi = jina ? h->d_alibi : nullptr;
+    CS_TRY(mask_plan());
     CS_TRY(embed());
     for (uint32_t l = 0; l < cfg.layers; ++l) {
         layer_begin(l);
@@ -603,7 +619,7 @@
         if (rotary) CS_TRY(launch_rope_split(qkvs, h->d_rope, T, L, H, cfg.heads, h->d_flag, s));
         if (qknorm) CS_TRY(launch_qk_layernorm_split(qkvs, P + lo.qln_g, cfg.layer_norm_eps, T, H, h->d_flag, s));
         CS_TRY(mark(CS_STAGE_QKV));
-        CS_TRY(launch_attention_sh2(qkvs, mask, ctxs, h->d_flag, nb, L, H, cfg.heads, s, nullptr, nullptr, nullptr, nullptr, alibi));
+        CS_TRY(launch_attention_sh2(qkvs, mask, ctxs, h->d_flag, nb, L, H, cfg.heads, s, nullptr, nullptr, nullptr, nullptr, alibi, 0, pm, pn));
         CS_TRY(mark(CS_STAGE_ATTENTION));
         a.g = P + lo.ao_ln_g; a.b = P + lo.ao_ln_b;
         if (p.fuse_ln) {
diff --git a/codesearch_amd/csrc/embedder_state.hpp b/codesearch_amd/csrc/embedder_state.hpp
--- a/codesearch_amd/csrc/embedder_state.hpp
+++ b/codesearch_amd/csrc/embedder_state.hpp
@@ -111,6 +111,8 @@
     size_t cap_tokens = 0, cap_seqs = 0;
     int32_t* d_ids = nullptr;
     int32_t* d_mask = nullptr;
+    float* d_attn_madd = nullptr;
+    uint32_t* d_attn_ntiles = nullptr;
     int32_t* d_types = nullptr;
     size_t cap_types = 0;
     bool types_on = false;
diff --git a/codesearch_amd/csrc/encoder.hpp b/codesearch_amd/csrc/encoder.hpp
--- a/codesearch_amd/csrc/encoder.hpp
+++ b/codesearch_amd/csrc/encoder.hpp
@@ -43,7 +43,11 @@
 int32_t launch_attention_sh2(const _Float16* qkv_split, const int32_t* mask, void* ctx_split, uint32_t* flag,
                              uint32_t B, uint32_t L, uint32_t H, uint32_t heads, hipStream_t s, float* range_out = nullptr,
                              uint32_t* range_pairs = nullptr, const uint32_t* seq_unit = nullptr,
-                             const uint32_t* unit_len = nullptr, const float* alibi = nullptr, uint32_t window = 0);
+                             const uint32_t* unit_len = nullptr, const float* alibi = nullptr, uint32_t window = 0,
+                             const float* plan_madd = nullptr, const uint32_t* plan_ntiles = nullptr);
+__host__ __device__ constexpr uint32_t attn_plan_stride(uint32_t L) { return (((L + 31) & ~31u) + 255) & ~255u; }
+inline size_t attn_plan_floats(size_t seqs, uint32_t L) { return seqs * attn_plan_stride(L); }
+int32_t launch_attention_mask_plan(const int32_t* mask, float* plan_madd, uint32_t* plan_ntiles, uint32_t B, uint32_t L, hipStream_t s);
 
 enum { SH_OUT_F32 = 0, SH_OUT_F32_RESID = 1, SH_OUT_SPLIT_GELU = 2, SH_OUT_SPLIT = 3,
        SH_OUT_PARTIAL = 4  };
diff --git a/include/codesearch_gpu_diag.h b/include/codesearch_gpu_diag.h
--- a/include/codesearch_gpu_diag.h
+++ b/include/codesearch_gpu_diag.h
@@ -26,6 +26,11 @@
                            const uint32_t* unit_len, uint32_t units, const float* proj_w, const float* proj_bias,
                            const float* proj_resid, float* out, float* range_pairs_out, uint32_t range_pairs_cap,
                            uint32_t* range_pairs, uint32_t* range_flag);
+
+CS_API int32_t cs_debug_attention_plan(int32_t device, const float* qkv, const int32_t* mask, uint32_t B, uint32_t L, uint32_t H,
+                                uint32_t heads, const float* alibi_slopes, uint32_t window, const uint32_t* seq_unit,
+                                const uint32_t* unit_len, uint32_t units, float* out, float* range_pairs_out,
+                                uint32_t range_pairs_cap, uint32_t* range_pairs, uint32_t* range_flag);
 
 CS_API int32_t cs_debug_rows(int32_t device, int32_t which, uint32_t H, uint32_t T, uint32_t L, uint32_t B, float eps, int32_t pooling,
                       const int32_t* ids, const float* word, const float* pos, const float* type_table, const int32_t* types,
```
